# ttaoREtw/semi-tts

Hardware: AMD Instinct MI355X
Metric: mel-frames/sec (decode+attn) (higher is better)
Workload: dtype f32

## Files before the change

include/semitts.h:

```cpp
#ifndef SEMITTS_H
#define SEMITTS_H

#include <stddef.h>
#include <stdint.h>

#ifdef __cplusplus
extern "C" {
#endif

#define ST_ABI_VERSION 1

#define ST_ACT_NONE 0
#define ST_ACT_RELU 1
#define ST_ACT_TANH 2
#define ST_ACT_SIGMOID 3

const char* st_last_error(void);
int st_abi_version(void);
int st_device_info(int* n_cu, int* lds_bytes, char* name, int name_len);

int st_stream_create(void** stream_out);
int st_stream_destroy(void* stream);
int st_stream_sync(void* stream);
int st_graph_begin(void* stream);
// ... 5 lines not shown
int st_event_elapsed_ms(void* ev_start, void* ev_stop, float* ms_out);
int st_event_destroy(void* ev);

typedef struct st_seg {
    const float* x;
    const float* w;
    int ldx;
    int ldw;
    int k;
} st_seg;

int st_lstm_cell_fwd(const st_seg* segs, int nseg, const float* b_ih, const float* b_hh,
                     const float* pre, int ldpre, const float* c_prev, int ldc_prev,
                     const float* mask, float* h_out, int ldh, float* c_out, int ldc,
                     float* gates_out, int B, int H, void* stream);

int st_skinny_linear_fwd(const st_seg* segs, int nseg, const float* bias, int act,
                         const float* mask, int ldmask, float* y, int ldy,
                         int n_split, float* y2, int ldy2, int rep,
                         int B, int N, void* stream);

typedef struct st_t16_view {
    float* base;
    int kb_stride;
    int kb0;
} st_t16_view;

size_t st_packed_weight_floats(const int* k, int nseg, int N, int lstm_H);
size_t st_t16_floats(int B, int K);
int st_pack_weight(const float* const* w, const int* ldw, const int* k, int nseg, int N, int lstm_H,
                   float* packed, void* stream);
typedef struct st_pack_job { const float* w[3]; int ldw[3]; int k[3]; int nseg; int N; int lstm_H; float* packed; } st_pack_job;
int st_pack_weight_batch(const st_pack_job* jobs, int n, void* stream);
int st_pack_weight_t(const float* const* w, const int* ldw, const int* cols, int nseg, int K, float* packed, void* stream);
int st_tile_rows(const float* src, int ld, const st_t16_view* dst, int B, int K, void* stream);
int st_untile_rows(const st_t16_view* src, float* dst, int ld, int B, int K, void* stream);
int st_lstm_cell_packed_fwd(const float* packed_w, const st_t16_view* x, int K,
                            const float* b_ih, const float* b_hh,
                            const float* c_prev, int ldc_prev, const float* mask,
                            const st_t16_view* h_dst0, const st_t16_view* h_dst1,
                            float* c_out, int ldc, float* gates_out,
                            const float* ada_std, const float* ada_mean, const st_t16_view* hadapt_dst,
                            int B, int H, void* stream);
int st_lstm_cell_packed_part_fwd(const float* packed_w, int w_kbs, const st_t16_view* x, int K, const float* part,
                                 const float* b_ih, const float* b_hh,
                                 const float* c_prev, int ldc_prev, const float* mask,
                                 const st_t16_view* h_dst0, const st_t16_view* h_dst1,
                                 float* c_out, int ldc, float* gates_out, int B, int H, void* stream);
typedef struct st_lstm_cell_packed_job {
    const float* packed_w; st_t16_view x; int K;
    const float* b_ih; const float* b_hh;
    const float* c_prev; int ldc_prev; const float* mask;
    st_t16_view h_dst0; st_t16_view h_dst1;
    float* c_out; int ldc; float* gates_out;
    const float* ada_std; const float* ada_mean; st_t16_view hadapt_dst;
    int B, H;
    const float* part; int w_kbs;
} st_lstm_cell_packed_job;
int st_lstm_cell_packed_pair_fwd(const st_lstm_cell_packed_job* j0, const st_lstm_cell_packed_job* j1, void* stream);
int st_skinny_linear_packed_fwd(const float* packed_w, const st_t16_view* x, int K,
                                const float* bias, int act, const float* mask, int ldmask,
                                float* y, int ldy, const st_t16_view* y_dst,
                                int n_split, float* y2, int ldy2, int rep,
                                int n_split2, int act2, const float* mask2, int ldmask2, const st_t16_view* y3_dst,
                                int B, int N, void* stream);

int st_attn_step_fwd(const float* pq, const float* pm, const float* memory,
                     const float* w_prev, int ld_wprev, const float* w_cum_prev,
                     float* w_out, int ld_wout, float* w_cum_out,
                     const float* loc_conv_w, const float* loc_lin_w, const float* v,
                     float* ctx, int ld_ctx,
                     const float* h_q, int ld_hq, const float* ada_std, const float* ada_mean,
                     float* h_adapt, int Q,
                     int B, int L, int A, int E, int F, int K, void* stream);
int st_attn_step_t16_fwd(const float* pq, const float* pm, const float* memory,
                         const float* w_prev, int ld_wprev, const float* w_cum_prev,
                         float* w_out, int ld_wout, float* w_cum_out,
                         const float* loc_conv_w, const float* loc_lin_w, const float* v,
                         const st_t16_view* ctx_dst, int n_ctx_dst, float* ctx, int ld_ctx,
                         int B, int L, int A, int E, int F, int K, void* stream);
int st_attn_pre_fwd(const float* pm, const float* w_prev, int ld_wprev, const float* w_cum_prev,
                    const float* loc_conv_w, const float* loc_lin_w, float* s_buf, int parts,
                    int B, int L, int A, int F, int K, void* stream);
int st_attn_fin_t16_fwd(const float* pq, const float* s_buf, const float* memory, const float* w_cum_prev,
                        float* w_out, int ld_wout, float* w_cum_out, const float* v,
                        const st_t16_view* ctx_dst, int n_ctx_dst, float* ctx, int ld_ctx, int parts,
                        int B, int L, int A, int E, int F, int K, void* stream);
struct st_partial_product_job;
typedef struct st_attn_pre_job {
    const float* pm; const float* w_prev; int ld_wprev; const float* w_cum_prev;
    const float* loc_conv_w; const float* loc_lin_w; float* s_buf;
    int L, A, F, K;
    int parts;
    float* cf_out;
    const struct st_partial_product_job* part;
} st_attn_pre_job;
int st_skinny_linear_packed_attnpre_fwd(const float* packed_w, const st_t16_view* x, int K,
                                        const float* bias, int act, const float* mask, int ldmask,
                                        float* y, int ldy, const st_t16_view* y_dst,
                                        int n_split, float* y2, int ldy2, int rep,
                                        int n_split2, int act2, const float* mask2, int ldmask2, const st_t16_view* y3_dst,
                                        int B, int N, const st_attn_pre_job* pre, void* stream);

typedef struct st_lstm_pw_job {
    int n0, H;
    const float* dh1; int ld1;
    const float* dh2; int ld2; const float* scale2;
    const float* mask;
    const float* gates;
    const float* c; int ldc; const float* c_prev; int ldcp;
    float* dc;
    float* dgates; int ldg;
    st_t16_view dgates_t16;
    int dh1_slabs; long dh1_slab_stride;
} st_lstm_pw_job;
int st_skinny_linear_packed_lstm_bwd_fwd(const float* packed_w, const st_t16_view* x, int K, float* y, int ldy, int B, int N,
                                         const st_lstm_pw_job* job, void* stream);

size_t st_attn_fin_split_workspace_floats(int B, int E, int parts);
int st_attn_fin_split_fwd(const float* pq, const float* s_buf, const float* memory, const float* w_cum_prev,
                          float* w_out, int ld_wout, float* w_cum_out, const float* v,
                          const st_t16_view* ctx_dst, int n_ctx_dst, float* ctx, int ld_ctx, float* workspace, int parts,
                          int B, int L, int A, int E, void* stream);

typedef struct st_attn_fin_job {
    const float* s_buf; const float* memory; const float* w_cum_prev;
    float* w_out; int ld_wout; float* w_cum_out; const float* v;
    st_t16_view ctx_dst[3]; int n_ctx_dst;
    int parts;
    int L, A, E, F, K;
    unsigned* status;
} st_attn_fin_job;
int st_query_attn_fin_fwd(const float* packed_wq, const st_t16_view* h_q, int Q, unsigned long long* granules, unsigned epoch,
                          const st_attn_fin_job* job, int B, void* stream);
typedef struct st_partial_product_job {
    const float* packed_w; int w_kbs; int kb0; int KB;
    st_t16_view x;
    int N;
    float* part;
} st_partial_product_job;
int st_query_attn_fin_part_fwd(const float* packed_wq, const st_t16_view* h_q, int Q, unsigned long long* granules, unsigned epoch,
                               const st_attn_fin_job* job, int B, const st_partial_product_job* part, void* stream);
int st_partial_product_fwd(const st_partial_product_job* job, int B, void* stream);
int st_query_attn_rng_fits(int B, int A, int parts);
size_t st_attn_rng_xchg_words(int B, int E, int parts);
int st_query_attn_rng_fwd(const float* packed_wq, const st_t16_view* h_q, int Q, unsigned long long* granules,
                          unsigned long long* xchg, unsigned epoch, const st_attn_fin_job* job, int B, void* stream);
int st_handoff_wait_selftest(const unsigned long long* granules, unsigned epoch, int A, unsigned* status, float* out,
                             int max_spins, void* stream);

typedef struct st_gemm_epilogue {
    const float* bias;
    int act_pre;
    const float* bn_mean; const float* bn_var; const float* bn_w; const float* bn_b; float bn_eps;
    int act_post;
    const float* res; int ldres;
    const float* highway_h; int ldhw;
    const float* mask; int ldmask;
    int w_tap_major;
    float* splitk_ws;
    int splitk_slabs;
} st_gemm_epilogue;
int st_gemm_splitk_slabs(int Bn, int Tout, int Cin, int N, int KT);

int st_gemm_fwd(const float* A, int lda, const float* W, float* C, int ldc, int coff,
                int Bn, int Tin, int Tout, int Cin, int N, int KT, int pad, int stride, int pool_prev,
                const st_gemm_epilogue* ep, void* stream);

typedef struct st_gemm_job {
    const float* A; int lda; const float* W; float* C; int ldc; int coff;
    int Bn, Tin, Tout, Cin, N, KT, pad, stride, pool_prev;
    st_gemm_epilogue ep;
} st_gemm_job;
int st_gemm_fwd_batch(const st_gemm_job* jobs, int n, void* stream);
int st_gemm_fwd_variant(const float* A, int lda, const float* W, const float* C, int ldc, int coff,
                        int Bn, int Tin, int Tout, int Cin, int N, int KT, int pad, int stride, int pool_prev,
                        const st_gemm_epilogue* ep);
int st_gemm_fwd_batch_variant(const st_gemm_job* jobs, int n);
// ... 134 lines not shown
int st_vq_pack_table(const float* table, float* packed, int D, int V, void* stream);
int st_vq_l2_packed_fwd(const float* x, const float* table, const float* packed, const float* temp, float* p_code,
                        int64_t* idx, float* out, int n, int D, int V, void* stream);
size_t st_vq_l2_workspace_floats(int D, int V);
int st_softmax_bwd(const float* p, const float* dp, const float* relu_scale, float scale, float* dz, float* rowsum,
                   int n, int V, void* stream);
int st_rowscale_combine(const float* a, float alpha, const float* x, const float* r, float beta, const float* c,
                        float* out, int M, int D, void* stream);
int st_vq_mean_fwd(const float* p_code, const float* latent, float* out, int* lens, int* frame_seg, float* frame_w,
                   int B, int T, int D, int V, int max_frames_per_phn, void* stream);
int st_vq_mean_bwd(const float* dout, int n_seg_rows, const int* frame_seg, const float* frame_w, float* dlatent,
                   int B, int T, int D, void* stream);
int st_softmax_argmax(const float* logits, float* p, int64_t* idx, int n, int V, void* stream);

typedef struct st_decoder_weights {
    const float* prenet_w0;
    const float* prenet_w1;
    const float* q_w_ih;
    const float* q_w_hh;
    const float* q_b_ih; const float* q_b_hh;
    const float* attn_query_w;
    const float* attn_v;
    const float* attn_loc_conv_w;
    const float* attn_loc_lin_w;
    const float* d_w_ih;
    const float* d_w_hh;
    const float* d_b_ih; const float* d_b_hh;
    const float* projgate_w;
    const float* projgate_b;
    const float* pre_norm_w[2]; const float* pre_norm_b[2];
    float* pre_norm_rm[2]; float* pre_norm_rv[2]; long long* pre_norm_nbt[2];
    float pre_norm_eps, pre_norm_momentum;
} st_decoder_weights;

typedef struct st_decoder_dims {
    int B, L, E, n_mels, r, P, Q, D, A, F, K;
    int fuse_pre0;
    int prenet_norm;
} st_decoder_dims;

typedef struct st_decoder_io {
    const float* memory;
    const float* pm;
    const float* ada_std;
    const float* ada_mean;
    const int* step_src;
    const float* teacher_pre;
    const float* teacher_mean;
    int Bt, Tt;
    const float* prenet_mask;
    const float* q_mask;
    const float* d_mask;
    int steps;
    float* mel_out;
    float* align_out;
    float* stop_out;
    const float* packed;
    float* xq_tape; float* xd_tape; float* xo_tape;
    float* cq_tape; float* cd_tape; float* wcum_tape;
    float* pq_buf;
    float* pre1_t16;
    float* mel_t16;
    float* zero_row;
    float* gates_q_tape;
    float* gates_d_tape;
    float* attn_s_buf;
    int attn_pre_parts;
    int attn_fin_parts;
    int defer_proj;
    int pre1_step_floats;
    int attn_s_step_floats;
    float* attn_loc_tape;
    float* attn_split_ws;
    int attn_split_parts;
    unsigned long long* pq_granules;
    const float* dec_in0;
    float* pre_nat;
    unsigned long long* attn_xchg;
    unsigned* handoff_status;
    int pair_cells;
    float* pre_nat_tape;
    float* gate_part;
    int gate_part_k;
} st_decoder_io;

int st_decoder_gate_split_k(const st_decoder_dims* d);
size_t st_decoder_packed_floats(const st_decoder_dims* d);
size_t st_decoder_tape_floats(const st_decoder_dims* d, int which);
int st_decoder_pack(const st_decoder_weights* w, const st_decoder_dims* d, float* packed, void* stream);
int st_decoder_forward(const st_decoder_weights* w, const st_decoder_dims* d, const st_decoder_io* io,
                       void* stream);
int st_decoder_fwd_forms(const st_decoder_dims* d, const st_decoder_io* io, int cus, int rng_capacity);

int st_attn_step_bwd(const float* pq, const float* pm, const float* memory,
                     const float* w_prev, int ld_wprev, const float* w_cum_prev, const float* w, int ld_w,
                     const float* loc_conv_w, const float* loc_lin_w, const float* v,
                     const float* const* dctx, const int* ld_dctx, int n_dctx,
                     const float* const* dw_direct, const int* ld_dw, int n_dw,
                     float* dcum, const float* dcum_add, int ld_dcum_add,
                     float* dpq, float* dhist, float* ds_t, float* loc_t, float* dloc_t, float* hist_t,
                     float* dctx_t, float* dv_t,
                     int B, int L, int A, int E, int F, int K, void* stream);

int st_attn_dmem(const float* align, const float* dctx_tape, float* dmem, int B, int steps, int L, int E, void* stream);

typedef struct st_decoder_bwd_weights {
    const float* q_w_cat_t;
    const float* d_w_cat_t;
    const float* attn_query_w_t;
    const float* q_w_cat_t_p16;
    const float* d_w_cat_t_p16;
    const float* attn_query_w_t_p16;
    const float* attn_v; const float* attn_loc_conv_w; const float* attn_loc_lin_w;
} st_decoder_bwd_weights;

typedef struct st_decoder_bwd_io {
    const float* memory; const float* pm; const float* ada_std;
    const float* align;
    const float* wcum_tape;
    const float* cq_tape; const float* cd_tape;
    const float* gates_q_tape; const float* gates_d_tape;
    const float* q_mask; const float* d_mask;
    const float* pq_all;
    int steps; int Bp;
    const float* dxo;
    const float* dalign;
    float* dgq; float* dgd;
    float* dxq; float* dxd;
    float* dpq;
    float* ds_tape; float* loc_tape; float* dloc_tape;
    float* hist_tape; float* dctx_tape; float* dv_tape;
    float* dcq; float* dcd;
    float* dhist[2];
    float* dcum;
    float* dhq_attn;
    float* dgq_t16; float* dgd_t16;
    const int* step_src; int Bt;
    float* dY;
    float* dxo_rw;
    const float* wpg_t;
    const float* pre_w1_t; const float* pre_w0_t;
    const float* own_mask;
    const float* xq_nat;
    const float* pre1_nat;
    float* d2_tape; float* dp1_tape;
    float* tmp_p; float* tmp_in;
    int fuse_pw;
    float* dgd_t16_b;
    float* dpq_t16;
    int need_dxq0;
    const float* attn_s_tape;
    int overlap_attn;
    int prenet_norm;
    const float* pre_y_tape;
    const float* pre_norm_w[2]; const float* pre_norm_rm[2]; const float* pre_norm_rv[2];
    float pre_norm_eps;
    float* dpre_norm_w[2]; float* dpre_norm_b[2];
    int attn_parts; float* dloc_part;
    float* dxd_part; int dxd_splits;
    float* dxq_part; int dxq_splits;
} st_decoder_bwd_io;
int st_decoder_bwd_fuse_dims(const st_decoder_dims* d);
int st_decoder_bwd_forms(const st_decoder_dims* d, const st_decoder_bwd_io* io);
int st_attn_step_bwd_s(const float* pq, const float* pm, const float* memory,
                       const float* w_prev, int ld_wprev, const float* w_cum_prev, const float* w, int ld_w,
                       const float* loc_conv_w, const float* loc_lin_w, const float* v,
                       const float* const* dctx, const int* ld_dctx, int n_dctx,
                       const float* const* dw_direct, const int* ld_dw, int n_dw,
                       float* dcum, const float* dcum_add, int ld_dcum_add,
                       float* dpq, float* dhist, float* ds_t, float* loc_t, float* dloc_t, float* hist_t,
                       float* dctx_t, float* dv_t, const float* s_in,
                       int B, int L, int A, int E, int F, int K, void* stream);
int st_attn_step_bwd_t16(const float* pq, const float* pm, const float* memory,
                         const float* w_prev, int ld_wprev, const float* w_cum_prev, const float* w, int ld_w,
                         const float* loc_conv_w, const float* loc_lin_w, const float* v,
// ... 152 lines not shown
```

semi_tts_amd/_lib.py:

```python
import ctypes as C
import os

HERE = os.path.dirname(os.path.abspath(__file__))
LIB_PATH = os.environ.get('ST_LIB_PATH') or os.path.join(HERE, 'lib', 'libsemitts_hip.so')

c_float_p = C.c_void_p
c_void_p = C.c_void_p


class StSeg(C.Structure):
    _fields_ = [('x', C.c_void_p), ('w', C.c_void_p), ('ldx', C.c_int), ('ldw', C.c_int), ('k', C.c_int)]


class StT16View(C.Structure):
    _fields_ = [('base', C.c_void_p), ('kb_stride', C.c_int), ('kb0', C.c_int)]


class StGemmEpilogue(C.Structure):
    _fields_ = [('bias', C.c_void_p), ('act_pre', C.c_int),
                ('bn_mean', C.c_void_p), ('bn_var', C.c_void_p), ('bn_w', C.c_void_p), ('bn_b', C.c_void_p),
                ('bn_eps', C.c_float), ('act_post', C.c_int),
                ('res', C.c_void_p), ('ldres', C.c_int),
                ('highway_h', C.c_void_p), ('ldhw', C.c_int),
                ('mask', C.c_void_p), ('ldmask', C.c_int), ('w_tap_major', C.c_int),
                ('splitk_ws', C.c_void_p), ('splitk_slabs', C.c_int)]


class StGemmJob(C.Structure):
    _fields_ = [('A', C.c_void_p), ('lda', C.c_int), ('W', C.c_void_p), ('C', C.c_void_p), ('ldc', C.c_int), ('coff', C.c_int),
                ('Bn', C.c_int), ('Tin', C.c_int), ('Tout', C.c_int), ('Cin', C.c_int), ('N', C.c_int), ('KT', C.c_int),
                ('pad', C.c_int), ('stride', C.c_int), ('pool_prev', C.c_int), ('ep', StGemmEpilogue)]


class StRelayoutDesc(C.Structure):
    _fields_ = [('src', C.c_void_p), ('dst', C.c_void_p), ('N', C.c_int), ('Cin', C.c_int), ('KT', C.c_int), ('mode', C.c_int),
                ('blk0', C.c_int), ('ld_dst', C.c_int)]


class StBnBankSeg(C.Structure):
    _fields_ = [('x', C.c_void_p), ('ldx', C.c_int), ('T', C.c_int), ('w', C.c_void_p), ('b', C.c_void_p), ('run_mean', C.c_void_p),
                ('run_var', C.c_void_p), ('batches_tracked', C.c_void_p), ('momentum', C.c_float), ('eps', C.c_float),
                ('mean', C.c_void_p), ('var', C.c_void_p), ('dx', C.c_void_p), ('lddx', C.c_int), ('sums', C.c_void_p)]


class StDecoderWeights(C.Structure):
    _fields_ = [(n, C.c_void_p) for n in (
        'prenet_w0', 'prenet_w1', 'q_w_ih', 'q_w_hh', 'q_b_ih', 'q_b_hh',
        'attn_query_w', 'attn_v', 'attn_loc_conv_w', 'attn_loc_lin_w',
        'd_w_ih', 'd_w_hh', 'd_b_ih', 'd_b_hh', 'projgate_w', 'projgate_b')] + [
        ('pre_norm_w', C.c_void_p * 2), ('pre_norm_b', C.c_void_p * 2), ('pre_norm_rm', C.c_void_p * 2), ('pre_norm_rv', C.c_void_p * 2),
        ('pre_norm_nbt', C.c_void_p * 2), ('pre_norm_eps', C.c_float), ('pre_norm_momentum', C.c_float)]


class StDecoderDims(C.Structure):
    _fields_ = [(n, C.c_int) for n in ('B', 'L', 'E', 'n_mels', 'r', 'P', 'Q', 'D', 'A', 'F', 'K', 'fuse_pre0', 'prenet_norm')]


class StDecoderIO(C.Structure):
    _fields_ = [('memory', C.c_void_p), ('pm', C.c_void_p), ('ada_std', C.c_void_p), ('ada_mean', C.c_void_p),
                ('step_src', C.POINTER(C.c_int)), ('teacher_pre', C.c_void_p), ('teacher_mean', C.c_void_p),
                ('Bt', C.c_int), ('Tt', C.c_int),
                ('prenet_mask', C.c_void_p), ('q_mask', C.c_void_p), ('d_mask', C.c_void_p),
                ('steps', C.c_int),
                ('mel_out', C.c_void_p), ('align_out', C.c_void_p), ('stop_out', C.c_void_p),
                ('packed', C.c_void_p),
                ('xq_tape', C.c_void_p), ('xd_tape', C.c_void_p), ('xo_tape', C.c_void_p),
                ('cq_tape', C.c_void_p), ('cd_tape', C.c_void_p), ('wcum_tape', C.c_void_p),
                ('pq_buf', C.c_void_p), ('pre1_t16', C.c_void_p), ('mel_t16', C.c_void_p),
                ('zero_row', C.c_void_p),
                ('gates_q_tape', C.c_void_p), ('gates_d_tape', C.c_void_p), ('attn_s_buf', C.c_void_p), ('attn_pre_parts', C.c_int), ('attn_fin_parts', C.c_int), ('defer_proj', C.c_int),
                ('pre1_step_floats', C.c_int), ('attn_s_step_floats', C.c_int), ('attn_loc_tape', C.c_void_p),
                ('attn_split_ws', C.c_void_p), ('attn_split_parts', C.c_int), ('pq_granules', C.c_void_p),
                ('dec_in0', C.c_void_p), ('pre_nat', C.c_void_p), ('attn_xchg', C.c_void_p), ('handoff_status', C.c_void_p),
                ('pair_cells', C.c_int), ('pre_nat_tape', C.c_void_p), ('gate_part', C.c_void_p), ('gate_part_k', C.c_int)]


class StDecoderBwdWeights(C.Structure):
    _fields_ = [(n, C.c_void_p) for n in ('q_w_cat_t', 'd_w_cat_t', 'attn_query_w_t', 'q_w_cat_t_p16', 'd_w_cat_t_p16', 'attn_query_w_t_p16',
                                          'attn_v', 'attn_loc_conv_w', 'attn_loc_lin_w')]


class StDecoderBwdIO(C.Structure):
    _fields_ = ([(n, C.c_void_p) for n in ('memory', 'pm', 'ada_std', 'align', 'wcum_tape', 'cq_tape', 'cd_tape',
                                           'gates_q_tape', 'gates_d_tape', 'q_mask', 'd_mask', 'pq_all')] +
                [('steps', C.c_int), ('Bp', C.c_int)] +
                [(n, C.c_void_p) for n in ('dxo', 'dalign', 'dgq', 'dgd', 'dxq', 'dxd', 'dpq', 'ds_tape', 'loc_tape', 'dloc_tape',
                                           'hist_tape', 'dctx_tape', 'dv_tape', 'dcq', 'dcd')] +
                [('dhist', C.c_void_p * 2), ('dcum', C.c_void_p), ('dhq_attn', C.c_void_p), ('dgq_t16', C.c_void_p),
                 ('dgd_t16', C.c_void_p), ('step_src', C.POINTER(C.c_int)), ('Bt', C.c_int)] +
                [(n, C.c_void_p) for n in ('dY', 'dxo_rw', 'wpg_t', 'pre_w1_t', 'pre_w0_t', 'own_mask', 'xq_nat', 'pre1_nat',
                                           'd2_tape', 'dp1_tape', 'tmp_p', 'tmp_in')] +
                [('fuse_pw', C.c_int), ('dgd_t16_b', C.c_void_p), ('dpq_t16', C.c_void_p), ('need_dxq0', C.c_int), ('attn_s_tape', C.c_void_p),
                 ('overlap_attn', C.c_int), ('prenet_norm', C.c_int), ('pre_y_tape', C.c_void_p), ('pre_norm_w', C.c_void_p * 2),
                 ('pre_norm_rm', C.c_void_p * 2), ('pre_norm_rv', C.c_void_p * 2), ('pre_norm_eps', C.c_float),
                 ('dpre_norm_w', C.c_void_p * 2), ('dpre_norm_b', C.c_void_p * 2), ('attn_parts', C.c_int), ('dloc_part', C.c_void_p),
                 ('dxd_part', C.c_void_p), ('dxd_splits', C.c_int), ('dxq_part', C.c_void_p), ('dxq_splits', C.c_int)])



class StLstmPwJob(C.Structure):
    _fields_ = [('n0', C.c_int), ('H', C.c_int), ('dh1', C.c_void_p), ('ld1', C.c_int), ('dh2', C.c_void_p), ('ld2', C.c_int),
                ('scale2', C.c_void_p), ('mask', C.c_void_p), ('gates', C.c_void_p), ('c', C.c_void_p), ('ldc', C.c_int),
                ('c_prev', C.c_void_p), ('ldcp', C.c_int), ('dc', C.c_void_p), ('dgates', C.c_void_p), ('ldg', C.c_int),
                ('dgates_t16', StT16View), ('dh1_slabs', C.c_int), ('dh1_slab_stride', C.c_long)]


class StLstmCellPackedJob(C.Structure):
    _fields_ = [('packed_w', C.c_void_p), ('x', StT16View), ('K', C.c_int), ('b_ih', C.c_void_p), ('b_hh', C.c_void_p),
                ('c_prev', C.c_void_p), ('ldc_prev', C.c_int), ('mask', C.c_void_p), ('h_dst0', StT16View), ('h_dst1', StT16View),
                ('c_out', C.c_void_p), ('ldc', C.c_int), ('gates_out', C.c_void_p), ('ada_std', C.c_void_p), ('ada_mean', C.c_void_p),
                ('hadapt_dst', StT16View), ('B', C.c_int), ('H', C.c_int), ('part', C.c_void_p), ('w_kbs', C.c_int)]


class StAttnBwdJob(C.Structure):
    _fields_ = [('pq', C.c_void_p), ('pm', C.c_void_p), ('memory', C.c_void_p),
                ('w_prev', C.c_void_p), ('ld_wprev', C.c_int), ('w_cum_prev', C.c_void_p), ('w', C.c_void_p), ('ld_w', C.c_int),
                ('loc_conv_w', C.c_void_p), ('loc_lin_w', C.c_void_p), ('v', C.c_void_p),
                ('dctx', C.c_void_p * 3), ('ld_dctx', C.c_int * 3), ('n_dctx', C.c_int),
                ('dw_direct', C.c_void_p * 3), ('ld_dw', C.c_int * 3), ('n_dw', C.c_int),
                ('dcum', C.c_void_p), ('dcum_add', C.c_void_p), ('ld_dcum_add', C.c_int),
                ('dpq', C.c_void_p), ('dpq_t16', StT16View), ('dhist', C.c_void_p), ('ds_t', C.c_void_p), ('loc_t', C.c_void_p),
                ('dloc_t', C.c_void_p), ('hist_t', C.c_void_p), ('dctx_t', C.c_void_p), ('dv_t', C.c_void_p), ('s_in', C.c_void_p),
                ('B', C.c_int), ('L', C.c_int), ('A', C.c_int), ('E', C.c_int), ('F', C.c_int), ('K', C.c_int),
                ('parts', C.c_int), ('dloc_part', C.c_void_p),
                ('dctx_more', C.c_void_p * 3), ('ld_dctx_more', C.c_int * 3), ('n_dctx_more', C.c_int)]


class StAttnHistJob(C.Structure):
    _fields_ = [('dloc_part', C.c_void_p), ('parts', C.c_int), ('loc_conv_w', C.c_void_p),
                ('w_prev', C.c_void_p), ('ld_wprev', C.c_int), ('w_cum_prev', C.c_void_p),
                ('dloc_t', C.c_void_p), ('hist_t', C.c_void_p), ('dhist', C.c_void_p), ('dcum', C.c_void_p),
                ('B', C.c_int), ('L', C.c_int), ('F', C.c_int), ('K', C.c_int)]


class StWgradJob(C.Structure):
    _fields_ = [('dC', C.c_void_p), ('lddc', C.c_int), ('dcoff', C.c_int), ('A', C.c_void_p), ('lda', C.c_int), ('dW', C.c_void_p), ('db', C.c_void_p),
                ('Bn', C.c_int), ('Tin', C.c_int), ('Tout', C.c_int), ('Cin', C.c_int), ('N', C.c_int), ('KT', C.c_int), ('pad', C.c_int)]


class StPartialSumJob(C.Structure):
    _fields_ = [('part', C.c_void_p), ('S', C.c_int), ('N', C.c_int), ('y', C.c_void_p), ('ldy', C.c_int), ('pw', C.c_void_p)]


class StAttnPreJob(C.Structure):
    _fields_ = [('pm', C.c_void_p), ('w_prev', C.c_void_p), ('ld_wprev', C.c_int), ('w_cum_prev', C.c_void_p),
                ('loc_conv_w', C.c_void_p), ('loc_lin_w', C.c_void_p), ('s_buf', C.c_void_p),
                ('L', C.c_int), ('A', C.c_int), ('F', C.c_int), ('K', C.c_int), ('parts', C.c_int), ('cf_out', C.c_void_p),
                ('part', C.c_void_p)]


class StAttnFinJob(C.Structure):
    _fields_ = [('s_buf', C.c_void_p), ('memory', C.c_void_p), ('w_cum_prev', C.c_void_p),
                ('w_out', C.c_void_p), ('ld_wout', C.c_int), ('w_cum_out', C.c_void_p), ('v', C.c_void_p),
                ('ctx_dst', StT16View * 3), ('n_ctx_dst', C.c_int), ('parts', C.c_int),
                ('L', C.c_int), ('A', C.c_int), ('E', C.c_int), ('F', C.c_int), ('K', C.c_int), ('status', C.c_void_p)]


P, I, F, Z = C.c_void_p, C.c_int, C.c_float, C.c_size_t

SIGNATURES = {
    'st_last_error': [],
    'st_abi_version': [],
    'st_device_info': [C.POINTER(I), C.POINTER(I), C.c_char_p, I],
    'st_stream_create': [C.POINTER(P)],
    'st_stream_destroy': [P],
    'st_stream_sync': [P],
    'st_graph_begin': [P],
    'st_graph_end': [P, C.POINTER(P)],
    'st_graph_launch': [P, P],
    'st_graph_destroy': [P],
    'st_event_create': [C.POINTER(P)],
    'st_event_record': [P, P],
    'st_event_elapsed_ms': [P, P, C.POINTER(F)],
    'st_event_destroy': [P],
    'st_lstm_cell_fwd': [C.POINTER(StSeg), I, P, P, P, I, P, I, P, P, I, P, I, P, I, I, P],
    'st_skinny_linear_fwd': [C.POINTER(StSeg), I, P, I, P, I, P, I, I, P, I, I, I, I, P],
    'st_attn_step_fwd': [P, P, P, P, I, P, P, I, P, P, P, P, P, I, P, I, P, P, P, I, I, I, I, I, I, I, P],
    'st_gemm_fwd': [P, I, P, P, I, I, I, I, I, I, I, I, I, I, I, C.POINTER(StGemmEpilogue), P],
    'st_gemm_fwd_batch': [C.POINTER(StGemmJob), I, P],
    'st_gemm_fwd_variant': [P, I, P, P, I, I, I, I, I, I, I, I, I, I, I, C.POINTER(StGemmEpilogue)],
    'st_gemm_fwd_batch_variant': [C.POINTER(StGemmJob), I],
    'st_highway_stack_supported': [I, I],
    'st_highway_stack_fwd': [P, I, C.POINTER(P), C.POINTER(P), C.POINTER(P), C.POINTER(P), I, P, I, I, I, P],
    'st_gemm_splitk_slabs': [I, I, I, I, I],
    'st_bn_stats': [P, I, I, I, I, P, P, P, P, F, P, P, P],
    'st_colreduce_workspace_floats': [I, I],
    'st_bn_apply': [P, I, I, I, I, P, P, P, P, F, I, P],
    'st_lstm_seq_fwd': [P, P, P, P, I, I, P, P, P, I, I, I, I, P],
    'st_lstm_cell_bwd_pointwise': [P, I, P, I, P, I, P, P, P, P, I, P, I, P, P, I, C.POINTER(StT16View), I, I, P],
    'st_lstm_seq_bwd': [P, I, I, P, P, P, P, P, I, I, I, I, P],
    'st_gru_seq_fwd': [P, P, P, P, P, P, P, I, P, I, I, I, I, P],
    'st_gru_seq_bwd': [P, I, P, I, P, P, P, P, P, P, P, I, I, I, I, P],
    'st_gru_seq_variant': [I, I],
    'st_vq_build_table': [P, I, P, I, P, P, I, P, I, P],
    'st_gather_rows': [P, P, P, I, I, I, P],
    'st_vq_l2_fwd': [P, P, P, P, P, P, P, I, I, I, P],
    'st_vq_pack_table': [P, P, I, I, P],
    'st_vq_l2_packed_fwd': [P, P, P, P, P, P, P, I, I, I, P],
    'st_vq_l2_workspace_floats': [I, I],
    'st_ctc_workspace_floats': [I, I],
    'st_ctc_loss': [P, P, C.c_float, P, P, P, I, I, I, I, I, P],
    'st_ctc_greedy_edit_distance': [P, I, I, I, P, I, P, I, P, P, P, P, P],
    'st_ids_edit_distance': [P, I, I, P, I, P, I, P, P, P, P, P],
    'st_hyp_edit_distance': [P, P, I, I, P, I, P, I, P, P, P],
    'st_ctc_beam_workspace_bytes': [I, I, I],
    'st_ctc_beam_search': [P, I, I, I, P, I, I, I, I, F, P, P, P, P, P],
    'st_ctc_beam_search_lm': [P, I, I, I, P, I, I, I, I, F, P, I, I, P, P, P, P, P],
    'st_ctc_align_workspace_bytes': [I, I, I],
    'st_ctc_forced_align': [P, I, I, I, P, P, I, P, I, I, F, P, P, P, P, P, P],
    'st_scalar_combine': [P, I, P, I, P, P],
    'st_scalar_fanout': [P, P, I, P, P],
    'st_softmax_bwd': [P, P, P, C.c_float, P, P, I, I, P],
    'st_rowscale_combine': [P, C.c_float, P, P, C.c_float, P, P, I, I, P],
    'st_vq_mean_fwd': [P, P, P, P, P, P, I, I, I, I, I, P],
    'st_vq_mean_bwd': [P, I, P, P, P, I, I, I, P],
    'st_softmax_argmax': [P, P, P, I, I, P],
    'st_packed_weight_floats': [C.POINTER(I), I, I, I],
    'st_t16_floats': [I, I],
    'st_pack_weight': [C.POINTER(P), C.POINTER(I), C.POINTER(I), I, I, I, P, P],
    'st_pack_weight_t': [C.POINTER(P), C.POINTER(I), C.POINTER(I), I, I, P, P],
    'st_relayout_blocks': [I, I, I],
    'st_relayout_batch': [P, I, I, P, P],
    'st_pack_weight_batch': [P, I, P],
    'st_tile_rows': [P, I, C.POINTER(StT16View), I, I, P],
    'st_untile_rows': [C.POINTER(StT16View), P, I, I, I, P],
    'st_lstm_cell_packed_fwd': [P, C.POINTER(StT16View), I, P, P, P, I, P, C.POINTER(StT16View), C.POINTER(StT16View),
                                P, I, P, P, P, C.POINTER(StT16View), I, I, P],
    'st_lstm_cell_packed_part_fwd': [P, I, C.POINTER(StT16View), I, P, P, P, P, I, P, C.POINTER(StT16View), C.POINTER(StT16View),
                                     P, I, P, I, I, P],
    'st_lstm_cell_packed_pair_fwd': [C.POINTER(StLstmCellPackedJob), C.POINTER(StLstmCellPackedJob), P],
    'st_skinny_linear_packed_fwd': [P, C.POINTER(StT16View), I, P, I, P, I, P, I, C.POINTER(StT16View), I, P, I, I,
                                    I, I, P, I, C.POINTER(StT16View), I, I, P],
    'st_attn_step_t16_fwd': [P, P, P, P, I, P, P, I, P, P, P, P, C.POINTER(StT16View), I, P, I, I, I, I, I, I, I, P],
    'st_skinny_linear_packed_attnpre_fwd': [P, C.POINTER(StT16View), I, P, I, P, I, P, I, C.POINTER(StT16View), I, P, I, I,
                                            I, I, P, I, C.POINTER(StT16View), I, I, C.POINTER(StAttnPreJob), P],
    'st_attn_pre_fwd': [P, P, I, P, P, P, P, I, I, I, I, I, I, P],
    'st_attn_fin_t16_fwd': [P, P, P, P, P, I, P, P, C.POINTER(StT16View), I, P, I, I, I, I, I, I, I, I, P],
    'st_attn_fin_split_workspace_floats': [I, I, I],
    'st_attn_fin_split_fwd': [P, P, P, P, P, I, P, P, C.POINTER(StT16View), I, P, I, P, I, I, I, I, I, P],
    'st_query_attn_fin_fwd': [P, C.POINTER(StT16View), I, P, C.c_uint, C.POINTER(StAttnFinJob), I, P],
    'st_query_attn_fin_part_fwd': [P, C.POINTER(StT16View), I, P, C.c_uint, C.POINTER(StAttnFinJob), I, P, P],
    'st_partial_product_fwd': [P, I, P],
    'st_layer_norm_fwd': [P, I, P, P, F, P, I, P, P, I, I, P],
    'st_layer_norm_bwd': [P, I, P, I, P, P, P, P, I, P, I, I, P],
    'st_log_softmax_fwd': [P, P, I, I, P],
    'st_log_softmax_bwd': [P, P, P, I, I, P],
    'st_prenet_norm_fwd': [P, I, I, P, P, P, P, P, F, F, P, I, C.POINTER(StT16View), I, I, I, P],
    'st_prenet_norm_bwd': [P, I, P, I, I, P, P, P, F, P, P, I, I, P],
    'st_handoff_wait_selftest': [P, C.c_uint, I, P, P, I, P],
    'st_query_attn_rng_fits': [I, I, I],
    'st_attn_rng_xchg_words': [I, I, I],
    'st_query_attn_rng_fwd': [P, C.POINTER(StT16View), I, P, P, C.c_uint, C.POINTER(StAttnFinJob), I, P],
    'st_decoder_packed_floats': [C.POINTER(StDecoderDims)],
    'st_decoder_gate_split_k': [C.POINTER(StDecoderDims)],
    'st_decoder_tape_floats': [C.POINTER(StDecoderDims), I],
    'st_decoder_pack': [C.POINTER(StDecoderWeights), C.POINTER(StDecoderDims), P, P],
    'st_decoder_forward': [C.POINTER(StDecoderWeights), C.POINTER(StDecoderDims), C.POINTER(StDecoderIO), P],
    'st_decoder_fwd_forms': [C.POINTER(StDecoderDims), C.POINTER(StDecoderIO), I, I],
    'st_attn_step_bwd': [P, P, P, P, I, P, P, I, P, P, P, C.POINTER(P), C.POINTER(I), I, C.POINTER(P), C.POINTER(I), I,
                         P, P, I, P, P, P, P, P, P, P, P, I, I, I, I, I, I, P],
    'st_attn_step_bwd_s': [P, P, P, P, I, P, P, I, P, P, P, C.POINTER(P), C.POINTER(I), I, C.POINTER(P), C.POINTER(I), I,
                           P, P, I, P, P, P, P, P, P, P, P, P, I, I, I, I, I, I, P],
    'st_attn_step_bwd_t16': [P, P, P, P, I, P, P, I, P, P, P, C.POINTER(P), C.POINTER(I), I, C.POINTER(P), C.POINTER(I), I,
                             P, P, I, P, C.POINTER(StT16View), P, P, P, P, P, P, P, P, I, I, I, I, I, I, P],
    'st_skinny_linear_packed_lstm_bwd_fwd': [P, C.POINTER(StT16View), I, P, I, I, I, C.POINTER(StLstmPwJob), P],
    'st_skinny_linear_packed_lstm_bwd_attn_bwd': [P, C.POINTER(StT16View), I, P, I, I, I, C.POINTER(StLstmPwJob), C.POINTER(StAttnBwdJob), P],
    'st_attn_bwd_wide_fits': [I, I, I, I, I],
    'st_attn_bwd_variant': [I, I, I, I, I, I, I, I, I, I, P],
    'st_skinny_linear_packed_attn_hist': [P, C.POINTER(StT16View), I, P, I, I, I, C.POINTER(StAttnHistJob), P],
    'st_skinny_partial_attn_hist': [P, C.POINTER(StT16View), I, P, I, I, I, C.POINTER(StAttnHistJob), P],
    'st_decoder_bwd_forms': [C.POINTER(StDecoderDims), C.POINTER(StDecoderBwdIO)],
    'st_decoder_bwd_fuse_dims': [C.POINTER(StDecoderDims)],
    'st_loop_graph_stats': [P, P],
    'st_loop_graphs_enable': [I],
    'st_skinny_partial_attn_bwd': [P, C.POINTER(StT16View), I, P, I, I, I, C.POINTER(StAttnBwdJob), P],
    'st_skinny_linear_packed_lstm_bwd_attn_hist_sum': [P, C.POINTER(StT16View), I, P, I, I, I, C.POINTER(StLstmPwJob), C.POINTER(StAttnHistJob),
                                                       C.POINTER(StPartialSumJob), P],
    'st_skinny_linear_packed_lstm_bwd_attn_hist': [P, C.POINTER(StT16View), I, P, I, I, I, C.POINTER(StLstmPwJob), C.POINTER(StAttnHistJob), P],
    'st_lstm_seq2_fwd': [C.POINTER(P), C.POINTER(P), C.POINTER(P), P, I, C.POINTER(I), P, C.POINTER(P), C.POINTER(P), I, I, I, P],
    'st_lstm_seq2_persist_supported': [I, I, I, I, I, I],
    'st_lstm_seq2_persist_fwd': [C.POINTER(P), C.POINTER(P), C.POINTER(P), P, I, C.POINTER(I), C.POINTER(P), C.POINTER(P), I, I, I, P, P],
    'st_lstm_seq2_bwd_persist_supported': [I, I, I, I, I, I],
    'st_lstm_seq2_bwd_persist': [P, I, C.POINTER(I), C.POINTER(P), C.POINTER(P), C.POINTER(P), C.POINTER(P), I, I, I, P, P],
    'st_lstm_seq2_bwd': [P, I, C.POINTER(I), C.POINTER(P), C.POINTER(P), C.POINTER(P), C.POINTER(P), P, I, I, I, P],
    'st_skinny_linear_pair_fwd': [P, C.POINTER(P), I, I, I, P],
    'st_lstm_seq2_bwd_packed': [P, I, C.POINTER(I), C.POINTER(P), C.POINTER(P), C.POINTER(P), C.POINTER(P), P, P, I, I, I, P],
    'st_skinny_linear_packed_lstm_bwd_pair_fwd': [C.POINTER(P), C.POINTER(StT16View), I, C.POINTER(P), I, I, I, C.POINTER(StLstmPwJob), P],
    'st_lstm_cell_pair_fwd': [P, C.POINTER(P), C.POINTER(P), I, C.POINTER(P), I, C.POINTER(P), I, C.POINTER(P), I, C.POINTER(P), I, I, P],
    'st_attn_dmem': [P, P, P, I, I, I, I, P],
    'st_decoder_backward': [C.POINTER(StDecoderBwdWeights), C.POINTER(StDecoderDims), C.POINTER(StDecoderBwdIO), P],
    'st_decoder_pack_dout': [P, P, P, I, I, I, I, I, I, P],
    'st_decoder_unpack_out': [P, P, P, I, I, I, I, I, I, P],
    'st_decoder_dteacher_sum': [P, P, I, I, I, I, I, I, I, P],
    'st_adain_bwd': [P, C.c_long, I, P, C.c_long, I, P, P, P, P, I, I, I, P],
    'st_mt_blocks': [P, I],
    'st_mt_table_misses': [],
    'st_mt_grad_norm': [P, P, I, P, P, P],
    'st_mt_clip_scale': [P, P, I, P, F, P],
    'st_mt_grad_norm_scaled': [P, P, I, P, P, F, P],
    'st_mt_clip_scale_pre': [P, P, I, P, F, F, P],
    'st_mt_copy': [P, P, P, I, P],
    'st_mt_adam': [P, P, P, P, P, I, F, F, F, F, F, P],
    'st_mt_adam_guarded': [P, P, P, P, P, I, F, F, F, F, F, P, P],
    'st_freq_loss': [P, P, P, P, P, I, I, I, I, F, F, F, I, P],
    'st_freq_loss_workspace_floats': [],
    'st_scale_by': [P, P, P, Z, P],
    'st_bn_norm_fwd': [P, I, I, P, I, I, I, I, P, P, P, P, F, I, P],
    'st_gemm_wgrad_workspace_floats': [I, I, I, I, I],
    'st_gemm_wgrad': [P, I, I, P, I, P, P, I, I, I, I, I, I, I, I, I, P],
    'st_gemm_wgrad_db': [P, I, I, P, I, P, P, P, I, I, I, I, I, I, I, I, I, P],
    'st_gemm_wgrad_batch_workspace_floats': [C.POINTER(StWgradJob), I],
    'st_gemm_wgrad_batch': [C.POINTER(StWgradJob), I, P, P],
    'st_gemm_wgrad_variant': [P, I, I, P, I, I, I, I, I, I, I, I, I, I, I, I],
    'st_gemm_wgrad_batch_variant': [C.POINTER(StWgradJob), I, C.POINTER(I)],
    'st_gemm_wgrad_split': [P, I, I, P, I, P, I, P, P, P, P, I, I, I, I, P],
    'st_colsum': [P, I, I, P, I, I, I, I, P, I, P, P],
    'st_act_bwd': [P, I, P, I, I, P, I, P, I, I, I, P],
    'st_bn_bwd': [P, I, I, P, I, I, I, P, I, I, P, P, P, F, I, I, P, I, I, P, P, I, P, P],
    'st_bn_bwd_reduce': [P, I, I, P, I, I, I, P, I, I, P, P, F, I, I, P, P, P],
    'st_bn_norm_res_mask_fwd': [P, P, P, I, I, P, P, P, P, F, I, P, P, P],
    'st_bn_bwd_reduce_masked': [P, I, P, I, P, I, I, P, I, P, P, F, I, I, P, P, P],
    'st_bn_bwd_apply_masked': [P, I, P, I, P, I, I, P, I, P, P, P, F, I, I, P, I, P, P, I, P, I, P],
    'st_bn_bwd_apply': [P, I, I, P, I, I, I, P, I, I, P, P, P, F, I, I, P, I, P, I, I, P],
    'st_bn_stats_record': [P, I, I, I, I, P, P, P, P],
    'st_bn_sync_merge': [P, I, I, P, P, P, P, F, P, P],
    'st_bn_bwd_apply_sync': [P, I, I, P, I, I, I, P, I, I, P, P, P, F, I, I, P, P, P, I, I, P],
    'st_highway_fwd': [P, P, P, P, Z, P],
    'st_bn_bank_workspace_floats': [I, I, I],
    'st_bn_bank_fwd': [C.POINTER(StBnBankSeg), I, I, I, P, I, I, P, P],
    'st_bn_bank_bwd': [C.POINTER(StBnBankSeg), I, I, I, P, I, I, I, P, P],
    'st_bn_bank_stats_record': [C.POINTER(StBnBankSeg), I, I, I, P, P, P],
    'st_bn_bank_sync_merge': [C.POINTER(StBnBankSeg), I, I, I, P, I, P, P],
    'st_bn_bank_norm': [C.POINTER(StBnBankSeg), I, I, I, P, I, I, P],
    'st_bn_bank_bwd_reduce': [C.POINTER(StBnBankSeg), I, I, I, P, I, I, P, P],
    'st_bn_bank_bwd_apply': [C.POINTER(StBnBankSeg), I, I, I, P, I, I, I, P, P],
    'st_highway_ht_fwd': [P, P, P, I, I, P],
    'st_highway_ht_bwd': [P, P, P, P, P, I, I, P],
    'st_highway_bwd': [P, P, P, P, P, P, P, Z, P],
    'st_pool_prev_fwd': [P, P, I, I, I, P],
    'st_pool_prev_bwd': [P, P, P, I, I, I, P],
    'st_copy3d': [P, C.c_long, C.c_long, P, C.c_long, C.c_long, I, I, I, I, P],
    'st_scatter_add_rows': [P, P, P, I, I, I, P],
    'st_fill': [P, F, Z, P],
    'st_copy2d': [P, I, P, I, I, I, P],
    'st_mean_rows': [P, P, I, I, I, P],
    'st_istft_workspace_floats': [I, I, I, I, I],
    'st_gl_workspace_floats': [I, I, I, I, I],
    'st_stft_fwd': [P, P, I, I, I, I, I, P],
    'st_istft': [P, P, I, I, I, I, I, P, P],
    'st_griffin_lim': [P, C.c_long, C.c_long, C.c_long, I, F, P, P, I, I, I, I, I, I, I, P, P],
    'st_features_workspace_floats': [I],
    'st_audio_features': [P, C.c_long, P, C.c_ulonglong, P, P, P, P, P, I, I, I, I, I, F, P, P, P, P, I, P, P, I, P, I, P, P],
    'st_feature_noise': [P, C.c_long, I, C.c_ulonglong, P],
}
_RESTYPES = {'st_last_error': C.c_char_p, 'st_packed_weight_floats': C.c_size_t, 'st_t16_floats': C.c_size_t,
             'st_decoder_packed_floats': C.c_size_t, 'st_vq_l2_workspace_floats': C.c_size_t, 'st_ctc_workspace_floats': C.c_size_t, 'st_decoder_tape_floats': C.c_size_t,
             'st_gemm_wgrad_workspace_floats': C.c_size_t, 'st_gemm_wgrad_batch_workspace_floats': C.c_size_t, 'st_freq_loss_workspace_floats': C.c_size_t, 'st_attn_fin_split_workspace_floats': C.c_size_t, 'st_attn_rng_xchg_words': C.c_size_t, 'st_colreduce_workspace_floats': C.c_size_t, 'st_mt_blocks': C.c_size_t, 'st_mt_table_misses': C.c_long,
             'st_bn_bank_workspace_floats': C.c_size_t, 'st_istft_workspace_floats': C.c_size_t, 'st_gl_workspace_floats': C.c_size_t,
             'st_features_workspace_floats': C.c_size_t, 'st_ctc_beam_workspace_bytes': C.c_size_t, 'st_ctc_align_workspace_bytes': C.c_size_t}

_lib = None


def load():
    global _lib
    if _lib is not None:
        return _lib
    import torch
    if not os.path.exists(LIB_PATH):
        raise RuntimeError(
            'libsemitts_hip.so not found at %s -- build it with `python -m semi_tts_amd.build` '
            '(hipcc --offload-arch=gfx950).  There is no CPU fallback.' % LIB_PATH)
    lib = C.CDLL(LIB_PATH)
    for name, args in SIGNATURES.items():
        fn = getattr(lib, name)
        fn.argtypes = args
        fn.restype = _RESTYPES.get(name, C.c_int)
    if lib.st_abi_version() != 1:
        raise RuntimeError('libsemitts_hip.so ABI version mismatch')
    _lib = lib
    return lib


def check(rc, what):
    if rc != 0:
        msg = load().st_last_error()
        raise RuntimeError('%s failed (%d): %s' % (what, rc, msg.decode() if msg else '?'))


def check_header_symbols():
    import re
    hdr = open(os.path.join(os.path.dirname(HERE), 'include', 'semitts.h')).read()
    declared = sorted(set(re.findall(r'\b(st_[a-z0-9_]+)\s*\(', hdr)))
    lib = C.CDLL(LIB_PATH)
    missing = [s for s in declared if not hasattr(lib, s)]
    if missing:
        raise RuntimeError('declared in include/semitts.h but not exported by %s: %s' % (LIB_PATH, missing))
    if sorted(SIGNATURES) != declared:
        raise RuntimeError('ctypes table and include/semitts.h disagree: %s' % sorted(set(SIGNATURES) ^ set(declared)))
    return declared
```

semi_tts_amd/csrc/attention.hip:

```cpp
#include "attention_body.h"

namespace {

template <int PART>
int at_launch(const AtArgs& a, hipStream_t stream) {
    ST_CHECK_ARG(a.B > 0 && a.L > 0 && a.A > 0 && a.E > 0 && a.F > 0 && a.K > 0, "attention step: bad dims");
    ST_CHECK_ARG(a.K % 2 == 1, "attention step: location kernel size %d must be odd", a.K);
    ST_CHECK_ARG(a.E % 4 == 0 && a.E / 4 <= AT_THREADS, "attention step: E=%d must be a multiple of 4 and <= %d", a.E, 4 * AT_THREADS);
    ST_CHECK_ARG(PART == 1 || st_aligned16(a.memory), "attention step: memory must be 16-byte aligned");
    ST_CHECK_ARG((a.A % 4 != 0) || (st_aligned16(a.pm) && st_aligned16(a.pq) && st_aligned16(a.v)),
                 "attention step: pm/pq/v must be 16-byte aligned");
    ST_CHECK_ARG(PART == 1 || a.ctx || a.ctx_dst[0].base, "attention step: no context output");
    ST_CHECK_ARG(PART == 0 || (a.s_buf && ((a.A % 4 != 0) || st_aligned16(a.s_buf))), "attention step: S buffer missing / unaligned");
    ST_CHECK_ARG(!a.h_q || (a.ada_std && a.ada_mean && a.h_adapt), "attention step: AdaIN pointers");
    const bool vec = (a.A % 4 == 0) && (a.F % 4 == 0) && st_aligned16(a.pm) && (PART == 1 || (st_aligned16(a.pq) && st_aligned16(a.v))) &&
                     st_aligned16(a.loc_lin_w);
    const int pre_parts = PART == 1 && a.pre_parts > 1 ? a.pre_parts : 1;
    const AtLds o = at_layout(a.L, a.A, a.E, a.F, a.K, PART, at_pos_per(a.L, pre_parts), PART == 1 && vec && a.F == 32 && a.A % 16 == 0);
    const size_t lds_bytes = (size_t)o.total * sizeof(float);
    ST_CHECK_ARG(lds_bytes <= 160 * 1024, "attention step: L=%d needs %zu B of LDS (> 160 KiB)%s", a.L, lds_bytes,
                 PART == 0 ? "; the split form (st_attn_pre_fwd with more parts + st_attn_fin_t16_fwd) takes longer texts" : "");
    static bool configured = false;
    if (!configured) {
        ST_HIP(hipFuncSetAttribute(reinterpret_cast<const void*>(at_kernel<true, PART>),
// ... 131 lines not shown
    for (int p = 0; p < CPF; ++p) cpf[p] = wsb[(size_t)min(p, P - 1) * (4 + E) + 4 + min(tid, E - 1)];
    if (tid < 64) {
        const float m = tid < P ? wsb[(size_t)tid * (4 + E)] : -INFINITY;
        const float s = tid < P ? wsb[(size_t)tid * (4 + E) + 1] : 0.0f;
        const float M = st_wave_max_dpp(m);
        const float t = tid < P ? s * __expf(m - M) : 0.0f;
        const float D = st_wave_sum_dpp(t);
        sc[tid] = tid < P ? __expf(m - M) / D : 0.0f;
    }
    __syncthreads();
    for (int e = tid; e < E; e += AT_THREADS) {
        float s = 0.0f;
        if (e == tid) {
#pragma unroll
            for (int p = 0; p < CPF; ++p) s = p < P ? fmaf(sc[p], cpf[p], s) : s;
            for (int p = CPF; p < P; ++p) s = fmaf(sc[p], wsb[(size_t)p * (4 + E) + 4 + e], s);
        } else {
            for (int p = 0; p < P; ++p) s = fmaf(sc[p], wsb[(size_t)p * (4 + E) + 4 + e], s);
        }
        if (a.ctx) a.ctx[(size_t)b * a.ld_ctx + e] = s;
#pragma unroll
        for (int d = 0; d < 3; ++d)
            if (a.ctx_dst[d].base) a.ctx_dst[d].base[at_t16_off(b, a.ctx_dst[d].kb0 * 16 + e, a.ctx_dst[d].kb_stride)] = s;
    }
    for (int l = tid; l < a.L; l += AT_THREADS) {
        const float w = a.w[(size_t)b * a.ld_w + l] * sc[l / a.Lp];
        a.w[(size_t)b * a.ld_w + l] = w;
        a.w_cum_out[(size_t)b * a.L + l] = w + a.w_cum_prev[(size_t)b * a.L + l];
    }
}

}

extern "C" int st_attn_step_fwd(const float* pq, const float* pm, const float* memory,
                                const float* w_prev, int ld_wprev, const float* w_cum_prev,
                                float* w_out, int ld_wout, float* w_cum_out,
                                const float* loc_conv_w, const float* loc_lin_w, const float* v,
                                float* ctx, int ld_ctx,
                                const float* h_q, int ld_hq, const float* ada_std, const float* ada_mean,
                                float* h_adapt, int Q,
                                int B, int L, int A, int E, int F, int K, void* stream) {
    (void)hipGetLastError();
    AtArgs a;
    memset(&a, 0, sizeof(a));
    a.pq = pq; a.pm = pm; a.memory = memory; a.w_prev = w_prev; a.ld_wprev = ld_wprev; a.w_cum_prev = w_cum_prev;
    a.w_out = w_out; a.ld_wout = ld_wout; a.w_cum_out = w_cum_out;
    a.loc_conv_w = loc_conv_w; a.loc_lin_w = loc_lin_w; a.v = v; a.ctx = ctx; a.ld_ctx = ld_ctx;
    a.h_q = h_q; a.ld_hq = ld_hq; a.ada_std = ada_std; a.ada_mean = ada_mean; a.h_adapt = h_adapt; a.Q = Q;
    a.B = B; a.L = L; a.A = A; a.E = E; a.F = F; a.K = K;
    return at_launch<0>(a, (hipStream_t)stream);
}

extern "C" int st_attn_step_t16_fwd(const float* pq, const float* pm, const float* memory,
                                    const float* w_prev, int ld_wprev, const float* w_cum_prev,
                                    float* w_out, int ld_wout, float* w_cum_out,
                                    const float* loc_conv_w, const float* loc_lin_w, const float* v,
                                    const st_t16_view* ctx_dst, int n_ctx_dst, float* ctx, int ld_ctx,
                                    int B, int L, int A, int E, int F, int K, void* stream) {
    (void)hipGetLastError();
    ST_CHECK_ARG(n_ctx_dst >= 0 && n_ctx_dst <= 3 && (n_ctx_dst == 0 || ctx_dst), "st_attn_step_t16_fwd: n_ctx_dst=%d", n_ctx_dst);
    AtArgs a;
    memset(&a, 0, sizeof(a));
    a.pq = pq; a.pm = pm; a.memory = memory; a.w_prev = w_prev; a.ld_wprev = ld_wprev; a.w_cum_prev = w_cum_prev;
    a.w_out = w_out; a.ld_wout = ld_wout; a.w_cum_out = w_cum_out;
    a.loc_conv_w = loc_conv_w; a.loc_lin_w = loc_lin_w; a.v = v; a.ctx = ctx; a.ld_ctx = ld_ctx;
    for (int d = 0; d < n_ctx_dst; ++d) a.ctx_dst[d] = ctx_dst[d];
    a.B = B; a.L = L; a.A = A; a.E = E; a.F = F; a.K = K;
    return at_launch<0>(a, (hipStream_t)stream);
}

extern "C" int st_attn_pre_fwd(const float* pm, const float* w_prev, int ld_wprev, const float* w_cum_prev,
                               const float* loc_conv_w, const float* loc_lin_w, float* s_buf, int parts,
                               int B, int L, int A, int F, int K, void* stream) {
    (void)hipGetLastError();
    AtArgs a;
    memset(&a, 0, sizeof(a));
    a.pm = pm; a.w_prev = w_prev; a.ld_wprev = ld_wprev; a.w_cum_prev = w_cum_prev;
    a.loc_conv_w = loc_conv_w; a.loc_lin_w = loc_lin_w; a.s_buf = s_buf;
    a.pre_parts = (parts >= 2 && parts <= 64 && (parts & (parts - 1)) == 0) ? parts : 1;
    a.B = B; a.L = L; a.A = A; a.E = 4; a.F = F; a.K = K;
    return at_launch<1>(a, (hipStream_t)stream);
}

extern "C" int st_attn_fin_t16_fwd(const float* pq, const float* s_buf, const float* memory, const float* w_cum_prev,
                                   float* w_out, int ld_wout, float* w_cum_out, const float* v,
                                   const st_t16_view* ctx_dst, int n_ctx_dst, float* ctx, int ld_ctx, int parts,
                                   int B, int L, int A, int E, int F, int K, void* stream) {
    (void)hipGetLastError();
    ST_CHECK_ARG(n_ctx_dst >= 0 && n_ctx_dst <= 3 && (n_ctx_dst == 0 || ctx_dst), "st_attn_fin_t16_fwd: n_ctx_dst=%d", n_ctx_dst);
    ST_CHECK_ARG(parts == 1 || ((parts == 2 || parts == 4 || parts == 8) && E % (4 * parts) == 0),
                 "st_attn_fin_t16_fwd: parts=%d must be 1, 2, 4 or 8 with E=%d a multiple of 4*parts", parts, E);
    AtArgs a;
    memset(&a, 0, sizeof(a));
    a.pq = pq; a.pm = s_buf; a.s_buf = const_cast<float*>(s_buf); a.memory = memory; a.w_cum_prev = w_cum_prev;
    a.w_out = w_out; a.ld_wout = ld_wout; a.w_cum_out = w_cum_out; a.v = v; a.ctx = ctx; a.ld_ctx = ld_ctx;
    a.loc_lin_w = s_buf;
    a.fin_parts = parts;
    for (int d = 0; d < n_ctx_dst; ++d) a.ctx_dst[d] = ctx_dst[d];
    a.B = B; a.L = L; a.A = A; a.E = E; a.F = F; a.K = K;
    return at_launch<2>(a, (hipStream_t)stream);
}

extern "C" size_t st_attn_fin_split_workspace_floats(int B, int E, int parts) { return (size_t)B * parts * (4 + E); }

extern "C" int st_attn_fin_split_fwd(const float* pq, const float* s_buf, const float* memory, const float* w_cum_prev,
                                     float* w_out, int ld_wout, float* w_cum_out, const float* v,
                                     const st_t16_view* ctx_dst, int n_ctx_dst, float* ctx, int ld_ctx, float* workspace, int parts,
                                     int B, int L, int A, int E, void* stream) {
    (void)hipGetLastError();
    ST_CHECK_ARG(pq && s_buf && memory && w_cum_prev && w_out && w_cum_out && v && workspace && B > 0 && L > 0, "st_attn_fin_split_fwd: bad arguments");
    ST_CHECK_ARG(n_ctx_dst >= 0 && n_ctx_dst <= 3 && (n_ctx_dst == 0 || ctx_dst) && (ctx || n_ctx_dst > 0), "st_attn_fin_split_fwd: context outputs");
    ST_CHECK_ARG(A % 4 == 0 && A >= 4 && A <= 256 && E % 4 == 0 && E / 4 <= AT_THREADS && AT_THREADS % (E / 4) == 0,
                 "st_attn_fin_split_fwd: A=%d must be a multiple of 4 up to 256, E=%d / 4 a divisor of %d", A, E, AT_THREADS);
    ST_CHECK_ARG(parts >= 2 && parts <= 64, "st_attn_fin_split_fwd: parts=%d (2..64)", parts);
    const int Lp = (L + parts - 1) / parts;
    ST_CHECK_ARG(Lp <= 512, "st_attn_fin_split_fwd: %d positions per part (> 512): use more parts", Lp);
    parts = (L + Lp - 1) / Lp;
    ST_CHECK_ARG(st_aligned16(pq) && st_aligned16(s_buf) && st_aligned16(memory) && st_aligned16(v) && st_aligned16(workspace),
                 "st_attn_fin_split_fwd: operands must be 16-byte aligned");
    AsArgs s;
    memset(&s, 0, sizeof(s));
    s.pq = pq; s.s_buf = s_buf; s.memory = memory; s.v = v; s.w_tmp = w_out; s.ld_w = ld_wout; s.ws = workspace;
    s.B = B; s.L = L; s.A = A; s.E = E; s.P = parts; s.Lp = Lp;
    hipLaunchKernelGGL(at_split_kernel, dim3(B * parts), dim3(AT_THREADS), 0, (hipStream_t)stream, s);
    ST_LAUNCH_CHECK();
    AcArgs c;
    memset(&c, 0, sizeof(c));
    c.ws = workspace; c.w = w_out; c.ld_w = ld_wout; c.w_cum_prev = w_cum_prev; c.w_cum_out = w_cum_out; c.ctx = ctx; c.ld_ctx = ld_ctx;
    for (int d = 0; d < n_ctx_dst; ++d) c.ctx_dst[d] = ctx_dst[d];
    c.B = B; c.L = L; c.E = E; c.P = parts; c.Lp = Lp;
    hipLaunchKernelGGL(at_combine_kernel, dim3(B), dim3(AT_THREADS), 0, (hipStream_t)stream, c);
    ST_LAUNCH_CHECK();
    return 0;
}


namespace {
__global__ __launch_bounds__(64) void handoff_wait_kernel(const unsigned long long* granules, unsigned epoch, int A, unsigned* status,
                                                          float* out, int max_spins) {
    const int lane = threadIdx.x;
    const f32x4 q4 = at_wait_granules(granules, epoch, lane, A, status, max_spins);
    if (lane * 4 < A) *reinterpret_cast<f32x4*>(out + lane * 4) = q4;
}
}

extern "C" int st_handoff_wait_selftest(const unsigned long long* granules, unsigned epoch, int A, unsigned* status, float* out,
                                        int max_spins, void* stream) {
    (void)hipGetLastError();
    ST_CHECK_ARG(granules && out && A > 0 && A % 4 == 0 && A <= 256 && max_spins > 0 && st_aligned16(out),
                 "st_handoff_wait_selftest: bad arguments");
    hipLaunchKernelGGL(handoff_wait_kernel, dim3(1), dim3(64), 0, (hipStream_t)stream, granules, epoch, A, status, out, max_spins);
    ST_LAUNCH_CHECK();
    return 0;
}
```

semi_tts_amd/csrc/attention_body.h:

```cpp
#pragma once
#include "st_common.h"

#ifndef AT_PROF
#define AT_PROF(n)
#endif

namespace {

constexpr int AT_THREADS = 512;
constexpr int AT_WAVES = AT_THREADS / 64;
constexpr int AT_PF = 12;
constexpr int AT_LB = 8;
constexpr int AT_LP = 6;
constexpr int AT_CB = 4;
constexpr int AT_WLPF = 4;

struct AtArgs {
    const float* pq; const float* pm; const float* memory;
    const float* w_prev; int ld_wprev; const float* w_cum_prev;
    float* w_out; int ld_wout; float* w_cum_out;
    const float* loc_conv_w; const float* loc_lin_w; const float* v;
    float* ctx; int ld_ctx; st_t16_view ctx_dst[3];
    const float* h_q; int ld_hq; const float* ada_std; const float* ada_mean; float* h_adapt; int Q;
    float* s_buf;
    float* cf_out;
    int pre_parts;
    int fin_parts;
    int B, L, A, E, F, K;
    const unsigned long long* pq_gran; unsigned epoch;
    unsigned* status;
};

constexpr int AT_GRAN_SPINS = 1 << 18;
__device__ __forceinline__ f32x4 at_wait_granules(const unsigned long long* base, unsigned epoch, int lane, int A, unsigned* status,
                                                  int max_spins) {
    typedef __attribute__((address_space(1))) unsigned long long gu64;
    gu64* gp = (gu64*)(base + min(lane * 4, A - 4));
    unsigned long long g0 = 0, g1 = 0, g2 = 0, g3 = 0;
    bool ok = false;
    for (int spins = 0; spins < max_spins; ++spins) {
        g0 = __hip_atomic_load(gp + 0, __ATOMIC_RELAXED, __HIP_MEMORY_SCOPE_AGENT);
        g1 = __hip_atomic_load(gp + 1, __ATOMIC_RELAXED, __HIP_MEMORY_SCOPE_AGENT);
        g2 = __hip_atomic_load(gp + 2, __ATOMIC_RELAXED, __HIP_MEMORY_SCOPE_AGENT);
        g3 = __hip_atomic_load(gp + 3, __ATOMIC_RELAXED, __HIP_MEMORY_SCOPE_AGENT);
        const bool mine = (unsigned)(g0 >> 32) == epoch && (unsigned)(g1 >> 32) == epoch &&
                          (unsigned)(g2 >> 32) == epoch && (unsigned)(g3 >> 32) == epoch;
        ok = __all(mine);
        if (ok) break;
        __builtin_amdgcn_s_sleep(2);
    }
    if (!ok && lane == 0 && status) __hip_atomic_fetch_or(status, 1u, __ATOMIC_RELAXED, __HIP_MEMORY_SCOPE_AGENT);
    const float nanv = __builtin_nanf("");
    return ok ? f32x4{__uint_as_float((unsigned)g0), __uint_as_float((unsigned)g1), __uint_as_float((unsigned)g2),
                      __uint_as_float((unsigned)g3)}
              : f32x4{nanv, nanv, nanv, nanv};
}

struct AtLds {
    int wt, wt_ld, wc, kp, hs, hl, cf, cf_ld, e, part, total;
};

__host__ __device__ inline int at_pos_per(int L, int nparts) {
    return nparts > 1 ? (((L + nparts - 1) / nparts + 11) / 12) * 12 : L;
}

__host__ __device__ inline AtLds at_layout(int L, int A, int E, int F, int K, int part = 0, int Lr = 0, bool pre_mfma = false) {
    AtLds o;
    int p = 0;
    const int Lh = part == 1 ? Lr : L;
    o.wt_ld = ((A + 3) & ~3) + 4;
    o.wt = p; if (part == 0 || (part == 1 && !pre_mfma)) p += F * o.wt_ld;
    o.kp = K <= 32 ? 32 : ((K + 3) & ~3);
    o.wc = p; if (part != 2) p += F * 2 * o.kp;
    o.hl = ((Lh + AT_CB + o.kp + 3) + 3) & ~3;
    o.hs = p; if (part != 2) p += 2 * o.hl;
    o.cf_ld = ((((Lh + AT_LP - 1) / AT_LP) * AT_LP + AT_CB + 3) & ~3) + (part == 1 ? 16 : 0);
    o.cf = p; if (part != 2) p += F * o.cf_ld;
    o.e = p; p += ((L + 3) & ~3);
    o.part = p; p += 4 * AT_THREADS;
    o.total = p;
    return o;
}

__device__ __forceinline__ float at_tanh(float x) {
    const float t = __expf(-2.0f * fabsf(x));
    return copysignf(__fdividef(1.0f - t, 1.0f + t), x);
}

__device__ __forceinline__ size_t at_t16_off(int b, int k, int KB) {
    return (((size_t)(b >> 4) * KB + (k >> 4)) * 64 + ((k >> 2) & 3) * 16 + (b & 15)) * 4 + (k & 3);
}

__device__ __forceinline__ void at_put_granule(unsigned long long* p, float v, unsigned epoch) {
    typedef __attribute__((address_space(1))) unsigned long long gu64;
    __hip_atomic_store((gu64*)p, ((unsigned long long)epoch << 32) | (unsigned long long)__float_as_uint(v), __ATOMIC_RELAXED,
                       __HIP_MEMORY_SCOPE_AGENT);
}

struct ArArgs {
    const float* s_buf; const float* memory; const float* v; const float* w_cum_prev;
    float* w_out; int ld_wout; float* w_cum_out;
    st_t16_view ctx_dst[3];
    const unsigned long long* pq_gran;
    unsigned long long* xchg;
    unsigned epoch; unsigned* status;
    int B, L, A, E, P, Lp;
};

template <int NT>
__device__ __forceinline__ void at_range_body(const ArArgs& a, const int wg) {
    __shared__ float es[512];
    __shared__ __attribute__((aligned(16))) float part[4 * NT];
    __shared__ __attribute__((aligned(16))) float pqs[256];
    __shared__ __attribute__((aligned(16))) float cb[8 * 256];
// ... 484 lines not shown
                const float keep = hi32 ? esum[j + 4] : esum[j];
                r4[j] = keep + __shfl_xor(send, 32, 64);
            }
#pragma unroll
            for (int j = 0; j < 2; ++j) {
                const float send = hi16 ? r4[j] : r4[j + 2];
                const float keep = hi16 ? r4[j + 2] : r4[j];
                r2[j] = keep + __shfl_xor(send, 16, 64);
            }
            float r = (hi8 ? r2[1] : r2[0]) + st_dpp<ST_DPP_ROW_ROR8>(hi8 ? r2[0] : r2[1]);
            r = st_oct_sum_dpp(r);
            const int l = l0 + (lane >> 3);
            if ((lane & 7) == 0 && (lane >> 3) < AT_LP && l < L) es[l] = r;
        }
    };
#pragma unroll
    for (int i = 0; i < NPB; ++i) {
        const int l0 = (wave + i * NWV) * AT_LP;
        if (l0 < pos_hi) energy_block(l0, pf_pm4[i]);
    }
    for (int l0 = pos_lo + (wave + NPB * NWV) * AT_LP; l0 < pos_hi; l0 += NWV * AT_LP) energy_block(l0, nullptr);
    if (PART == 1) return;
    AT_PROF(6);
    st_lds_barrier();
    AT_PROF(7);

    if (wave == 0) {
        float m = -INFINITY;
        for (int l = lane; l < L; l += 64) m = fmaxf(m, es[l]);
        m = st_wave_max_dpp(m);
        float s = 0.0f;
        for (int l = lane; l < L; l += 64) {
            const float ex = expf(es[l] - m);
            es[l] = ex;
            s += ex;
        }
        s = st_wave_sum_dpp(s);
        for (int l = lane; l < L; l += 64) {
            const float w = es[l] / s;
            es[l] = w;
            if (PART == 2 && ipart != 0) continue;
            a.w_out[(size_t)b * a.ld_wout + l] = w;
            const float cum_prev = PART == 2 ? (VEC && l < 64 ? pf_cum : a.w_cum_prev[(size_t)b * L + l]) : hs[o.hl + pad + l];
            a.w_cum_out[(size_t)b * L + l] = w + cum_prev;
        }
    }
    AT_PROF(8);
    st_lds_barrier();
    AT_PROF(9);

    if (ctx_active) {
        f32x4 acc = {0.f, 0.f, 0.f, 0.f};
#pragma unroll
        for (int j = 0; j < PFR; ++j) {
            const int l = g + j * ng;
            const float wv = es[min(l, L - 1)];
            const float w = l < L ? wv : 0.0f;
            acc[0] = fmaf(w, mpf[j][0], acc[0]); acc[1] = fmaf(w, mpf[j][1], acc[1]);
            acc[2] = fmaf(w, mpf[j][2], acc[2]); acc[3] = fmaf(w, mpf[j][3], acc[3]);
        }
        for (int l = g + PFR * ng; l < L; l += ng) {
            const f32x4 m4 = st_ld4(memb + (size_t)l * E + e_lo + e4 * 4);
            const float w = es[l];
            acc[0] = fmaf(w, m4[0], acc[0]); acc[1] = fmaf(w, m4[1], acc[1]);
            acc[2] = fmaf(w, m4[2], acc[2]); acc[3] = fmaf(w, m4[3], acc[3]);
        }
        *reinterpret_cast<f32x4*>(part + (size_t)(g * ne4 + e4) * 4) = acc;
    }
    AT_PROF(10);
    st_lds_barrier();
    AT_PROF(11);
    for (int e = tid; e < Es; e += NT) {
        float s = 0.0f;
        for (int gg = 0; gg < ng; ++gg) s += part[gg * Es + e];
        if (a.ctx) a.ctx[(size_t)b * a.ld_ctx + e_lo + e] = s;
#pragma unroll
        for (int d = 0; d < 3; ++d)
            if (a.ctx_dst[d].base) a.ctx_dst[d].base[at_t16_off(b, a.ctx_dst[d].kb0 * 16 + e_lo + e, a.ctx_dst[d].kb_stride)] = s;
    }
    AT_PROF(12);
}


template <bool VEC, int PART, int NT = AT_THREADS>
__global__ __launch_bounds__(NT) void at_kernel(const float* pq, const float* pm, const float* v, const float* w_cum_prev, const float* memory,
                                                float* s_buf, const int L, const int A, const int E, const int fin_parts, const AtArgs rest) {
    extern __shared__ __attribute__((aligned(16))) float at_lds[];
    AtArgs a = rest;
    a.pq = pq; a.pm = pm; a.v = v; a.w_cum_prev = w_cum_prev; a.memory = memory; a.s_buf = s_buf; a.L = L; a.A = A; a.E = E; a.fin_parts = fin_parts;
    at_body<VEC, PART, NT>(a, blockIdx.x, at_lds);
}

}
```

semi_tts_amd/csrc/decoder.hip:

```cpp
#include "st_common.h"
#include "loop_graph.h"
#include <cstdlib>

namespace {

struct ZeroArgs { float* p[12]; size_t floats[12]; int n; };
__global__ __launch_bounds__(256) void zero_regions_kernel(const ZeroArgs a) {
    float* __restrict__ p = a.p[blockIdx.y];
    const size_t n = a.floats[blockIdx.y];
    const size_t n4 = (((uintptr_t)p & 15u) == 0) ? n / 4 : 0;
    const f32x4 z = {0.f, 0.f, 0.f, 0.f};
    for (size_t i = (size_t)blockIdx.x * blockDim.x + threadIdx.x; i < n4; i += (size_t)gridDim.x * blockDim.x) reinterpret_cast<f32x4*>(p)[i] = z;
    for (size_t i = n4 * 4 + (size_t)blockIdx.x * blockDim.x + threadIdx.x; i < n; i += (size_t)gridDim.x * blockDim.x) p[i] = 0.0f;
}

}

extern "C" size_t st_packed_weight_floats(const int* k, int nseg, int N, int lstm_H);
extern "C" size_t st_t16_floats(int B, int K);

namespace {

struct PackedLayout {
    size_t q, pq, d, pg, p0, p1, total;
};

PackedLayout packed_layout(const st_decoder_dims* d) {
    PackedLayout o;
    const int in_dim = d->r * d->n_mels;
    size_t p = 0;
    { int k[3] = {d->P, d->E, d->Q}; o.q = p; p += st_packed_weight_floats(k, 3, 4 * d->Q, d->Q); }
    { int k[1] = {d->Q}; o.pq = p; p += st_packed_weight_floats(k, 1, d->A, 0); }
    { int k[3] = {d->E, d->Q, d->D}; o.d = p; p += st_packed_weight_floats(k, 3, 4 * d->D, d->D); }
    { int k[2] = {d->D, d->E}; o.pg = p; p += st_packed_weight_floats(k, 2, in_dim + 1 + (d->fuse_pre0 ? d->P : 0), 0); }
    { int k[1] = {in_dim}; o.p0 = p; p += st_packed_weight_floats(k, 1, d->P, 0); }
    { int k[1] = {d->P}; o.p1 = p; p += st_packed_weight_floats(k, 1, d->P, 0); }
    o.total = p;
    return o;
}

inline int kb16(int k) { return (k + 15) >> 4; }

struct StepViews {
    int q_kbs, q_ctx, q_h;
    int d_kbs, d_ha, d_h;
    int o_kbs, o_ctx;
    size_t q_floats, d_floats, o_floats;
};

StepViews step_views(const st_decoder_dims* d) {
    StepViews v;
    const int bt = (d->B + 15) >> 4;
    v.q_ctx = kb16(d->P); v.q_h = v.q_ctx + kb16(d->E); v.q_kbs = v.q_h + kb16(d->Q);
    v.d_ha = kb16(d->E); v.d_h = v.d_ha + kb16(d->Q); v.d_kbs = v.d_h + kb16(d->D);
    v.o_ctx = kb16(d->D); v.o_kbs = v.o_ctx + kb16(d->E);
    v.q_floats = (size_t)bt * v.q_kbs * 256; v.d_floats = (size_t)bt * v.d_kbs * 256; v.o_floats = (size_t)bt * v.o_kbs * 256;
    return v;
}

__global__ __launch_bounds__(256) void tile_teacher_kernel(const float* teacher_pre, int Tt, float* xq_tape, size_t slot_floats,
                                                           int q_kbs, int steps, int Bt, int P) {
    const size_t total = (size_t)(steps - 1) * Bt * P;
    for (size_t i = (size_t)blockIdx.x * blockDim.x + threadIdx.x; i < total; i += (size_t)gridDim.x * blockDim.x) {
        const int k = (int)(i % P);
        const size_t sb = i / P;
        const int b = (int)(sb % Bt), s = (int)(sb / Bt) + 1;
        const int frame = s - 1 < Tt ? s - 1 : Tt - 1;
        const float v = teacher_pre[((size_t)b * Tt + frame) * P + k];
        xq_tape[(size_t)s * slot_floats + (((size_t)(b >> 4) * q_kbs + (k >> 4)) * 64 + ((k >> 2) & 3) * 16 + (b & 15)) * 4 + (k & 3)] = v;
    }
}

int prenet_own(const st_decoder_weights* w, const st_decoder_dims* d, const st_decoder_io* io, const PackedLayout& pl, const StepViews& sv,
               int t, bool layer1_done, void* stream) {
    const int in_dim = d->r * d->n_mels;
    const size_t BP = (size_t)d->B * d->P;
    const float* m1 = io->prenet_mask ? io->prenet_mask + ((size_t)t * 2 + 0) * BP : nullptr;
    const float* m2 = io->prenet_mask ? io->prenet_mask + ((size_t)t * 2 + 1) * BP : nullptr;
    st_t16_view mel = {io->mel_t16, kb16(in_dim), 0};
    st_t16_view pre1 = {io->pre1_t16 + (size_t)t * io->pre1_step_floats, kb16(d->P), 0};
    int rc = 0;
    if (d->prenet_norm) {
        st_t16_view next_n = {io->xq_tape + (size_t)(t + 1) * sv.q_floats, sv.q_kbs, 0};
        const st_t16_view* dsts[2] = {&pre1, &next_n};
        const st_t16_view* srcs[2] = {&mel, &pre1};
        const float* pw[2] = {io->packed + pl.p0, io->packed + pl.p1};
        const int Ks[2] = {16 * kb16(in_dim), 16 * kb16(d->P)};
        const float* ms[2] = {m1, m2};
        const int b0 = io->step_src[t] == -1 ? 0 : io->Bt;
        for (int l = 0; l < 2; ++l) {
            float* y = io->pre_nat_tape ? io->pre_nat_tape + ((size_t)t * 2 + l) * BP : io->pre_nat;
            rc = st_skinny_linear_packed_fwd(pw[l], srcs[l], Ks[l], nullptr, ST_ACT_NONE, nullptr, 0, y, d->P, nullptr, 0,
                                             nullptr, 0, 0, 0, 0, nullptr, 0, nullptr, d->B, d->P, stream);
            if (rc) return rc;
            rc = st_prenet_norm_fwd(y, d->P, d->prenet_norm, w->pre_norm_w[l], w->pre_norm_b[l], w->pre_norm_rm[l], w->pre_norm_rv[l],
                                    w->pre_norm_nbt[l], w->pre_norm_eps, w->pre_norm_momentum, ms[l], d->P, dsts[l], b0, d->B, d->P, stream);
            if (rc) return rc;
        }
        return 0;
    }
    if (!layer1_done)
        rc = st_skinny_linear_packed_fwd(io->packed + pl.p0, &mel, 16 * kb16(in_dim), nullptr, ST_ACT_RELU, m1, d->P,
                                         nullptr, 0, &pre1, 0, nullptr, 0, 0, 0, 0, nullptr, 0, nullptr, d->B, d->P, stream);
    if (rc) return rc;
    st_t16_view next = {io->xq_tape + (size_t)(t + 1) * sv.q_floats, sv.q_kbs, 0};
    return st_skinny_linear_packed_fwd(io->packed + pl.p1, &pre1, 16 * kb16(d->P), nullptr, ST_ACT_RELU, m2, d->P,
                                       nullptr, 0, &next, 0, nullptr, 0, 0, 0, 0, nullptr, 0, nullptr, d->B, d->P, stream);
}

}

extern "C" int st_decoder_gate_split_k(const st_decoder_dims* d) {
    if (!d) return 0;
    const StepViews sv = step_views(d);
    int hosted = (sv.d_kbs / 2) / 16 * 16;
    if (hosted < 16 || hosted > sv.d_kbs - sv.d_ha) hosted = sv.d_kbs - sv.d_ha;
    return 16 * (sv.d_kbs - hosted);
}

extern "C" size_t st_decoder_packed_floats(const st_decoder_dims* d) { return d ? packed_layout(d).total : 0; }

extern "C" int st_decoder_pack(const st_decoder_weights* w, const st_decoder_dims* d, float* packed, void* stream) {
    (void)hipGetLastError();
    ST_CHECK_ARG(w && d && packed, "st_decoder_pack: null pointer");
    const PackedLayout pl = packed_layout(d);
    const int in_dim = d->r * d->n_mels;
    st_pack_job j[6];
    memset(j, 0, sizeof(j));
    auto seg = [&](st_pack_job& q, int s, const float* wp, int ld, int k) { q.w[s] = wp; q.ldw[s] = ld; q.k[s] = k; q.nseg = s + 1; };
    seg(j[0], 0, w->q_w_ih, d->P + d->E, d->P); seg(j[0], 1, w->q_w_ih + d->P, d->P + d->E, d->E); seg(j[0], 2, w->q_w_hh, d->Q, d->Q);
    j[0].N = 4 * d->Q; j[0].lstm_H = d->Q; j[0].packed = packed + pl.q;
    seg(j[1], 0, w->attn_query_w, d->Q, d->Q); j[1].N = d->A; j[1].packed = packed + pl.pq;
    seg(j[2], 0, w->d_w_ih, d->E + d->Q, d->E); seg(j[2], 1, w->d_w_ih + d->E, d->E + d->Q, d->Q); seg(j[2], 2, w->d_w_hh, d->D, d->D);
    j[2].N = 4 * d->D; j[2].lstm_H = d->D; j[2].packed = packed + pl.d;
    seg(j[3], 0, w->projgate_w, d->D + d->E, d->D); seg(j[3], 1, w->projgate_w + d->D, d->D + d->E, d->E);
    j[3].N = in_dim + 1 + (d->fuse_pre0 ? d->P : 0); j[3].packed = packed + pl.pg;
    seg(j[4], 0, w->prenet_w0, in_dim, in_dim); j[4].N = d->P; j[4].packed = packed + pl.p0;
    seg(j[5], 0, w->prenet_w1, d->P, d->P); j[5].N = d->P; j[5].packed = packed + pl.p1;
    return st_pack_weight_batch(j, 6, stream);
}

extern "C" size_t st_decoder_tape_floats(const st_decoder_dims* d, int which) {
    if (!d) return 0;
    const StepViews sv = step_views(d);
    return which == 0 ? sv.q_floats : (which == 1 ? sv.d_floats : sv.o_floats);
}

namespace {

enum FwdAttn {
    ATTN_WHOLE,
    ATTN_PRE_FIN,
    ATTN_FIN_SPLIT,
    ATTN_PQ_FIN,
    ATTN_PQ_RNG
};
enum FwdProd {
    PROD_NONE,
    PROD_OWN,
    PROD_PQ_FIN,
    PROD_PQ_PRE
};
struct FwdForms {
    bool pure_tf;
    bool defer;
    bool pre_in_pq;
    bool pair_cells;
    FwdAttn attn;
    FwdProd prod;
    int fin_parts;
    int pq_pre_parts;
    int d_k0;
};

FwdForms fwd_forms(const st_decoder_dims* d, const st_decoder_io* io, int cus, int rng_capacity) {
    FwdForms f;
    const int B = d->B, L = d->L, E = d->E, Q = d->Q, D = d->D, A = d->A, BT = (B + 15) / 16;
    f.pure_tf = io->teacher_pre && io->Bt == B && io->Tt > 0;
    for (int t = 0; t + 1 < io->steps && f.pure_tf; ++t) f.pure_tf = io->step_src[t] == (t < io->Tt ? t : io->Tt - 1);
    f.defer = io->defer_proj != 0;
    f.pair_cells = f.defer && f.pure_tf && io->pair_cells;
    const bool split_attn = io->attn_s_buf != nullptr;
    f.pre_in_pq = split_attn && f.defer;
    const int fp_req = io->attn_fin_parts;
    f.fin_parts = (fp_req == 2 || fp_req == 4 || fp_req == 8) && E % (4 * fp_req) == 0 ? fp_req : 1;
    const int sp = io->attn_split_parts;
    const bool fin_split = split_attn && io->attn_split_ws && sp >= 2 && sp <= 64 && A % 4 == 0 && A <= 256 && E % 4 == 0 &&
                           E / 4 <= 512 && 512 % (E / 4) == 0 && (L + sp - 1) / sp <= 512;
    const bool fin_rng = fin_split && !f.pre_in_pq && io->pq_granules && io->attn_xchg && sp <= 8 && A % 16 == 0 && E % (4 * sp) == 0 &&
                         E / sp <= 256 && (sp - 1) * ((L + sp - 1) / sp) < L && (A / 16) * BT + B * sp <= rng_capacity;
    const bool fuse_pq_fin = !fin_split && split_attn && !f.pre_in_pq && io->pq_granules && A % 16 == 0 && A <= 256 && E % 4 == 0 &&
                             (A / 16) * BT + B * f.fin_parts <= cus;
    f.attn = !split_attn ? ATTN_WHOLE : fin_rng ? ATTN_PQ_RNG : fin_split ? ATTN_FIN_SPLIT : fuse_pq_fin ? ATTN_PQ_FIN : ATTN_PRE_FIN;
    const bool split_d = io->gate_part && (!f.defer || f.pre_in_pq) && B > 16 && B <= 32 && D % 16 == 0 && (D / 4) % 2 == 0 &&
                         E % 16 == 0 && Q % 16 == 0 && st_aligned16(io->gate_part);
    const int pre_parts_split = io->attn_pre_parts > 2 ? 2 : io->attn_pre_parts;
    const bool split_pre = split_d && f.pre_in_pq && A <= 16 * 128 &&
                           ((A + 15) / 16) * BT + B * (pre_parts_split > 1 ? pre_parts_split : 1) + (4 * D) / 32 <= cus;
    f.pq_pre_parts = split_pre ? pre_parts_split : io->attn_pre_parts;
    if (!split_d) f.prod = PROD_NONE;
    else if (split_pre) f.prod = PROD_PQ_PRE;
    else if (fuse_pq_fin && (A / 16) * BT + B * f.fin_parts + (4 * D) / 32 <= cus) f.prod = PROD_PQ_FIN;
    else f.prod = PROD_OWN;
    f.d_k0 = (io->gate_part_k ? io->gate_part_k : st_decoder_gate_split_k(d)) / 16;
    return f;
}

}

int pk_attnrng_capacity();

extern "C" int st_decoder_fwd_forms(const st_decoder_dims* d, const st_decoder_io* io, int cus, int rng_capacity) {
    if (!d || !io || (io->steps > 1 && !io->step_src)) return -1;
    const FwdForms f = fwd_forms(d, io, cus > 0 ? cus : st_device_cus(), rng_capacity > 0 ? rng_capacity : pk_attnrng_capacity());
    return (int)f.attn | ((int)f.prod << 4) | (f.pure_tf ? 1 << 8 : 0) | (f.defer ? 1 << 9 : 0) | (f.pre_in_pq ? 1 << 10 : 0) |
           (f.pair_cells ? 1 << 11 : 0) | (f.fin_parts << 12) | ((f.prod != PROD_NONE ? f.d_k0 & 0xfff : 0) << 16);
}

static int decoder_forward_issue(const st_decoder_weights* w, const st_decoder_dims* d, const st_decoder_io* io, void* stream);

static stlg::Cache g_fwd_graphs;
extern "C" void st_loop_graph_stats(long* fwd3, long* bwd3);
extern "C" void stx_fwd_loop_graph_stats(long* out3) {
    std::lock_guard<std::mutex> lock(g_fwd_graphs.mu);
    out3[0] = g_fwd_graphs.replays; out3[1] = g_fwd_graphs.captures; out3[2] = g_fwd_graphs.eager;
}

extern "C" int st_decoder_forward(const st_decoder_weights* w, const st_decoder_dims* d, const st_decoder_io* io,
                                  void* stream) {
    (void)hipGetLastError();
    ST_CHECK_ARG(w && d && io, "st_decoder_forward: null struct pointer");
    if (io->defer_proj && io->steps > 0 && io->step_src && stlg::enabled(d->B)) {
        st_decoder_io key_io = *io;
        key_io.step_src = nullptr;
        uint64_t key = stlg::fnv(stlg::FNV0, w, sizeof(*w));
        key = stlg::fnv(key, d, sizeof(*d));
        key = stlg::fnv(key, &key_io, sizeof(key_io));
        key = stlg::fnv(key, io->step_src, sizeof(int) * (size_t)io->steps);
        stlg::Entry* e = nullptr;
        hipStream_t issue_on = (hipStream_t)stream;
        const int mode = stlg::begin(g_fwd_graphs, key, (hipStream_t)stream, &e, &issue_on);
        if (mode == 1) return 0;
        int rc = decoder_forward_issue(w, d, io, (void*)issue_on);
        if (mode == 2) {
            rc = stlg::end(g_fwd_graphs, e, (hipStream_t)stream, rc);
            if (rc == -5) st_set_error("st_decoder_forward: capturing the loop into a hipGraph failed");
        }
        return rc;
    }
    return decoder_forward_issue(w, d, io, stream);
}

static int decoder_forward_issue(const st_decoder_weights* w, const st_decoder_dims* d, const st_decoder_io* io, void* stream) {
    ST_CHECK_ARG(w && d && io, "st_decoder_forward: null struct pointer");
    const int B = d->B, L = d->L, E = d->E, P = d->P, Q = d->Q, D = d->D, A = d->A;
    const int steps = io->steps;
    const int in_dim = d->r * d->n_mels;
    ST_CHECK_ARG(B > 0 && L > 0 && steps > 0 && in_dim > 0, "st_decoder_forward: B=%d L=%d steps=%d", B, L, steps);
    ST_CHECK_ARG(io->memory && io->pm && io->ada_std && io->ada_mean && io->step_src && io->packed,
                 "st_decoder_forward: null input");
    ST_CHECK_ARG(io->mel_out && io->align_out && io->stop_out, "st_decoder_forward: null output");
    ST_CHECK_ARG(io->xq_tape && io->xd_tape && io->xo_tape && io->cq_tape && io->cd_tape && io->wcum_tape &&
                 io->pq_buf && io->pre1_t16 && io->mel_t16 && io->zero_row, "st_decoder_forward: null tape/scratch");
    ST_CHECK_ARG(d->prenet_norm >= 0 && d->prenet_norm <= 3 && (!d->prenet_norm || (!d->fuse_pre0 && io->pre_nat && w->pre_norm_w[0] &&
                 w->pre_norm_w[1] && w->pre_norm_b[0] && w->pre_norm_b[1])), "st_decoder_forward: normalised prenet needs pre_nat, the norm weights and fuse_pre0 = 0");
    for (int t = 0; t + 1 < steps; ++t) {
        const int src = io->step_src[t];
        ST_CHECK_ARG(!d->fuse_pre0 || src == -1, "st_decoder_forward: fuse_pre0 needs every next input to be the own output");
        ST_CHECK_ARG(src >= -2 && (src < 0 || (io->teacher_pre && src < io->Tt)), "st_decoder_forward: step_src[%d]=%d invalid", t, src);
        ST_CHECK_ARG(src != -2 || io->teacher_mean, "st_decoder_forward: step_src[%d]=-2 without teacher_mean", t);
        ST_CHECK_ARG(src == -1 || (io->Bt > 0 && io->Bt <= B), "st_decoder_forward: Bt=%d invalid", io->Bt);
    }
    const StepViews sv = step_views(d);
    ST_CHECK_ARG(io->gate_part_k == 0 || !io->gate_part || (io->gate_part_k % 16 == 0 && io->gate_part_k >= 16 * sv.d_ha && io->gate_part_k < 16 * sv.d_kbs),
                 "st_decoder_forward: gate_part_k = %d must be a multiple of 16 in [%d, %d)", io->gate_part_k, 16 * sv.d_ha, 16 * sv.d_kbs);
    FwdForms f = fwd_forms(d, io, st_device_cus(), pk_attnrng_capacity());
    ST_CHECK_ARG(!f.defer || (f.pure_tf && !d->fuse_pre0), "st_decoder_forward: defer_proj needs pure teacher forcing");
#ifdef ST_ABLATE
    const int skip = getenv("ST_SKIP") ? atoi(getenv("ST_SKIP")) : 0;
    if ((skip & 8) || (f.prod == PROD_PQ_FIN && (skip & 6)) || (f.prod == PROD_PQ_PRE && (skip & 2))) f.prod = PROD_NONE;
#define ST_SKIPPED(bit) (skip & (1 << (bit)))
#else
#define ST_SKIPPED(bit) 0
#endif
    hipStream_t st = (hipStream_t)stream;
    const PackedLayout pl = packed_layout(d);
    const size_t BQ = (size_t)B * Q, BD = (size_t)B * D, BL = (size_t)B * L;
    ZeroArgs za;
    memset(&za, 0, sizeof(za));
    auto zero = [&](void* p, size_t bytes) { za.p[za.n] = (float*)p; za.floats[za.n] = bytes / sizeof(float); ++za.n; };
    zero(io->cq_tape, BQ * sizeof(float));
    zero(io->cd_tape, BD * sizeof(float));
    zero(io->wcum_tape, BL * sizeof(float));
    zero(io->zero_row, BL * sizeof(float));
    zero(io->xq_tape, sv.q_floats * sizeof(float));
    zero(io->xd_tape, sv.d_floats * sizeof(float));
    if (io->attn_loc_tape) zero(io->attn_loc_tape, BL * d->F * sizeof(float));
    const int sp_parts = io->attn_split_parts;
    if (f.attn == ATTN_PQ_FIN || f.attn == ATTN_PQ_RNG) zero(io->pq_granules, (size_t)B * A * sizeof(unsigned long long));
    if (f.attn == ATTN_PQ_RNG) zero(io->attn_xchg, st_attn_rng_xchg_words(B, E, sp_parts) * sizeof(unsigned long long));
    {
        size_t most = 0;
        for (int i = 0; i < za.n; ++i) most = za.floats[i] > most ? za.floats[i] : most;
        size_t blocks = (most / 4 + 255) / 256 + 1;
        if (blocks > 256) blocks = 256;
        hipLaunchKernelGGL(zero_regions_kernel, dim3((unsigned)blocks, za.n), dim3(256), 0, st, za);
        ST_LAUNCH_CHECK();
    }
    if (io->dec_in0) {
        st_t16_view xq0 = {io->xq_tape, sv.q_kbs, 0};
        int rc0 = st_tile_rows(io->dec_in0, P, &xq0, B, P, stream);
        if (rc0) return rc0;
    }
    if (f.pure_tf && steps > 1) {
        const size_t total = (size_t)(steps - 1) * B * P;
        size_t blocks = (total + 255) / 256;
        if (blocks > 4096) blocks = 4096;
        hipLaunchKernelGGL(tile_teacher_kernel, dim3((unsigned)blocks), dim3(256), 0, st, io->teacher_pre, io->Tt, io->xq_tape,
                           sv.q_floats, sv.q_kbs, steps, B, P);
        ST_LAUNCH_CHECK();
    }

    const size_t ldmel = (size_t)steps * in_dim;
    const int ldal = steps * L;
    const int Kq = 16 * sv.q_kbs, Kd = 16 * sv.d_kbs, Ko = 16 * sv.o_kbs;
    st_partial_product_job pj_d;
    memset(&pj_d, 0, sizeof(pj_d));
    pj_d.packed_w = io->packed + pl.d; pj_d.w_kbs = sv.d_kbs; pj_d.kb0 = f.d_k0; pj_d.KB = sv.d_kbs - f.d_k0; pj_d.N = 4 * D; pj_d.part = io->gate_part;
    int rc = 0;
    for (int t = 0; t < steps; ++t) {
        float* xq = io->xq_tape + (size_t)t * sv.q_floats;
        float* xq_next = io->xq_tape + (size_t)(t + 1) * sv.q_floats;
        float* xd = io->xd_tape + (size_t)t * sv.d_floats;
        float* xd_next = io->xd_tape + (size_t)(t + 1) * sv.d_floats;
        float* xo = io->xo_tape + (size_t)t * sv.o_floats;
        pj_d.x = st_t16_view{xd, sv.d_kbs, f.d_k0};

        st_t16_view xq_v = {xq, sv.q_kbs, 0};
        st_t16_view hq_dst = {xq_next, sv.q_kbs, sv.q_h};
        st_t16_view ha_dst = {xd, sv.d_kbs, sv.d_ha};
        if (!(f.pair_cells && t > 0) && !ST_SKIPPED(0)) {
            rc = st_lstm_cell_packed_fwd(io->packed + pl.q, &xq_v, Kq, w->q_b_ih, w->q_b_hh,
                                         io->cq_tape + (size_t)t * BQ, Q, io->q_mask ? io->q_mask + (size_t)t * BQ : nullptr,
                                         &hq_dst, nullptr, io->cq_tape + (size_t)(t + 1) * BQ, Q,
                                         io->gates_q_tape ? io->gates_q_tape + (size_t)t * 4 * BQ : nullptr,
                                         io->ada_std, io->ada_mean, &ha_dst, B, Q, stream);
            if (rc) return rc;
        }

        if (f.attn != ATTN_PQ_FIN && f.attn != ATTN_PQ_RNG && !ST_SKIPPED(1)) {
            if (f.pre_in_pq && t > 0) {
                st_attn_pre_job job = {io->pm, io->align_out + (size_t)(t - 1) * L, ldal, io->wcum_tape + (size_t)t * BL,
                                       w->attn_loc_conv_w, w->attn_loc_lin_w, io->attn_s_buf + (size_t)t * io->attn_s_step_floats, L, A, d->F,
                                       d->K, f.pq_pre_parts, io->attn_loc_tape ? io->attn_loc_tape + (size_t)t * BL * d->F : nullptr};
                if (f.prod == PROD_PQ_PRE) job.part = &pj_d;
                rc = st_skinny_linear_packed_attnpre_fwd(io->packed + pl.pq, &hq_dst, 16 * kb16(Q), nullptr, ST_ACT_NONE, nullptr, 0,
                                                         io->pq_buf, A, nullptr, 0, nullptr, 0, 0, 0, 0, nullptr, 0, nullptr, B, A,
                                                         &job, stream);
            } else
                rc = st_skinny_linear_packed_fwd(io->packed + pl.pq, &hq_dst, 16 * kb16(Q), nullptr, ST_ACT_NONE, nullptr, 0,
                                                 io->pq_buf, A, nullptr, 0, nullptr, 0, 0, 0, 0, nullptr, 0, nullptr, B, A, stream);
            if (rc) return rc;
        }

        st_t16_view ctx_dst[3] = {{xq_next, sv.q_kbs, sv.q_ctx}, {xd, sv.d_kbs, 0}, {xo, sv.o_kbs, sv.o_ctx}};
        const float* s_t = t == 0 || f.attn == ATTN_WHOLE ? io->pm : io->attn_s_buf + (size_t)t * io->attn_s_step_floats;
        auto fin_job = [&](int parts) {
            st_attn_fin_job fj;
            memset(&fj, 0, sizeof(fj));
            fj.s_buf = s_t; fj.memory = io->memory; fj.w_cum_prev = io->wcum_tape + (size_t)t * BL;
            fj.w_out = io->align_out + (size_t)t * L; fj.ld_wout = ldal; fj.w_cum_out = io->wcum_tape + (size_t)(t + 1) * BL; fj.v = w->attn_v;
            for (int c = 0; c < 3; ++c) fj.ctx_dst[c] = ctx_dst[c];
            fj.status = io->handoff_status;
            fj.n_ctx_dst = 3; fj.parts = parts; fj.L = L; fj.A = A; fj.E = E; fj.F = d->F; fj.K = d->K;
            return fj;
        };
        switch (f.attn) {
        case ATTN_WHOLE:
            if (!ST_SKIPPED(2))
                rc = st_attn_step_t16_fwd(io->pq_buf, io->pm, io->memory, t == 0 ? io->zero_row : io->align_out + (size_t)(t - 1) * L,
                                          t == 0 ? L : ldal, io->wcum_tape + (size_t)t * BL, io->align_out + (size_t)t * L, ldal,
                                          io->wcum_tape + (size_t)(t + 1) * BL,
                                          w->attn_loc_conv_w, w->attn_loc_lin_w, w->attn_v, ctx_dst, 3, nullptr, 0,
                                          B, L, A, E, d->F, d->K, stream);
            break;
        case ATTN_PRE_FIN:
            if (!ST_SKIPPED(2))
                rc = st_attn_fin_t16_fwd(io->pq_buf, s_t, io->memory, io->wcum_tape + (size_t)t * BL,
                                         io->align_out + (size_t)t * L, ldal, io->wcum_tape + (size_t)(t + 1) * BL, w->attn_v,
                                         ctx_dst, 3, nullptr, 0, f.fin_parts, B, L, A, E, d->F, d->K, stream);
            break;
        case ATTN_FIN_SPLIT:
            if (!ST_SKIPPED(2))
                rc = st_attn_fin_split_fwd(io->pq_buf, s_t, io->memory, io->wcum_tape + (size_t)t * BL, io->align_out + (size_t)t * L, ldal,
                                           io->wcum_tape + (size_t)(t + 1) * BL, w->attn_v, ctx_dst, 3, nullptr, 0, io->attn_split_ws, sp_parts,
                                           B, L, A, E, stream);
            break;
        case ATTN_PQ_FIN:
            if (!(ST_SKIPPED(1) || ST_SKIPPED(2))) {
                const st_attn_fin_job fj = fin_job(f.fin_parts);
                rc = f.prod == PROD_PQ_FIN
                         ? st_query_attn_fin_part_fwd(io->packed + pl.pq, &hq_dst, 16 * kb16(Q), io->pq_granules, (unsigned)(t + 1), &fj, B, &pj_d, stream)
                         : st_query_attn_fin_fwd(io->packed + pl.pq, &hq_dst, 16 * kb16(Q), io->pq_granules, (unsigned)(t + 1), &fj, B, stream);
            }
            break;
        case ATTN_PQ_RNG:
            if (!(ST_SKIPPED(1) || ST_SKIPPED(2))) {
                const st_attn_fin_job fj = fin_job(sp_parts);
                rc = st_query_attn_rng_fwd(io->packed + pl.pq, &hq_dst, 16 * kb16(Q), io->pq_granules, io->attn_xchg, (unsigned)(t + 1), &fj, B, stream);
            }
            break;
        }
        if (rc) return rc;

        if (f.prod == PROD_OWN || (f.prod == PROD_PQ_PRE && t == 0)) {
            rc = st_partial_product_fwd(&pj_d, B, stream);
            if (rc) return rc;
        }
        st_t16_view xd_v = {xd, sv.d_kbs, 0};
        st_t16_view hd_dst0 = {xd_next, sv.d_kbs, sv.d_h};
        st_t16_view hd_dst1 = {xo, sv.o_kbs, 0};
        const bool part = f.prod != PROD_NONE;
        if (!ST_SKIPPED(3)) {
            if (f.pair_cells && t + 1 < steps) {
                st_lstm_cell_packed_job jd, jq;
                memset(&jd, 0, sizeof(jd)); memset(&jq, 0, sizeof(jq));
                jd.packed_w = io->packed + pl.d; jd.x = xd_v; jd.K = Kd; jd.b_ih = w->d_b_ih; jd.b_hh = w->d_b_hh;
                if (part) { jd.K = 16 * f.d_k0; jd.part = io->gate_part; jd.w_kbs = sv.d_kbs; }
                jd.c_prev = io->cd_tape + (size_t)t * BD; jd.ldc_prev = D; jd.mask = io->d_mask ? io->d_mask + (size_t)t * BD : nullptr;
                jd.h_dst0 = hd_dst0; jd.h_dst1 = hd_dst1; jd.c_out = io->cd_tape + (size_t)(t + 1) * BD; jd.ldc = D;
                jd.gates_out = io->gates_d_tape ? io->gates_d_tape + (size_t)t * 4 * BD : nullptr;
                jd.B = B; jd.H = D;
                float* xq_next2 = io->xq_tape + (size_t)(t + 2) * sv.q_floats;
                jq.packed_w = io->packed + pl.q; jq.x = st_t16_view{xq_next, sv.q_kbs, 0}; jq.K = Kq; jq.b_ih = w->q_b_ih; jq.b_hh = w->q_b_hh;
                jq.c_prev = io->cq_tape + (size_t)(t + 1) * BQ; jq.ldc_prev = Q; jq.mask = io->q_mask ? io->q_mask + (size_t)(t + 1) * BQ : nullptr;
                jq.h_dst0 = st_t16_view{xq_next2, sv.q_kbs, sv.q_h}; jq.c_out = io->cq_tape + (size_t)(t + 2) * BQ; jq.ldc = Q;
                jq.gates_out = io->gates_q_tape ? io->gates_q_tape + (size_t)(t + 1) * 4 * BQ : nullptr;
                jq.ada_std = io->ada_std; jq.ada_mean = io->ada_mean; jq.hadapt_dst = st_t16_view{xd_next, sv.d_kbs, sv.d_ha};
                jq.B = B; jq.H = Q;
                rc = st_lstm_cell_packed_pair_fwd(&jd, &jq, stream);
            } else if (part)
                rc = st_lstm_cell_packed_part_fwd(io->packed + pl.d, sv.d_kbs, &xd_v, 16 * f.d_k0, io->gate_part, w->d_b_ih, w->d_b_hh,
                                                  io->cd_tape + (size_t)t * BD, D, io->d_mask ? io->d_mask + (size_t)t * BD : nullptr,
                                                  &hd_dst0, &hd_dst1, io->cd_tape + (size_t)(t + 1) * BD, D,
                                                  io->gates_d_tape ? io->gates_d_tape + (size_t)t * 4 * BD : nullptr, B, D, stream);
            else
                rc = st_lstm_cell_packed_fwd(io->packed + pl.d, &xd_v, Kd, w->d_b_ih, w->d_b_hh,
                                             io->cd_tape + (size_t)t * BD, D, io->d_mask ? io->d_mask + (size_t)t * BD : nullptr,
                                             &hd_dst0, &hd_dst1, io->cd_tape + (size_t)(t + 1) * BD, D,
                                             io->gates_d_tape ? io->gates_d_tape + (size_t)t * 4 * BD : nullptr,
                                             nullptr, nullptr, nullptr, B, D, stream);
            if (rc) return rc;
        }

        st_t16_view xo_v = {xo, sv.o_kbs, 0};
        st_t16_view mel_dst = {io->mel_t16, kb16(in_dim), 0};
        st_t16_view pre1_dst = {io->pre1_t16 + (size_t)t * io->pre1_step_floats, kb16(P), 0};
        const bool fuse = d->fuse_pre0 != 0;
        if (f.defer) continue;
        const bool split_attn = f.attn != ATTN_WHOLE;
        st_attn_pre_job job = {io->pm, io->align_out + (size_t)t * L, ldal, io->wcum_tape + (size_t)(t + 1) * BL,
                               w->attn_loc_conv_w, w->attn_loc_lin_w,
                               split_attn ? io->attn_s_buf + (size_t)(t + 1) * io->attn_s_step_floats : nullptr, L, A, d->F, d->K,
                               io->attn_pre_parts, io->attn_loc_tape ? io->attn_loc_tape + (size_t)(t + 1) * BL * d->F : nullptr};
        if (!ST_SKIPPED(4)) {
            rc = st_skinny_linear_packed_attnpre_fwd(io->packed + pl.pg, &xo_v, ST_SKIPPED(7) ? Ko / 4 : Ko, w->projgate_b, ST_ACT_NONE, nullptr, 0,
                                                     io->mel_out + (size_t)t * in_dim, (int)ldmel, fuse ? nullptr : &mel_dst, in_dim,
                                                     io->stop_out + (size_t)t * d->r, steps * d->r, d->r,
                                                     fuse ? in_dim + 1 : 0, ST_ACT_RELU,
                                                     io->prenet_mask ? io->prenet_mask + (size_t)t * 2 * B * P : nullptr, P,
                                                     fuse ? &pre1_dst : nullptr, B, in_dim + 1 + (fuse ? P : 0),
                                                     split_attn && t + 1 < steps && !ST_SKIPPED(6) ? &job : nullptr, stream);
            if (rc) return rc;
        }

        if (t + 1 < steps) {
            const int src = io->step_src[t];
            st_t16_view next = {xq_next, sv.q_kbs, 0};
            if ((src == -1 || io->Bt < B) && !ST_SKIPPED(5)) {
                rc = prenet_own(w, d, io, pl, sv, t, fuse, stream);
                if (rc) return rc;
            }
            if (!f.pure_tf && src >= 0) rc = st_tile_rows(io->teacher_pre + (size_t)src * P, io->Tt * P, &next, io->Bt, P, stream);
            else if (!f.pure_tf && src == -2) rc = st_tile_rows(io->teacher_mean, P, &next, io->Bt, P, stream);
            if (rc) return rc;
        } else if (d->prenet_norm == 3 && (io->step_src[t] == -1 || io->Bt < B)) {
            rc = prenet_own(w, d, io, pl, sv, t, false, stream);
            if (rc) return rc;
        }
    }
    return 0;
}
```

semi_tts_amd/csrc/skinny_packed.hip:

```cpp
#include "st_common.h"
#include "attention_body.h"
#include "attention_bwd_body.h"
#include <cstdlib>

#ifndef PK_PROF
#define PK_PROF(n)
#endif
#ifndef RT2_PROF
#define RT2_PROF(n)
#endif

namespace {

constexpr int PK_MAXSEG = 3;

__host__ __device__ inline int pk_kb(int k) { return (k + 15) >> 4; }

struct PackArgs {
    const float* w[PK_MAXSEG]; int ldw[PK_MAXSEG]; int k[PK_MAXSEG]; int kb0[PK_MAXSEG];
    int nseg; int N; int H; int KB; int tiles; float* out;
};

__device__ __forceinline__ void pack_weight_body(const PackArgs& a);
__global__ __launch_bounds__(256) void pack_weight_kernel(const PackArgs a) { pack_weight_body(a); }
// ... 812 lines not shown
    if (exp_ == 2 && i >= n_ab) return;
    if (i < n_ab) {
        if (KW * 64 > AB_THREADS && (int)threadIdx.x >= AB_THREADS) return;
        const int part = i / ab.B;
        ab_body<true, LBLK, NS>(ab, i - part * ab.B, pk_dyn_lds, part);
        return;
    }
    pk_part_body<KW, TRIP>(p, i - n_ab, red);
}

template <int KW, int TRIP>
__global__ __launch_bounds__(KW * 64) void pk_part_hist_kernel(const PkPartArgs p, const int n_h, const AbHistArgs hist) {
    extern __shared__ __attribute__((aligned(16))) float pk_dyn_lds[];
    __shared__ f32x4 red[KW * 4 * 64];
    const int i = blockIdx.x;
    if (i < n_h) { ab_hist_body(hist, i, pk_dyn_lds); return; }
    pk_part_body<KW, TRIP>(p, i - n_h, red);
}

template <int KW, int TRIP>
__global__ __launch_bounds__(KW * 64) void pk_part_kernel(const PkPartArgs p) {
    __shared__ f32x4 red[KW * 4 * 64];
    pk_part_body<KW, TRIP>(p, blockIdx.x, red);
}

template <int KW, int TRIP, int LBLK, int NS>
__global__ __launch_bounds__(2 * KW * 64) void pk_pw_ab_dual_kernel(const f32x4* w, const f32x4* x, const int w_kbs, const int x_kbs, const int KB,
                                                                    const int B, const int N, const int n_ab,
                                                                    const PkArgs rest, const PkPw pw, const AbArgs ab, const int exp_) {
    extern __shared__ __attribute__((aligned(16))) float pk_dyn_lds[];
    __shared__ f32x4 red[2 * KW * 64];
    static_assert(KW * 64 == AB_THREADS, "both parts use 512-thread bodies");
    const int i = blockIdx.x;
    const int half = __builtin_amdgcn_readfirstlane((int)threadIdx.x / (KW * 64));
    if (exp_ == 1 && i < n_ab) return;
    if (exp_ == 2 && i >= n_ab) return;
    if (i < n_ab) {
        if (half) return;
        const int part = i / ab.B;
        ab_body<true, LBLK, NS>(ab, i - part * ab.B, pk_dyn_lds, part);
        return;
    }
    PkArgs a = rest;
    a.w = w; a.x = x; a.w_kbs = w_kbs; a.x_kbs = x_kbs; a.KB = KB; a.B = B; a.N = N; a.H = 0;
    pk_body<2, 1, KW, TRIP>(a, i - n_ab, half, red + half * KW * 64, &pw, half * KW * 64);
}

template <int MODE, int NB, int KW, int TRIP>
__global__ __launch_bounds__(KW * 64) void pk_pw_hist_kernel(const f32x4* w, const f32x4* x, const int w_kbs, const int x_kbs, const int KB,
                                                             const int B, const int N, const int tiles_a, const int n_h, const int n_sum,
                                                             const PkArgs rest, const PkPw pw, const AbHistArgs hist, const PkSumArgs sum, const int exp_) {
    extern __shared__ __attribute__((aligned(16))) float pk_dyn_lds[];
    __shared__ f32x4 red[KW * NB * 64];
    const int i = blockIdx.x;
    if (exp_ == 3 && i < n_h) return;
    if (exp_ == 4 && i >= n_h && i < n_h + n_sum) return;
    if (exp_ == 5 && i >= n_h + n_sum) return;
    if (i < n_h) { ab_hist_body(hist, i, pk_dyn_lds); return; }
    if (i < n_h + n_sum) { pk_sum_body(sum, i - n_h, KW * 64); return; }
    PkArgs a = rest;
    a.w = w; a.x = x; a.w_kbs = w_kbs; a.x_kbs = x_kbs; a.KB = KB; a.B = B; a.N = N; a.H = 0;
    const int j = i - n_h - n_sum;
    const int by = j / tiles_a;
    pk_body<MODE, NB, KW, TRIP>(a, j - by * tiles_a, by, red, MODE == 2 ? &pw : nullptr);
}

template <int NB, int KW, int TRIP, bool VEC>
__global__ __launch_bounds__(KW * 64) void pk_attnpre_kernel(const f32x4* w, const f32x4* x, const int w_kbs, const int x_kbs, const int KB,
                                                             const int B, const int N, const int tiles_a, const int n_lin,
                                                             const float* at_pm, const float* at_wprev, const int at_L,
                                                             const PkArgs a_rest, const AtArgs t_rest) {
    extern __shared__ __attribute__((aligned(16))) float pk_dyn_lds[];
    __shared__ f32x4 red[KW * NB * 64];
    PkArgs a = a_rest;
    a.w = w; a.x = x; a.w_kbs = w_kbs; a.x_kbs = x_kbs; a.KB = KB; a.B = B; a.N = N;
    AtArgs t = t_rest;
    t.pm = at_pm; t.w_prev = at_wprev; t.L = at_L;
    static_assert(KW * 64 == AT_THREADS, "both parts use 512-thread workgroups");
    const int i = blockIdx.x;
    if (i < n_lin) {
        const int by = n_lin <= 2 * tiles_a ? (i >= tiles_a ? 1 : 0) : i / tiles_a;
        pk_body<1, NB, KW, TRIP>(a, i - by * tiles_a, by, red);
    }
    else at_body<VEC, 1>(t, i - n_lin, pk_dyn_lds);
}

template <int NB, int KW, int TRIP, bool VEC>
__global__ __launch_bounds__(KW * 64) void pk_attnpre_part_kernel(const f32x4* w, const f32x4* x, const int w_kbs, const int x_kbs, const int KB,
                                                                  const int B, const int N, const int tiles_a, const int n_lin,
                                                                  const float* at_pm, const float* at_wprev, const int at_L,
                                                                  const PkArgs a_rest, const AtArgs t_rest, const int n_at, const PkPartArgs p) {
    extern __shared__ __attribute__((aligned(16))) float pk_dyn_lds[];
    __shared__ f32x4 red[KW * NB * 64];
    static_assert(KW * 64 == AT_THREADS, "both parts use 512-thread workgroups");
    const int i = blockIdx.x;
    if (i < n_lin) {
        PkArgs a = a_rest;
        a.w = w; a.x = x; a.w_kbs = w_kbs; a.x_kbs = x_kbs; a.KB = KB; a.B = B; a.N = N;
        const int by = n_lin <= 2 * tiles_a ? (i >= tiles_a ? 1 : 0) : i / tiles_a;
        pk_body<1, NB, KW, TRIP>(a, i - by * tiles_a, by, red);
    } else if (i < n_lin + n_at) {
        AtArgs t = t_rest;
        t.pm = at_pm; t.w_prev = at_wprev; t.L = at_L;
        at_body<VEC, 1>(t, i - n_lin, pk_dyn_lds);
    } else pk_part_body<KW, 2>(p, i - n_lin - n_at, reinterpret_cast<f32x4*>(pk_dyn_lds));
}


template <int NB, int KW, int TRIP>
__global__ __launch_bounds__(KW * 64) void pk_attnfin_kernel(const f32x4* w, const f32x4* x, const int w_kbs, const int x_kbs, const int KB,
                                                             const int B, const int N, const int tiles_a, const int n_lin,
                                                             const PkArgs a_rest, const AtArgs t) {
    extern __shared__ __attribute__((aligned(16))) float pk_dyn_lds[];
    __shared__ f32x4 red[KW * NB * 64];
    static_assert(KW * 64 == AT_THREADS, "both parts use 512-thread workgroups");
    const int i = blockIdx.x;
    if (i < n_lin) {
        PkArgs a = a_rest;
        a.w = w; a.x = x; a.w_kbs = w_kbs; a.x_kbs = x_kbs; a.KB = KB; a.B = B; a.N = N;
        const int by = n_lin <= 2 * tiles_a ? (i >= tiles_a ? 1 : 0) : i / tiles_a;
        pk_body<1, NB, KW, TRIP>(a, i - by * tiles_a, by, red);
    }
    else at_body<true, 2, AT_THREADS, true>(t, i - n_lin, pk_dyn_lds);
}

template <int NB, int KW, int TRIP>
__global__ __launch_bounds__(KW * 64) void pk_attnfin_part_kernel(const f32x4* w, const f32x4* x, const int w_kbs, const int x_kbs, const int KB,
                                                                  const int B, const int N, const int tiles_a, const int n_lin,
                                                                  const PkArgs a_rest, const AtArgs t, const int n_att, const PkPartArgs p) {
    extern __shared__ __attribute__((aligned(16))) float pk_dyn_lds[];
    __shared__ f32x4 red[KW * NB * 64];
    static_assert(KW * 64 == AT_THREADS, "both parts use 512-thread workgroups");
    const int i = blockIdx.x;
    if (i < n_lin) {
        PkArgs a = a_rest;
        a.w = w; a.x = x; a.w_kbs = w_kbs; a.x_kbs = x_kbs; a.KB = KB; a.B = B; a.N = N;
        const int by = n_lin <= 2 * tiles_a ? (i >= tiles_a ? 1 : 0) : i / tiles_a;
        pk_body<1, NB, KW, TRIP>(a, i - by * tiles_a, by, red);
    }
    else if (i < n_att) at_body<true, 2, AT_THREADS, true>(t, i - n_lin, pk_dyn_lds);
    else pk_part_body<KW, 2>(p, i - n_att, reinterpret_cast<f32x4*>(pk_dyn_lds));
}

template <int NB, int KW, int TRIP>
__global__ __launch_bounds__(KW * 64, 4) void pk_attnrng_kernel(const f32x4* w, const f32x4* x, const int w_kbs, const int x_kbs, const int KB,
                                                                const int B, const int N, const int tiles_a, const int n_lin,
                                                                const PkArgs a_rest, const ArArgs t) {
    __shared__ f32x4 red[KW * NB * 64];
    static_assert(KW * 64 == AT_THREADS, "both parts use 512-thread workgroups");
    const int i = blockIdx.x;
    if (i < n_lin) {
        PkArgs a = a_rest;
        a.w = w; a.x = x; a.w_kbs = w_kbs; a.x_kbs = x_kbs; a.KB = KB; a.B = B; a.N = N;
        const int by = n_lin <= 2 * tiles_a ? (i >= tiles_a ? 1 : 0) : i / tiles_a;
        pk_body<1, NB, KW, TRIP>(a, i - by * tiles_a, by, red);
    }
    else at_range_body<AT_THREADS>(t, i - n_lin);
}

#ifndef PK_TRIP_SMALL
#define PK_TRIP_SMALL 2
#endif
int pk_fill(PkArgs& a, const float* packed_w, const st_t16_view* x, int K, const char* who);

template <int NB>
int pk_launch_attnpre(const PkArgs& a, int tiles, const AtArgs& t, hipStream_t st, const PkPartArgs* pp = nullptr) {
    constexpr int KW = 8, TRIP = NB == 1 ? PK_TRIP_SMALL : 2;
    const int BT = (a.B + 15) >> 4, gy = (BT + NB - 1) / NB;
    if constexpr (NB == 1) if (pp) {
        const bool vec = (t.A % 4 == 0) && (t.F % 4 == 0) && st_aligned16(t.pm) && st_aligned16(t.loc_lin_w) && st_aligned16(t.s_buf);
        const AtLds o = at_layout(t.L, t.A, t.E, t.F, t.K, 1, at_pos_per(t.L, t.pre_parts > 1 ? t.pre_parts : 1), vec && t.F == 32 && t.A % 16 == 0);
        size_t lds = (size_t)o.total * sizeof(float);
        if (lds < sizeof(f32x4) * KW * 4 * 64) lds = sizeof(f32x4) * KW * 4 * 64;
        ST_CHECK_ARG(lds + sizeof(f32x4) * KW * NB * 64 <= 160 * 1024, "linear + attention-pre launch: L=%d needs too much LDS (use more parts)", t.L);
        auto kern = vec ? pk_attnpre_part_kernel<NB, KW, TRIP, true> : pk_attnpre_part_kernel<NB, KW, TRIP, false>;
        static size_t configured[2] = {0, 0};
        if (lds > 32 * 1024 && lds > configured[vec ? 1 : 0]) {
            ST_HIP(hipFuncSetAttribute(reinterpret_cast<const void*>(kern), hipFuncAttributeMaxDynamicSharedMemorySize, (int)lds));
            configured[vec ? 1 : 0] = lds;
        }
        const int n_at = t.B * (t.pre_parts > 1 ? t.pre_parts : 1);
        hipLaunchKernelGGL(kern, dim3(tiles * gy + n_at + (pp->N >> 5)), dim3(KW * 64), lds, st, a.w, a.x, a.w_kbs, a.x_kbs,
                           a.KB, a.B, a.N, tiles, tiles * gy, t.pm, t.w_prev, t.L, a, t, n_at, *pp);
        ST_LAUNCH_CHECK();
        return 0;
    }
    const bool vec = (t.A % 4 == 0) && (t.F % 4 == 0) && st_aligned16(t.pm) && st_aligned16(t.loc_lin_w) && st_aligned16(t.s_buf);
    const AtLds o = at_layout(t.L, t.A, t.E, t.F, t.K, 1, at_pos_per(t.L, t.pre_parts > 1 ? t.pre_parts : 1), vec && t.F == 32 && t.A % 16 == 0);
    const size_t lds = (size_t)o.total * sizeof(float);
    ST_CHECK_ARG(lds + sizeof(f32x4) * KW * NB * 64 <= 160 * 1024, "linear + attention-pre launch: L=%d needs too much LDS (use more parts)", t.L);
    auto kern = vec ? pk_attnpre_kernel<NB, KW, TRIP, true> : pk_attnpre_kernel<NB, KW, TRIP, false>;
    static size_t configured[2] = {0, 0};
    if (lds > 48 * 1024 && lds > configured[vec ? 1 : 0]) {
        ST_HIP(hipFuncSetAttribute(reinterpret_cast<const void*>(kern), hipFuncAttributeMaxDynamicSharedMemorySize, (int)lds));
        configured[vec ? 1 : 0] = lds;
    }
    hipLaunchKernelGGL(kern, dim3(tiles * gy + t.B * (t.pre_parts > 1 ? t.pre_parts : 1)), dim3(KW * 64), lds, st, a.w, a.x, a.w_kbs, a.x_kbs,
                       a.KB, a.B, a.N, tiles, tiles * gy, t.pm, t.w_prev, t.L, a, t);
    ST_LAUNCH_CHECK();
    return 0;
}

template <int MODE, int NB>
int pk_launch(const PkArgs& a, int tiles, hipStream_t st) {
    constexpr int KW = 8, TRIP = (MODE == 1 && NB == 1) ? PK_TRIP_SMALL : 2;
    const int BT = (a.B + 15) >> 4;
    dim3 grid(tiles, (BT + NB - 1) / NB);
    hipLaunchKernelGGL((pk_kernel<MODE, NB, KW, TRIP>), grid, dim3(KW * 64), 0, st, a.w, a.x, a.w_kbs, a.x_kbs, a.KB, a.B, a.N, a.H, a);
    ST_LAUNCH_CHECK();
    return 0;
}

#ifndef PK_LSTM_KW
#define PK_LSTM_KW 8
#endif
#ifndef PK_LSTM_TRIP
#define PK_LSTM_TRIP 2
#endif
inline bool pk_rt2_shape(int B, int tiles) {
    const int BT = (B + 15) >> 4;
    return (tiles & 1) == 0 && (BT == 2 || BT == 4) && B > 16 * (BT - 1);
}

template <int MODE>
int pk_dispatch(const PkArgs& a, int tiles, hipStream_t st) {
    const int BT = (a.B + 15) >> 4;
    if (MODE == 0 && pk_rt2_shape(a.B, tiles)) {
        constexpr int LKW = PK_LSTM_KW, LTR = PK_LSTM_TRIP;
#if defined(PK_AUX_Q0) || defined(PK_AUX_D0)
        if (BT == 2 && a.KB > 128)
            hipLaunchKernelGGL((pk_lstm_rt2_kernel<LKW, LTR, 1, PK_AUX_D0, PK_AUX_D1>), dim3(tiles / 2, 2), dim3(LKW * 64), 0, st, a.w, a.x, a.w_kbs, a.x_kbs, a.KB, a.B, a.H, a);
        else if (BT == 2)
            hipLaunchKernelGGL((pk_lstm_rt2_kernel<LKW, LTR, 1, PK_AUX_Q0, PK_AUX_Q1>), dim3(tiles / 2, 2), dim3(LKW * 64), 0, st, a.w, a.x, a.w_kbs, a.x_kbs, a.KB, a.B, a.H, a);
        else
#endif
        if (BT == 2)
            hipLaunchKernelGGL((pk_lstm_rt2_kernel<LKW, LTR, 1>), dim3(tiles / 2, 2), dim3(LKW * 64), 0, st, a.w, a.x, a.w_kbs, a.x_kbs, a.KB, a.B, a.H, a);
#ifdef PK_C5_NB4
        else if (getenv("ST_C5_NB4"))
            hipLaunchKernelGGL((pk_lstm_rt2_kernel<LKW, LTR, 4>), dim3(tiles / 2, 1), dim3(LKW * 64), 0, st, a.w, a.x, a.w_kbs, a.x_kbs, a.KB, a.B, a.H, a);
#endif
        else
            hipLaunchKernelGGL((pk_lstm_rt2_kernel<LKW, LTR, 2>), dim3(tiles / 2, 2), dim3(LKW * 64), 0, st, a.w, a.x, a.w_kbs, a.x_kbs, a.KB, a.B, a.H, a);
        ST_LAUNCH_CHECK();
        return 0;
    }
    if (MODE == 1 && BT > 1) {
        int nb = 1;
        while (nb < 4 && tiles * ((BT + nb - 1) / nb) > 512) ++nb;
        if (nb == 1) return pk_launch<MODE, 1>(a, tiles, st);
        if (nb == 2) return pk_launch<MODE, 2>(a, tiles, st);
        if (nb == 3) return pk_launch<MODE, 3>(a, tiles, st);
        return pk_launch<MODE, 4>(a, tiles, st);
    }
    if (BT == 1) return pk_launch<MODE, 1>(a, tiles, st);
    if (BT == 2) return pk_launch<MODE, 2>(a, tiles, st);
    if (BT == 3) return pk_launch<MODE, 3>(a, tiles, st);
    return pk_launch<MODE, 4>(a, tiles, st);
}

PkOut pk_out(const st_t16_view* v) {
    PkOut o = {nullptr, 0, 0};
    if (v && v->base) { o.base = v->base; o.kb_stride = v->kb_stride; o.kb0 = v->kb0; }
    return o;
}

int pk_fill(PkArgs& a, const float* packed_w, const st_t16_view* x, int K, const char* who) {
    ST_CHECK_ARG(packed_w && x && x->base && K > 0, "%s: bad packed operands", who);
    ST_CHECK_ARG(st_aligned16(packed_w) && st_aligned16(x->base), "%s: operands must be 16-byte aligned", who);
    ST_CHECK_ARG(x->kb0 >= 0 && x->kb0 + pk_kb(K) <= x->kb_stride, "%s: k-block range [%d,%d) outside the T16 buffer (%d)",
                 who, x->kb0, x->kb0 + pk_kb(K), x->kb_stride);
    a.w = reinterpret_cast<const f32x4*>(packed_w);
// ... 153 lines not shown
                                       float* c_out, int ldc, float* gates_out,
                                       const float* ada_std, const float* ada_mean, const st_t16_view* hadapt_dst,
                                       int B, int H, void* stream) {
    return lstm_cell_packed_impl(packed_w, x, K, b_ih, b_hh, c_prev, ldc_prev, mask, h_dst0, h_dst1, c_out, ldc, gates_out, ada_std, ada_mean,
                                 hadapt_dst, B, H, 0, nullptr, stream);
}

extern "C" int st_lstm_cell_packed_part_fwd(const float* packed_w, int w_kbs, const st_t16_view* x, int K, const float* part,
                                            const float* b_ih, const float* b_hh,
                                            const float* c_prev, int ldc_prev, const float* mask,
                                            const st_t16_view* h_dst0, const st_t16_view* h_dst1,
                                            float* c_out, int ldc, float* gates_out, int B, int H, void* stream) {
    ST_CHECK_ARG(part, "st_lstm_cell_packed_part_fwd: null slab");
    return lstm_cell_packed_impl(packed_w, x, K, b_ih, b_hh, c_prev, ldc_prev, mask, h_dst0, h_dst1, c_out, ldc, gates_out, nullptr, nullptr,
                                 nullptr, B, H, w_kbs, part, stream);
}

static int pk_lstm_fill(PkArgs& a, const st_lstm_cell_packed_job* j, const char* who) {
    ST_CHECK_ARG(j && j->B > 0 && j->H > 0 && j->H % 4 == 0 && j->c_out && j->h_dst0.base, "%s: bad arguments", who);
    memset(&a, 0, sizeof(a));
    int rc = pk_fill(a, j->packed_w, &j->x, j->K, who);
    if (rc) return rc;
    a.B = j->B; a.N = 4 * j->H; a.H = j->H;
    a.b_ih = j->b_ih; a.b_hh = j->b_hh;
    a.c_prev = j->c_prev; a.ldc_prev = j->ldc_prev; a.mask = j->mask;
    a.c_out = j->c_out; a.ldc = j->ldc; a.gates_out = j->gates_out;
    a.h_dst[0] = pk_out(&j->h_dst0); a.h_dst[1] = pk_out(&j->h_dst1);
    a.ada_std = j->ada_std; a.ada_mean = j->ada_mean; a.ha_dst = pk_out(&j->hadapt_dst);
    if (j->part) {
        ST_CHECK_ARG(pk_rt2_shape(j->B, j->H / 4) && ((j->B + 15) >> 4) == 2 && j->w_kbs >= a.KB && st_aligned16(j->part),
                     "%s: a slab needs B = 17..32, an even number of row tiles, w_kbs >= K / 16 and 16-byte alignment", who);
        a.part = j->part; a.w_kbs = j->w_kbs;
    }
    return 0;
}

extern "C" int st_lstm_cell_packed_pair_fwd(const st_lstm_cell_packed_job* j0, const st_lstm_cell_packed_job* j1, void* stream) {
    (void)hipGetLastError();
    PkArgs a0, a1;
    int rc = pk_lstm_fill(a0, j0, "st_lstm_cell_packed_pair_fwd");
    if (rc) return rc;
    rc = pk_lstm_fill(a1, j1, "st_lstm_cell_packed_pair_fwd");
    if (rc) return rc;
    const int t0 = a0.H / 4, t1 = a1.H / 4;
    const bool pair = pk_rt2_shape(a0.B, t0) && pk_rt2_shape(a1.B, t1) && ((a0.B + 15) >> 4) == 2 && ((a1.B + 15) >> 4) == 2 &&
                      a0.H % 8 == 0 && a1.H % 8 == 0;
    if (!pair) {
        rc = pk_dispatch<0>(a0, t0, (hipStream_t)stream);
        if (rc) return rc;
        return pk_dispatch<0>(a1, t1, (hipStream_t)stream);
    }
    hipLaunchKernelGGL((pk_lstm_rt2_pair_kernel<PK_LSTM_KW, PK_LSTM_TRIP>), dim3(t0 + t1), dim3(PK_LSTM_KW * 64), 0, (hipStream_t)stream, t0, a0, a1);
    ST_LAUNCH_CHECK();
    return 0;
}

static int pk_linear_impl(const float* packed_w, const st_t16_view* x, int K,
                          const float* bias, int act, const float* mask, int ldmask,
                          float* y, int ldy, const st_t16_view* y_dst,
                          int n_split, float* y2, int ldy2, int rep,
                          int n_split2, int act2, const float* mask2, int ldmask2,
                          const st_t16_view* y3_dst,
                          int B, int N, const st_attn_pre_job* pre, void* stream) {
    ST_CHECK_ARG(n_split2 <= 0 || (y3_dst && y3_dst->base && n_split2 >= n_split), "st_skinny_linear_packed_fwd: third range");
    ST_CHECK_ARG(B > 0 && N > 0 && (y || (y_dst && y_dst->base)), "st_skinny_linear_packed_fwd: bad arguments");
    ST_CHECK_ARG(n_split <= 0 || (y2 && rep >= 1), "st_skinny_linear_packed_fwd: n_split without y2/rep");
    PkArgs a;
    memset(&a, 0, sizeof(a));
    int rc = pk_fill(a, packed_w, x, K, "st_skinny_linear_packed_fwd");
    if (rc) return rc;
    a.B = B; a.N = N; a.H = 0;
    a.bias = bias; a.act = act; a.lmask = mask; a.ldmask = ldmask;
    a.y = y; a.ldy = ldy; a.y_dst = pk_out(y_dst);
    a.n_split = n_split; a.y2 = y2; a.ldy2 = ldy2; a.rep = rep;
    a.n_split2 = n_split2; a.act2 = act2; a.mask2 = mask2; a.ldmask2 = ldmask2; a.y3_dst = pk_out(y3_dst);
    const int tiles = (N + 15) / 16;
    if (pre && pre->s_buf) {
        ST_CHECK_ARG(pre->pm && pre->w_prev && pre->w_cum_prev && pre->loc_conv_w && pre->loc_lin_w && pre->L > 0 && pre->A > 0 &&
                     pre->F > 0 && pre->K > 0 && (pre->K & 1), "st_skinny_linear_packed_attnpre_fwd: bad attention job");
        AtArgs t;
        memset(&t, 0, sizeof(t));
        t.pm = pre->pm; t.w_prev = pre->w_prev; t.ld_wprev = pre->ld_wprev; t.w_cum_prev = pre->w_cum_prev;
        t.loc_conv_w = pre->loc_conv_w; t.loc_lin_w = pre->loc_lin_w; t.s_buf = pre->s_buf; t.cf_out = pre->cf_out;
        t.B = B; t.L = pre->L; t.A = pre->A; t.E = 4; t.F = pre->F; t.K = pre->K;
        t.pre_parts = (pre->parts >= 2 && pre->parts <= 64 && (pre->parts & (pre->parts - 1)) == 0) ? pre->parts : 1;
        const int BT = (B + 15) >> 4;
        if (pre->part) {
            const st_partial_product_job* pj = pre->part;
            ST_CHECK_ARG(pj->packed_w && pj->x.base && pj->part && pj->KB > 0 && pj->kb0 >= 0 && pj->kb0 + pj->KB <= pj->w_kbs &&
                         pj->x.kb0 + pj->KB <= pj->x.kb_stride && B > 16 && B <= 32 && pj->N > 0 && pj->N % 32 == 0 && st_aligned16(pj->packed_w) &&
                         st_aligned16(pj->x.base) && st_aligned16(pj->part) && tiles <= 128,
                         "st_skinny_linear_packed_attnpre_fwd: bad partial product (B = 17..32, N %% 32 == 0, a linear of at most 128 row tiles)");
            PkPartArgs pp;
            memset(&pp, 0, sizeof(pp));
            pp.w = reinterpret_cast<const f32x4*>(pj->packed_w) + (size_t)pj->kb0 * 64; pp.w_kbs = pj->w_kbs;
            pp.x = reinterpret_cast<const f32x4*>(pj->x.base) + (size_t)pj->x.kb0 * 64; pp.x_kbs = pj->x.kb_stride;
            pp.KB = pj->KB; pp.S = 1; pp.B = B; pp.N = pj->N; pp.part = pj->part;
            return pk_launch_attnpre<1>(a, tiles, t, (hipStream_t)stream, &pp);
        }
        if (BT == 1 || tiles <= 128) return pk_launch_attnpre<1>(a, tiles, t, (hipStream_t)stream);
        if (BT == 2) return pk_launch_attnpre<2>(a, tiles, t, (hipStream_t)stream);
        if (BT == 3) return pk_launch_attnpre<3>(a, tiles, t, (hipStream_t)stream);
        return pk_launch_attnpre<4>(a, tiles, t, (hipStream_t)stream);
    }
    return pk_dispatch<1>(a, tiles, (hipStream_t)stream);
}

static int query_attn_fin_impl(const float* packed_wq, const st_t16_view* h_q, int Q, unsigned long long* granules, unsigned epoch,
                               const st_attn_fin_job* job, int B, const st_partial_product_job* pj, void* stream) {
    (void)hipGetLastError();
    ST_CHECK_ARG(packed_wq && h_q && h_q->base && granules && epoch != 0 && job && B > 0, "st_query_attn_fin_fwd: bad arguments");
    const int L = job->L, A = job->A, E = job->E, parts = job->parts;
    ST_CHECK_ARG(L > 0 && E > 0 && A > 0 && A % 16 == 0 && A <= 256, "st_query_attn_fin_fwd: attention dim %d must be a multiple of 16, at most 256", A);
    ST_CHECK_ARG(parts == 1 || ((parts == 2 || parts == 4 || parts == 8) && E % (4 * parts) == 0), "st_query_attn_fin_fwd: parts=%d, E=%d", parts, E);
    ST_CHECK_ARG(job->s_buf && job->memory && job->w_cum_prev && job->w_out && job->w_cum_out && job->v, "st_query_attn_fin_fwd: null attention operand");
    ST_CHECK_ARG(job->n_ctx_dst >= 0 && job->n_ctx_dst <= 3, "st_query_attn_fin_fwd: n_ctx_dst=%d", job->n_ctx_dst);
    ST_CHECK_ARG(st_aligned16(job->s_buf) && st_aligned16(job->memory) && st_aligned16(job->v) && (reinterpret_cast<uintptr_t>(granules) & 7) == 0 &&
                 E % 4 == 0 && E / 4 <= AT_THREADS, "st_query_attn_fin_fwd: operands must be 16-byte aligned, E a multiple of 4");
    PkArgs a;
    memset(&a, 0, sizeof(a));
    int rc = pk_fill(a, packed_wq, h_q, Q, "st_query_attn_fin_fwd");
    if (rc) return rc;
    a.B = B; a.N = A; a.H = 0; a.act = ST_ACT_NONE;
    a.gran = granules; a.epoch = epoch;
    AtArgs t;
    memset(&t, 0, sizeof(t));
    t.pm = job->s_buf; t.s_buf = const_cast<float*>(job->s_buf); t.memory = job->memory; t.w_cum_prev = job->w_cum_prev;
    t.w_out = job->w_out; t.ld_wout = job->ld_wout; t.w_cum_out = job->w_cum_out; t.v = job->v; t.loc_lin_w = job->s_buf;
    t.fin_parts = parts;
    for (int d = 0; d < job->n_ctx_dst; ++d) t.ctx_dst[d] = job->ctx_dst[d];
    t.B = B; t.L = L; t.A = A; t.E = E; t.F = job->F; t.K = job->K;
    t.pq_gran = granules; t.epoch = epoch; t.status = job->status;
    const int tiles = A / 16, BT = (B + 15) >> 4;
    const int n_lin = tiles * BT, n_fin = B * parts;
    ST_CHECK_ARG(n_lin + n_fin <= st_device_cus(), "st_query_attn_fin_fwd: %d + %d workgroups do not fit the device at once (use the two launches)",
                 n_lin, n_fin);
    const AtLds o = at_layout(L, A, E, job->F, job->K, 2, L, false);
    size_t lds = (size_t)o.total * sizeof(float);
    constexpr int KW = 8;
    ST_CHECK_ARG(lds + sizeof(f32x4) * KW * 64 <= 160 * 1024, "st_query_attn_fin_fwd: L=%d needs too much LDS", L);
    if (pj) {
        ST_CHECK_ARG(pj->packed_w && pj->x.base && pj->part && pj->KB > 0 && pj->kb0 >= 0 && pj->kb0 + pj->KB <= pj->w_kbs &&
                     pj->x.kb0 + pj->KB <= pj->x.kb_stride && B > 16 && B <= 32 && pj->N > 0 && pj->N % 32 == 0 && st_aligned16(pj->packed_w) &&
                     st_aligned16(pj->x.base) && st_aligned16(pj->part), "st_query_attn_fin_part_fwd: bad partial product (B = 17..32, N %% 32 == 0)");
        const int n_part = pj->N >> 5;
        ST_CHECK_ARG(n_lin + n_fin + n_part <= st_device_cus(), "st_query_attn_fin_part_fwd: %d + %d + %d workgroups do not fit the device at once",
                     n_lin, n_fin, n_part);
        PkPartArgs pp;
        memset(&pp, 0, sizeof(pp));
        pp.w = reinterpret_cast<const f32x4*>(pj->packed_w) + (size_t)pj->kb0 * 64; pp.w_kbs = pj->w_kbs;
        pp.x = reinterpret_cast<const f32x4*>(pj->x.base) + (size_t)pj->x.kb0 * 64; pp.x_kbs = pj->x.kb_stride;
        pp.KB = pj->KB; pp.S = 1; pp.B = B; pp.N = pj->N; pp.part = pj->part;
        if (lds < sizeof(f32x4) * KW * 4 * 64) lds = sizeof(f32x4) * KW * 4 * 64;
        auto kernp = pk_attnfin_part_kernel<1, KW, PK_TRIP_SMALL>;
        static size_t configured_p = 0;
        if (lds > 48 * 1024 && lds > configured_p) {
            ST_HIP(hipFuncSetAttribute(reinterpret_cast<const void*>(kernp), hipFuncAttributeMaxDynamicSharedMemorySize, (int)lds));
            configured_p = lds;
        }
        hipLaunchKernelGGL(kernp, dim3(n_lin + n_fin + n_part), dim3(KW * 64), lds, (hipStream_t)stream, a.w, a.x, a.w_kbs, a.x_kbs, a.KB, a.B, a.N,
                           tiles, n_lin, a, t, n_lin + n_fin, pp);
        ST_LAUNCH_CHECK();
        return 0;
    }
    auto kern = pk_attnfin_kernel<1, KW, PK_TRIP_SMALL>;
    static size_t configured = 0;
// ... 429 lines not shown
```

semi_tts_amd/module.py:

```python
import ctypes as C

import numpy as np
import os
import torch
import torch.nn as nn

from . import ops
from . import _lib
from . import autograd as AG
from ._lib import StDecoderWeights, StDecoderDims, StDecoderIO, check


_ONES = {}


def _scaled_mask(shape, p, device):
    n = int(torch.Size(shape).numel())
    key = (str(device), n)
    ones = _ONES.get(key)
    if ones is None:
        if len(_ONES) > 64:
            _ONES.clear()
        ones = _ONES[key] = torch.ones(n, device=device, dtype=torch.float32)
    return torch.nn.functional.dropout(ones, p, training=True).view(shape)
# ... 205 lines not shown
        ctx = torch.empty(B, E, device=memory.device, dtype=torch.float32)
        wc, wl = self.location_weights()
        ops.attn_step(pq, processed_memory, memory, w_prev, w_cum, w, w_cum_new, wc.detach().contiguous(), wl.detach().contiguous(),
                      self.v.linear.weight, ctx)
        return ctx, w


def plan_decode(teacher_is_int, teacher_frames, teacher_bs, B, r, tf_rate, drop_dec_in, unpair_max_frame,
                coin=None):
    coin = coin or np.random.rand
    inference = tf_rate == 0.0
    partial = (not teacher_is_int) and B != teacher_bs
    if inference:
        steps = teacher_frames // r if teacher_is_int else teacher_frames
        t_groups = None
    else:
        assert not teacher_is_int, 'teacher forcing needs a teacher tensor'
        t_groups = teacher_frames // r
        if partial:
            assert unpair_max_frame is not None
            steps = max(t_groups, unpair_max_frame // r)
        else:
            steps = t_groups
    src = []
    for t in range(steps):
        if inference or (coin() > tf_rate):
            src.append(-1)
        elif coin() < drop_dec_in:
            src.append(-2)
        else:
            src.append(min(t, t_groups - 1))
    return steps, src


class Decoder(nn.Module):

    def __init__(self, n_mels, n_frames_per_step, enc_embed_dim, spkr_embed_dim, prenet_dim, prenet_dropout,
                 query_rnn_dim, dec_rnn_dim, query_dropout, dec_dropout, attn_dim, n_location_filters,
                 location_kernel_size, loc_aware, use_summed_weights, drop_dec_in, prenet_norm_type=None,
                 pretrain=False, spkr_embed_mode='adaIN'):
        super().__init__()
        self.n_mels = n_mels
        self.n_frames_per_step = n_frames_per_step
        self.enc_embed_dim = enc_embed_dim
        self.spkr_embed_dim = spkr_embed_dim
        self.query_rnn_dim = query_rnn_dim
        self.dec_rnn_dim = dec_rnn_dim
        self.prenet_dropout = prenet_dropout
        self.prenet_dim = prenet_dim
        self.query_dropout = nn.Dropout(query_dropout)
        self.dec_dropout = nn.Dropout(dec_dropout)
        self.attn_dim = attn_dim
        self.n_location_filters = n_location_filters
        self.location_kernel_size = location_kernel_size
        self.pretrain = pretrain
        self.loc_aware = loc_aware
        self.use_summed_weights = use_summed_weights
        self.drop_dec_in = drop_dec_in
        self.prenet_norm_type = prenet_norm_type
        self.spkr_embed_mode = spkr_embed_mode.lower()
        if self.spkr_embed_mode == 'adain':
            self.pseudo_latent_mean = nn.Linear(spkr_embed_dim, query_rnn_dim)
            self.pseudo_latent_std = nn.Sequential(nn.Linear(spkr_embed_dim, query_rnn_dim), nn.ReLU())
        elif self.spkr_embed_mode == 'concat':
            self.spkr_mem_proj = nn.Linear(spkr_embed_dim + enc_embed_dim, enc_embed_dim)
        elif self.spkr_embed_mode == 'add':
            self.spkr_proj = nn.Linear(spkr_embed_dim, enc_embed_dim)
            self.spkr_mem_proj = nn.Linear(enc_embed_dim, enc_embed_dim)
        else:
            raise NotImplementedError
        self.prenet = Prenet(n_mels * n_frames_per_step, [prenet_dim, prenet_dim], apply_dropout=prenet_dropout,
                             norm_type=prenet_norm_type)
        self.query_rnn = nn.LSTMCell(prenet_dim + enc_embed_dim, query_rnn_dim)
        self.attn = Attention(query_rnn_dim, enc_embed_dim, attn_dim, n_location_filters, location_kernel_size,
                              loc_aware, use_summed_weights)
        self.dec_rnn = nn.LSTMCell(query_rnn_dim + enc_embed_dim, dec_rnn_dim)
        self.proj = Linear(dec_rnn_dim + enc_embed_dim, n_mels * n_frames_per_step)
        self.gate_layer = Linear(dec_rnn_dim + enc_embed_dim, 1, bias=True, w_init_gain='sigmoid')
        self.last_tapes = None
        self.fuse_prenet = True
        self.cache_packed = False
        self.attn_split = True
        self.attn_pre_parts = 4
        self.attn_fin_parts = 2
        self.attn_pq_in_fin = True
        self.split_gates = os.environ.get('ST_SPLIT_GATES', '1') != '0'
        self.split_cell_k = int(os.environ.get('ST_SPLIT_CELL_K', '0'))
        self.split_gates_train = os.environ.get('ST_SPLIT_GATES_TRAIN', '1') != '0'
        self.check_handoff = True
        self.handoff_status = None
        self.attn_split_min_len = 128
        self.attn_split_positions = 43
        self.bwd_fuse_pointwise = True
        self.bwd_overlap_attn = True
        self.bwd_dxq_splits = int(os.environ.get('ST_DXQ_SPLITS', '4'))
        self.bwd_dxd_splits = int(os.environ.get('ST_DXD_SPLITS', '2'))
        self.bwd_attn_parts = int(os.environ.get('ST_ATTN_PARTS', '2'))
        self._last_fwd_forms = None
        self._last_bwd_forms = None
        self.fwd_pair_cells = True
        self.attn_rng_one_launch = True

    def gate_split_k(self):
        if self.split_cell_k:
            return int(self.split_cell_k)
        import ctypes as C
        from . import _lib
        d = StDecoderDims(B=32, L=1, E=self.enc_embed_dim, n_mels=self.n_mels, r=self.n_frames_per_step, P=self.prenet_dim,
                          Q=self.query_rnn_dim, D=self.dec_rnn_dim, A=1)
        return int(_lib.load().st_decoder_gate_split_k(C.byref(d)))

    def _weights_struct(self, keep, fuse_pre0=False):
        w = StDecoderWeights()
        pw, gw = self.proj.linear.weight, self.gate_layer.linear.weight
        in_dim, KO = pw.shape
        n_rows = in_dim + 1 + (self.prenet_dim if fuse_pre0 else 0)
        if not fuse_pre0 and not ops.capturing():
            pg_w = ops.cat_params([pw.detach(), gw.detach()])
            pg_b = ops.cat_params([self.proj.linear.bias.detach(), self.gate_layer.linear.bias.detach()])
        else:
            pg_w = torch.empty(n_rows, KO, device=pw.device, dtype=torch.float32)
            pg_b = torch.empty(n_rows, device=pw.device, dtype=torch.float32)
            ops.copy2d(pg_w, pw, in_dim, KO)
            ops.copy2d(pg_w[in_dim:], gw, 1, KO)
            ops.copy2d(pg_b.view(1, -1), self.proj.linear.bias.view(1, -1), 1, in_dim)
            ops.copy2d(pg_b.view(1, -1)[:, in_dim:], self.gate_layer.linear.bias.view(1, -1), 1, 1)
        if fuse_pre0:
            w0 = self.prenet.layers[0].linear.weight
            pwT = pw.detach().t().contiguous()
            ops.gemm(w0, pwT, out=pg_w[in_dim + 1:])
            ops.gemm(w0, self.proj.linear.bias.view(1, -1), out=pg_b[in_dim + 1:].view(-1, 1))
            keep.append(pwT)
        loc_wc, loc_wl = (t.detach().contiguous() for t in self.attn.location_weights())
        keep += [loc_wc, loc_wl]
        keep += [pg_w, pg_b]
        tensors = dict(
            prenet_w0=self.prenet.layers[0].linear.weight, prenet_w1=self.prenet.layers[1].linear.weight,
            q_w_ih=self.query_rnn.weight_ih, q_w_hh=self.query_rnn.weight_hh,
            q_b_ih=self.query_rnn.bias_ih, q_b_hh=self.query_rnn.bias_hh,
            attn_query_w=self.attn.query_layer.linear.weight, attn_v=self.attn.v.linear.weight,
            attn_loc_conv_w=loc_wc, attn_loc_lin_w=loc_wl,
            d_w_ih=self.dec_rnn.weight_ih, d_w_hh=self.dec_rnn.weight_hh,
            d_b_ih=self.dec_rnn.bias_ih, d_b_hh=self.dec_rnn.bias_hh, projgate_w=pg_w, projgate_b=pg_b)
        for k, t in tensors.items():
            setattr(w, k, ops._p(t))
        if self.prenet_norm_type is not None:
            for l, layer in enumerate(self.prenet.layers):
                nm = layer.norm
                w.pre_norm_w[l], w.pre_norm_b[l] = ops._p(nm.weight), ops._p(nm.bias)
                if self.prenet_norm_type == 'BatchNorm1d':
                    w.pre_norm_rm[l], w.pre_norm_rv[l] = ops._p(nm.running_mean), ops._p(nm.running_var)
                    w.pre_norm_nbt[l] = ops._p(nm.num_batches_tracked, torch.int64)
                    w.pre_norm_momentum = float(nm.momentum)
                w.pre_norm_eps = float(nm.eps)
        return w

    def forward(self, memory, memory_lengths, teacher, spkr_embed, tf_rate=0.0, unpair_max_frame=None, _masks=None):
        assert len(self.prenet.layers) == 2
        dev = memory.device
        memory = memory.contiguous()
        spkr_embed = spkr_embed.contiguous()
        B, L, E = memory.shape
        r, n_mels, P = self.n_frames_per_step, self.n_mels, self.prenet_dim
        Q, D, A = self.query_rnn_dim, self.dec_rnn_dim, self.attn_dim
        _masks = _masks or {}
        is_int = isinstance(teacher, int)
# ... 90 lines not shown
        for k, n in sizes.items():
            tapes[k] = tiled[off:off + n]
            off += n
        tapes.update(cq=torch.empty(steps + 1, B, Q, **f32), cd=torch.empty(steps + 1, B, D, **f32),
                     wcum=torch.empty(steps + 1, B, L, **f32), pq=torch.empty(B, A, **f32),
                     zero=torch.empty(B, L, **f32), tiled=tiled)
        if keep_tapes:
            tapes['gates_q'] = torch.empty(steps, B, 4, Q, **f32)
            tapes['gates_d'] = torch.empty(steps, B, 4, D, **f32)

        cache = self.__dict__.setdefault('_packed_cache', {}) if (self.cache_packed and not self.training) else None
        ckey = (bool(fuse_pre0), str(dev), tuple(p._version for p in self.parameters())) if cache is not None else None
        if cache is not None and ckey not in cache:
            cache.clear()
        if cache is not None and ckey in cache:
            w, keep_w, packed = cache[ckey]
            keep.append(keep_w)
        else:
            w = self._weights_struct(keep, fuse_pre0)
            packed = torch.empty(int(lib.st_decoder_packed_floats(C.byref(dims))), **f32)
            check(lib.st_decoder_pack(C.byref(w), C.byref(dims), ops._p(packed), ops.stream_handle()), 'st_decoder_pack')
            if cache is not None:
                cache[ckey] = (w, list(keep), packed)
        io = StDecoderIO()
        src_arr = (C.c_int * max(steps, 1))(*step_src)
        io.memory, io.pm, io.ada_std, io.ada_mean = ops._p(memory), ops._p(pm), ops._p(ada_std), ops._p(ada_mean)
        io.step_src = C.cast(src_arr, C.POINTER(C.c_int))
        io.teacher_pre, io.teacher_mean = ops._p(teacher_pre), ops._p(teacher_mean)
        io.Bt, io.Tt = Bt, Tt
        io.prenet_mask, io.q_mask, io.d_mask = ops._p(own_mask), ops._p(q_mask), ops._p(d_mask)
        io.steps = steps
        io.mel_out, io.align_out, io.stop_out = ops._p(mel), ops._p(align), ops._p(stop)
        io.packed = ops._p(packed)
        io.xq_tape, io.xd_tape, io.xo_tape = (ops._p(tapes[k]) for k in ('xq', 'xd', 'xo'))
        io.cq_tape, io.cd_tape, io.wcum_tape = (ops._p(tapes[k]) for k in ('cq', 'cd', 'wcum'))
        io.pq_buf, io.pre1_t16, io.mel_t16 = (ops._p(tapes[k]) for k in ('pq', 'pre1', 'melt'))
        io.zero_row = ops._p(tapes['zero'])
        if pn_mode:
            tapes['pre_nat'] = torch.empty(B, P, **f32)
            io.pre_nat = ops._p(tapes['pre_nat'])
            tapes['pn_mode'] = pn_mode
            if keep_tapes:
                tapes['pre_y'] = torch.empty(steps, 2, B, P, **f32)
                io.pre_nat_tape = ops._p(tapes['pre_y'])
        if plan.get('dec_in0') is not None:
            io.dec_in0 = ops._p(plan['dec_in0'])
        io.gates_q_tape, io.gates_d_tape = ops._p(tapes.get('gates_q')), ops._p(tapes.get('gates_d'))
        io.pre1_step_floats = t16(P) if keep_tapes else 0
        pure_tf = teacher_pre is not None and Bt == B and all(step_src[t] == min(t, Tt - 1) for t in range(steps - 1))
        defer = bool(keep_tapes and pure_tf)
        io.defer_proj = 1 if defer else 0
        io.pair_cells = 1 if (defer and self.fwd_pair_cells) else 0
        if self.attn_split and (not self.training or defer):
            if keep_tapes:
                tapes['attn_s'] = ops.uninit(steps, B, L, A, **f32)
                tapes['attn_loc'] = ops.uninit(steps, B, L, self.n_location_filters, **f32)
                io.attn_s_step_floats = B * L * A
                io.attn_loc_tape = ops._p(tapes['attn_loc'])
            else:
                tapes['attn_s'] = torch.empty(B, L, A, **f32)
            io.attn_s_buf = ops._p(tapes['attn_s'])
            parts = int(self.attn_pre_parts)
            while parts < 64 and (L + parts - 1) // parts > 512:
                parts *= 2
            io.attn_pre_parts = parts
            io.attn_fin_parts = int(self.attn_fin_parts)
            if L >= self.attn_split_min_len and not keep_tapes:
                sp = max(2, min(64, (L + self.attn_split_positions - 1) // self.attn_split_positions))
                tapes['attn_split_ws'] = torch.empty(int(lib.st_attn_fin_split_workspace_floats(B, E, sp)), **f32)
                io.attn_split_ws, io.attn_split_parts = ops._p(tapes['attn_split_ws']), sp
                if self.attn_pq_in_fin and sp <= 8 and self.attn_rng_one_launch:
                    tapes['attn_xchg'] = torch.empty(2 * int(lib.st_attn_rng_xchg_words(B, E, sp)), **f32)
                    io.attn_xchg = ops._p(tapes['attn_xchg'])
            if self.split_gates and 16 < B <= 32 and ((not keep_tapes and L < self.attn_split_min_len) or (defer and self.split_gates_train)):
                tapes['gate_part'] = torch.empty(B, 4 * D, **f32)
                io.gate_part = ops._p(tapes['gate_part'])
                io.gate_part_k = int(self.split_cell_k)
            if self.attn_pq_in_fin and not keep_tapes:
                tapes['pq_gran'] = torch.empty(B, 2 * A, **f32)
                io.pq_granules = ops._p(tapes['pq_gran'])
                if self.handoff_status is None or self.handoff_status.device != dev:
                    self.handoff_status = torch.zeros(1, device=dev, dtype=torch.int32)
                io.handoff_status = ops._p(self.handoff_status, torch.int32)
        self._last_fwd_forms = int(lib.st_decoder_fwd_forms(C.byref(dims), C.byref(io), 0, 0))
        check(lib.st_decoder_forward(C.byref(w), C.byref(dims), C.byref(io), ops.stream_handle()),
              'st_decoder_forward')
        if io.handoff_status and self.check_handoff and not ops.capturing():
            if ops.handoff_starved(self.handoff_status):
                ops.degrade('decode loop (query projection -> attention hand-off)', 'one launch each (attn_pq_in_fin = False)')
                self.attn_pq_in_fin = False
                io.pq_granules, io.handoff_status, io.attn_xchg = None, None, None
                self._last_fwd_forms = int(lib.st_decoder_fwd_forms(C.byref(dims), C.byref(io), 0, 0))
                check(lib.st_decoder_forward(C.byref(w), C.byref(dims), C.byref(io), ops.stream_handle()), 'st_decoder_forward')
        if not keep_tapes and self.check_handoff and not ops.capturing():
            ops.check_persist_status(dev)
        if defer:
            kb = ops.kb16
            Bp = ((B + 15) // 16) * 16
            xo_nat = ops.untile_tape(tapes['xo'], steps, Bp, kb(D) + kb(E), [(0, D), (kb(D), E)])
            y = ops.gemm(xo_nat.view(-1, D + E), keep[-2], bias=keep[-1]).view(steps, Bp, in_dim + 1)
            check(lib.st_decoder_unpack_out(ops._p(y), ops._p(mel), ops._p(stop), B, Bp, steps, r, n_mels, in_dim + 1, ops.stream_handle()),
                  'st_decoder_unpack_out')
            tapes['xo_nat'] = xo_nat
        tapes['packed'] = packed
        tapes.update(pm=pm, ada_std=ada_std, ada_mean=ada_mean, teacher_pre=teacher_pre, masks=(own_mask, q_mask, d_mask),
                     keep=keep, step_src=step_src, slot=slot)
        return mel, align, stop, tapes


class BatchNormConv1d(nn.Module):

    def __init__(self, in_size, out_size, kernel_size, stride, padding, activation=None):
        super().__init__()
        assert stride == 1
        self.conv1d = nn.Conv1d(in_size, out_size, kernel_size=kernel_size, stride=stride, padding=padding, bias=False)
        self.bn = nn.BatchNorm1d(out_size, momentum=0.99, eps=1e-3)
        self.activation = activation
        self.padding = padding

    def forward(self, x_cl, training=None, Tout=None, out=None, coff=0, pool_prev=False, stats_Tout=None, collect=None):
        order = 'relu_bn' if self.activation is not None else 'bn'
        return _conv_bn_act(x_cl, self.conv1d.weight, None, self.bn, self.padding, self.bn.eps, self.bn.momentum,
                            order, self.training if training is None else training, Tout, out, coff, pool_prev,
                            stats_Tout, collect)


class Highway(nn.Module):

    def __init__(self, in_size, out_size):
        super().__init__()
        self.H = nn.Linear(in_size, out_size)
        self.H.bias.data.zero_()
        self.T = nn.Linear(in_size, out_size)
        self.T.bias.data.fill_(-1)

    def forward(self, x):
        if self.training:
            return AG.highway_layer(x, self.H.weight, self.H.bias, self.T.weight, self.T.bias)
        h = ops.gemm(x, self.H.weight, bias=self.H.bias, act_pre='relu')
        return ops.gemm(x, self.T.weight, bias=self.T.bias, act_pre='sigmoid', highway_h=h, res=x)


class CBHG(nn.Module):

    def __init__(self, in_dim, K=16, hidden_sizes=(128, 128)):
        super().__init__()
        hidden_sizes = list(hidden_sizes)
        self.in_dim = in_dim
        relu = nn.ReLU()
        self.conv1d_banks = nn.ModuleList([BatchNormConv1d(in_dim, in_dim, kernel_size=k, stride=1, padding=k // 2,
                                                           activation=relu) for k in range(1, K + 1)])
        in_sizes = [K * in_dim] + hidden_sizes[:-1]
        acts = [relu] * (len(hidden_sizes) - 1) + [None]
        self.conv1d_projs = nn.ModuleList([BatchNormConv1d(i, o, kernel_size=3, stride=1, padding=1, activation=a)
                                           for i, o, a in zip(in_sizes, hidden_sizes, acts)])
        self.pre_highway_proj = nn.Linear(hidden_sizes[-1], in_dim, bias=False)
        self.highways = nn.ModuleList([Highway(in_dim, in_dim) for _ in range(4)])
        self.gru = nn.GRU(in_dim, in_dim, num_layers=1, batch_first=True, bidirectional=True)

    def forward(self, inputs, input_lengths=None):
        assert input_lengths is None, 'the reference never passes lengths to the postnet CBHG'
        x = inputs.contiguous()
        B, T, Cn = x.shape
        assert Cn == self.in_dim
        K = len(self.conv1d_banks)
        if self.training:
            return self._forward_train(x)
# ... 80 lines not shown
```

semi_tts_amd/ops.py:

```python
import os
import ctypes as C
from contextlib import contextmanager

import numpy as np
import torch

from . import _lib
from ._lib import StSeg, StGemmEpilogue, check

ACT = {None: 0, 'none': 0, 'relu': 1, 'tanh': 2, 'sigmoid': 3}

POISON_UNINIT = False


def uninit(*shape, device, dtype=torch.float32):
    t = torch.empty(*shape, device=device, dtype=dtype)
    if POISON_UNINIT:
        t.fill_(float('nan'))
    return t

_stream_override = None


def zeros(*shape, device, dtype=torch.float32):
# ... 88 lines not shown
    for ev in _SIDE_PENDING:
        torch.cuda.current_stream().wait_event(ev)


def _p(t, dtype=torch.float32):
    if t is None:
        return None
    if not t.is_cuda:
        raise RuntimeError('semi_tts_amd: the HIP path needs device tensors (got a CPU tensor); there is no CPU fallback')
    if t.dtype != dtype:
        raise RuntimeError('semi_tts_amd: expected %s, got %s' % (dtype, t.dtype))
    return t.data_ptr()


def _seg(x, w, k=None, ldx=None, ldw=None):
    s = StSeg()
    s.x, s.w = _p(x), _p(w)
    s.k = int(k if k is not None else w.shape[-1])
    s.ldx = int(ldx if ldx is not None else x.stride(-2) if x.dim() > 1 else s.k)
    s.ldw = int(ldw if ldw is not None else w.stride(-2) if w.dim() > 1 else s.k)
    return s


def _segs(pairs):
    arr = (StSeg * len(pairs))()
    for i, s in enumerate(pairs):
        arr[i] = s
    return arr


def lstm_cell(segs, b_ih, b_hh, c_prev, h_out, c_out, mask=None, pre=None, ldpre=0, gates_out=None,
              ldh=None, ldc=None, ldc_prev=None):
    lib = _lib.load()
    B, H = h_out.shape[0], h_out.shape[-1]
    arr = _segs(segs)
    check(lib.st_lstm_cell_fwd(arr, len(segs), _p(b_ih), _p(b_hh), _p(pre), int(ldpre),
                               _p(c_prev), int(ldc_prev if ldc_prev is not None else (c_prev.stride(0) if c_prev is not None else H)),
                               _p(mask), _p(h_out), int(ldh if ldh is not None else h_out.stride(0)),
                               _p(c_out), int(ldc if ldc is not None else c_out.stride(0)),
                               _p(gates_out), B, H, stream_handle()), 'st_lstm_cell_fwd')


seg = _seg


def skinny_linear(segs, y, bias=None, act=None, mask=None, n_split=0, y2=None, rep=0, N=None):
    lib = _lib.load()
    B = y.shape[0]
    N = int(N if N is not None else y.shape[-1])
    arr = _segs(segs)
    check(lib.st_skinny_linear_fwd(arr, len(segs), _p(bias), ACT[act], _p(mask), int(mask.stride(0)) if mask is not None else 0,
                                   _p(y), int(y.stride(0)), int(n_split), _p(y2), int(y2.stride(0)) if y2 is not None else 0,
                                   int(rep), B, N, stream_handle()), 'st_skinny_linear_fwd')
    return y


def linear_small(x, w, bias=None, act=None, mask=None, out=None):
    if out is None:
        out = torch.empty(x.shape[0], w.shape[0], device=x.device, dtype=torch.float32)
    return skinny_linear([_seg(x, w)], out, bias, act, mask)


def attn_step(pq, pm, memory, w_prev, w_cum_prev, w_out, w_cum_out, loc_conv_w, loc_lin_w, v, ctx,
              h_q=None, ada_std=None, ada_mean=None, h_adapt=None):
    lib = _lib.load()
    B, L, E = memory.shape
    A = pm.shape[-1]
    F_, _, K = loc_conv_w.shape
    Q = h_q.shape[-1] if h_q is not None else 0
    check(lib.st_attn_step_fwd(_p(pq), _p(pm), _p(memory), _p(w_prev), int(w_prev.stride(0)), _p(w_cum_prev),
                               _p(w_out), int(w_out.stride(0)), _p(w_cum_out), _p(loc_conv_w), _p(loc_lin_w), _p(v),
                               _p(ctx), int(ctx.stride(0)), _p(h_q), int(h_q.stride(0)) if h_q is not None else 0,
                               _p(ada_std), _p(ada_mean), _p(h_adapt), Q, B, L, A, E, F_, K, stream_handle()),
          'st_attn_step_fwd')


def attn_pre(pm, w_prev, w_cum_prev, loc_conv_w, loc_lin_w, s_buf=None, parts=1):
    B, L, A = pm.shape
    F_, _, K = loc_conv_w.shape
    if s_buf is None:
        s_buf = torch.empty(B, L, A, device=pm.device, dtype=torch.float32)
    check(_lib.load().st_attn_pre_fwd(_p(pm), _p(w_prev), int(w_prev.stride(0)), _p(w_cum_prev), _p(loc_conv_w), _p(loc_lin_w),
                                      _p(s_buf), int(parts), B, L, A, F_, K, stream_handle()), 'st_attn_pre_fwd')
    return s_buf


def attn_fin(pq, s_buf, memory, w_cum_prev, v, w_out, w_cum_out, ctx, F_, K, parts=1):
    B, L, E = memory.shape
    A = s_buf.shape[-1]
    check(_lib.load().st_attn_fin_t16_fwd(_p(pq), _p(s_buf), _p(memory), _p(w_cum_prev), _p(w_out), int(w_out.stride(0)),
                                          _p(w_cum_out), _p(v), None, 0, _p(ctx), int(ctx.stride(0)), int(parts), B, L, A, E, int(F_), int(K),
                                          stream_handle()), 'st_attn_fin_t16_fwd')


def attn_fin_split(pq, s_buf, memory, w_cum_prev, v, w_out, w_cum_out, ctx, parts):
    lib = _lib.load()
    B, L, E = memory.shape
    A = s_buf.shape[-1]
    ws = torch.empty(int(lib.st_attn_fin_split_workspace_floats(B, E, int(parts))), device=memory.device, dtype=torch.float32)
    check(lib.st_attn_fin_split_fwd(_p(pq), _p(s_buf), _p(memory), _p(w_cum_prev), _p(w_out), int(w_out.stride(0)), _p(w_cum_out), _p(v),
                                    None, 0, _p(ctx), int(ctx.stride(0)), _p(ws), int(parts), B, L, A, E, stream_handle()),
          'st_attn_fin_split_fwd')


def query_attn_fin(packed_wq, h_q_t16, Q, s_buf, memory, w_cum_prev, v, w_out, w_cum_out, ctx_t16, F_, K, parts=2, epoch=1, granules=None):
    B, L, E = memory.shape
    A = s_buf.shape[-1]
    if granules is None:
        granules = torch.zeros(B, 2 * A, device=memory.device, dtype=torch.float32)
    job = _lib.StAttnFinJob()
    job.s_buf, job.memory, job.w_cum_prev = _p(s_buf), _p(memory), _p(w_cum_prev)
    job.w_out, job.ld_wout, job.w_cum_out, job.v = _p(w_out), int(w_out.stride(0)), _p(w_cum_out), _p(v)
    job.ctx_dst[0] = t16_view(ctx_t16, K=E)
    job.n_ctx_dst, job.parts, job.L, job.A, job.E, job.F, job.K = 1, int(parts), L, A, E, int(F_), int(K)
    hv = t16_view(h_q_t16, K=Q)
    check(_lib.load().st_query_attn_fin_fwd(_p(packed_wq), C.byref(hv), 16 * kb16(Q), _p(granules), int(epoch), C.byref(job), B,
                                            stream_handle()), 'st_query_attn_fin_fwd')
    return granules


def query_attn_rng(packed_wq, h_q_t16, Q, s_buf, memory, w_cum_prev, v, w_out, w_cum_out, ctx_t16, parts, epoch=1, granules=None,
                   xchg=None, status=None):
    lib = _lib.load()
    B, L, E = memory.shape
    A = s_buf.shape[-1]
    if granules is None:
        granules = torch.zeros(B, 2 * A, device=memory.device, dtype=torch.float32)
    if xchg is None:
        xchg = torch.zeros(2 * int(lib.st_attn_rng_xchg_words(B, E, int(parts))), device=memory.device, dtype=torch.float32)
    job = _lib.StAttnFinJob()
    job.s_buf, job.memory, job.w_cum_prev = _p(s_buf), _p(memory), _p(w_cum_prev)
    job.w_out, job.ld_wout, job.w_cum_out, job.v = _p(w_out), int(w_out.stride(0)), _p(w_cum_out), _p(v)
    job.ctx_dst[0] = t16_view(ctx_t16, K=E)
    job.n_ctx_dst, job.parts, job.L, job.A, job.E, job.F, job.K = 1, int(parts), L, A, E, 0, 0
    job.status = _p(status, torch.int32)
    hv = t16_view(h_q_t16, K=Q)
    check(lib.st_query_attn_rng_fwd(_p(packed_wq), C.byref(hv), 16 * kb16(Q), _p(granules), _p(xchg), int(epoch), C.byref(job), B,
                                    stream_handle()), 'st_query_attn_rng_fwd')
    return granules, xchg


class _ParamLayouts:
    MAX_ENTRIES = 1024

    def __init__(self):
        self.entries = {}
        self.cats = {}
        self.table = None
        self.blk_desc = None
        self.count = 0
        self.total_blocks = 0
        self.dirty = True
        self.refreshes = 0
        self.epoch = 0

    def get(self, w, mode):
        key = (w.data_ptr(), tuple(w.shape), mode)
        e = self.entries.get(key)
        if e is not None:
            e[4] = self.epoch
            if capturing():
                e[5] = True
            if e[2] != e[0]._version:
                self.epoch += 1
                e[4] = self.epoch
                self.refresh()
# ... 1399 lines not shown
```

Baseline: 2.896 million.

## Fold location conv and linear into one packed filter applied via MFMA

Precomputes the product of the location-conv weights and the location-linear weights into a single A x (2K) filter, packed at weight-pack time in an MFMA-friendly layout. The attention-pre stage then computes s = pm + filter * [w_prev, w_cum] windows directly with 16x16x4 f32 MFMAs, with no LDS and no intermediate F-channel conv output. This cuts the two-stage conv+linear work and the LDS footprint, which could also improve occupancy of the fused linear+attn-pre kernel. In exchange the per-tap work grows from F to A columns, and summation order changes because the product is precomputed in double.

```diff
diff --git a/include/semitts.h b/include/semitts.h
--- a/include/semitts.h
+++ b/include/semitts.h
@@ -111,6 +111,10 @@
 int st_attn_pre_fwd(const float* pm, const float* w_prev, int ld_wprev, const float* w_cum_prev,
                     const float* loc_conv_w, const float* loc_lin_w, float* s_buf, int parts,
                     int B, int L, int A, int F, int K, void* stream);
+size_t st_attn_loc_filter_floats(int A, int K);
+int st_attn_loc_filter_pack(const float* loc_conv_w, const float* loc_lin_w, float* loc_filter, int A, int F, int K, void* stream);
+int st_attn_pre_fused_fwd(const float* pm, const float* w_prev, int ld_wprev, const float* w_cum_prev, const float* loc_filter,
+                          float* s_buf, int parts, int B, int L, int A, int K, void* stream);
 int st_attn_fin_t16_fwd(const float* pq, const float* s_buf, const float* memory, const float* w_cum_prev,
                         float* w_out, int ld_wout, float* w_cum_out, const float* v,
                         const st_t16_view* ctx_dst, int n_ctx_dst, float* ctx, int ld_ctx, int parts,
@@ -123,6 +127,7 @@
     int parts;
     float* cf_out;
     const struct st_partial_product_job* part;
+    const float* loc_filter;
 } st_attn_pre_job;
 int st_skinny_linear_packed_attnpre_fwd(const float* packed_w, const st_t16_view* x, int K,
                                         const float* bias, int act, const float* mask, int ldmask,
@@ -423,6 +428,7 @@
     float* pre_nat_tape;
     float* gate_part;
     int gate_part_k;
+    int attn_pre_two_phase;
 } st_decoder_io;
 
 int st_decoder_gate_split_k(const st_decoder_dims* d);
@@ -432,6 +438,7 @@
 int st_decoder_forward(const st_decoder_weights* w, const st_decoder_dims* d, const st_decoder_io* io,
                        void* stream);
 int st_decoder_fwd_forms(const st_decoder_dims* d, const st_decoder_io* io, int cus, int rng_capacity);
+int st_decoder_attn_pre_form(const st_decoder_dims* d, const st_decoder_io* io);
 
 int st_attn_step_bwd(const float* pq, const float* pm, const float* memory,
                      const float* w_prev, int ld_wprev, const float* w_cum_prev, const float* w, int ld_w,
diff --git a/semi_tts_amd/_lib.py b/semi_tts_amd/_lib.py
--- a/semi_tts_amd/_lib.py
+++ b/semi_tts_amd/_lib.py
@@ -72,7 +72,8 @@
                 ('pre1_step_floats', C.c_int), ('attn_s_step_floats', C.c_int), ('attn_loc_tape', C.c_void_p),
                 ('attn_split_ws', C.c_void_p), ('attn_split_parts', C.c_int), ('pq_granules', C.c_void_p),
                 ('dec_in0', C.c_void_p), ('pre_nat', C.c_void_p), ('attn_xchg', C.c_void_p), ('handoff_status', C.c_void_p),
-                ('pair_cells', C.c_int), ('pre_nat_tape', C.c_void_p), ('gate_part', C.c_void_p), ('gate_part_k', C.c_int)]
+                ('pair_cells', C.c_int), ('pre_nat_tape', C.c_void_p), ('gate_part', C.c_void_p), ('gate_part_k', C.c_int),
+                ('attn_pre_two_phase', C.c_int)]
 
 
 class StDecoderBwdWeights(C.Structure):
@@ -146,7 +147,7 @@
     _fields_ = [('pm', C.c_void_p), ('w_prev', C.c_void_p), ('ld_wprev', C.c_int), ('w_cum_prev', C.c_void_p),
                 ('loc_conv_w', C.c_void_p), ('loc_lin_w', C.c_void_p), ('s_buf', C.c_void_p),
                 ('L', C.c_int), ('A', C.c_int), ('F', C.c_int), ('K', C.c_int), ('parts', C.c_int), ('cf_out', C.c_void_p),
-                ('part', C.c_void_p)]
+                ('part', C.c_void_p), ('loc_filter', C.c_void_p)]
 
 
 class StAttnFinJob(C.Structure):
@@ -235,6 +236,9 @@
     'st_skinny_linear_packed_attnpre_fwd': [P, C.POINTER(StT16View), I, P, I, P, I, P, I, C.POINTER(StT16View), I, P, I, I,
                                             I, I, P, I, C.POINTER(StT16View), I, I, C.POINTER(StAttnPreJob), P],
     'st_attn_pre_fwd': [P, P, I, P, P, P, P, I, I, I, I, I, I, P],
+    'st_attn_loc_filter_floats': [I, I],
+    'st_attn_loc_filter_pack': [P, P, P, I, I, I, P],
+    'st_attn_pre_fused_fwd': [P, P, I, P, P, P, I, I, I, I, I, P],
     'st_attn_fin_t16_fwd': [P, P, P, P, P, I, P, P, C.POINTER(StT16View), I, P, I, I, I, I, I, I, I, I, P],
     'st_attn_fin_split_workspace_floats': [I, I, I],
     'st_attn_fin_split_fwd': [P, P, P, P, P, I, P, P, C.POINTER(StT16View), I, P, I, P, I, I, I, I, I, P],
@@ -257,6 +261,7 @@
     'st_decoder_pack': [C.POINTER(StDecoderWeights), C.POINTER(StDecoderDims), P, P],
     'st_decoder_forward': [C.POINTER(StDecoderWeights), C.POINTER(StDecoderDims), C.POINTER(StDecoderIO), P],
     'st_decoder_fwd_forms': [C.POINTER(StDecoderDims), C.POINTER(StDecoderIO), I, I],
+    'st_decoder_attn_pre_form': [C.POINTER(StDecoderDims), C.POINTER(StDecoderIO)],
     'st_attn_step_bwd': [P, P, P, P, I, P, P, I, P, P, P, C.POINTER(P), C.POINTER(I), I, C.POINTER(P), C.POINTER(I), I,
                          P, P, I, P, P, P, P, P, P, P, P, I, I, I, I, I, I, P],
     'st_attn_step_bwd_s': [P, P, P, P, I, P, P, I, P, P, P, C.POINTER(P), C.POINTER(I), I, C.POINTER(P), C.POINTER(I), I,
@@ -354,7 +359,7 @@
     'st_feature_noise': [P, C.c_long, I, C.c_ulonglong, P],
 }
 _RESTYPES = {'st_last_error': C.c_char_p, 'st_packed_weight_floats': C.c_size_t, 'st_t16_floats': C.c_size_t,
-             'st_decoder_packed_floats': C.c_size_t, 'st_vq_l2_workspace_floats': C.c_size_t, 'st_ctc_workspace_floats': C.c_size_t, 'st_decoder_tape_floats': C.c_size_t,
+             'st_decoder_packed_floats': C.c_size_t, 'st_attn_loc_filter_floats': C.c_size_t, 'st_vq_l2_workspace_floats': C.c_size_t, 'st_ctc_workspace_floats': C.c_size_t, 'st_decoder_tape_floats': C.c_size_t,
              'st_gemm_wgrad_workspace_floats': C.c_size_t, 'st_gemm_wgrad_batch_workspace_floats': C.c_size_t, 'st_freq_loss_workspace_floats': C.c_size_t, 'st_attn_fin_split_workspace_floats': C.c_size_t, 'st_attn_rng_xchg_words': C.c_size_t, 'st_colreduce_workspace_floats': C.c_size_t, 'st_mt_blocks': C.c_size_t, 'st_mt_table_misses': C.c_long,
              'st_bn_bank_workspace_floats': C.c_size_t, 'st_istft_workspace_floats': C.c_size_t, 'st_gl_workspace_floats': C.c_size_t,
              'st_features_workspace_floats': C.c_size_t, 'st_ctc_beam_workspace_bytes': C.c_size_t, 'st_ctc_align_workspace_bytes': C.c_size_t}
diff --git a/semi_tts_amd/csrc/attention.hip b/semi_tts_amd/csrc/attention.hip
--- a/semi_tts_amd/csrc/attention.hip
+++ b/semi_tts_amd/csrc/attention.hip
@@ -237,6 +237,53 @@
     return at_launch<1>(a, (hipStream_t)stream);
 }
 
+namespace {
+
+__global__ __launch_bounds__(256) void at_loc_filter_pack_kernel(const float* conv_w, const float* lin_w, float* out, int A, int F, int K) {
+    const size_t total = at_wf_floats(A);
+    for (size_t idx = (size_t)blockIdx.x * blockDim.x + threadIdx.x; idx < total; idx += (size_t)gridDim.x * blockDim.x) {
+        const int e = (int)(idx & 3), lane = (int)((idx >> 2) & 63), q = (int)((idx >> 8) % (AT_WF_KS / 4)), mt = (int)((idx >> 8) / (AT_WF_KS / 4));
+        const int s = 4 * q + e, c = s / (AT_WF_KS / 2), k = 4 * (s % (AT_WF_KS / 2)) + (lane >> 4), row = mt * 16 + (lane & 15);
+        double acc = 0.0;
+        if (k < K)
+            for (int f = 0; f < F; ++f) acc += (double)lin_w[(size_t)row * F + f] * (double)conv_w[((size_t)f * 2 + c) * K + k];
+        out[idx] = (float)acc;
+    }
+}
+
+__global__ __launch_bounds__(AT_THREADS) void at_pre_fused_kernel(const AtArgs a) { at_pre_fused_body(a, blockIdx.x); }
+
+}
+
+extern "C" size_t st_attn_loc_filter_floats(int A, int K) { return at_wf_shape_ok(A, K) ? at_wf_floats(A) : 0; }
+
+extern "C" int st_attn_loc_filter_pack(const float* loc_conv_w, const float* loc_lin_w, float* loc_filter, int A, int F, int K, void* stream) {
+    (void)hipGetLastError();
+    ST_CHECK_ARG(loc_conv_w && loc_lin_w && loc_filter && F > 0, "st_attn_loc_filter_pack: null pointer / F=%d", F);
+    ST_CHECK_ARG(at_wf_shape_ok(A, K) && (K & 1), "st_attn_loc_filter_pack: A=%d must be a multiple of 16, K=%d odd and <= %d", A, K, AT_WF_KC);
+    const size_t total = at_wf_floats(A);
+    hipLaunchKernelGGL(at_loc_filter_pack_kernel, dim3((unsigned)((total + 255) / 256)), dim3(256), 0, (hipStream_t)stream, loc_conv_w, loc_lin_w,
+                       loc_filter, A, F, K);
+    ST_LAUNCH_CHECK();
+    return 0;
+}
+
+extern "C" int st_attn_pre_fused_fwd(const float* pm, const float* w_prev, int ld_wprev, const float* w_cum_prev, const float* loc_filter,
+                                     float* s_buf, int parts, int B, int L, int A, int K, void* stream) {
+    (void)hipGetLastError();
+    ST_CHECK_ARG(pm && w_prev && w_cum_prev && loc_filter && s_buf && B > 0 && L > 0, "st_attn_pre_fused_fwd: null pointer / B=%d L=%d", B, L);
+    ST_CHECK_ARG(at_wf_shape_ok(A, K) && (K & 1), "st_attn_pre_fused_fwd: A=%d must be a multiple of 16, K=%d odd and <= %d", A, K, AT_WF_KC);
+    ST_CHECK_ARG(st_aligned16(pm) && st_aligned16(s_buf) && st_aligned16(loc_filter), "st_attn_pre_fused_fwd: pm / s_buf / loc_filter must be 16-byte aligned");
+    AtArgs a;
+    memset(&a, 0, sizeof(a));
+    a.pm = pm; a.w_prev = w_prev; a.ld_wprev = ld_wprev; a.w_cum_prev = w_cum_prev; a.loc_filter = loc_filter; a.s_buf = s_buf;
+    a.pre_parts = (parts >= 2 && parts <= 64 && (parts & (parts - 1)) == 0) ? parts : 1;
+    a.B = B; a.L = L; a.A = A; a.E = 4; a.K = K;
+    hipLaunchKernelGGL(at_pre_fused_kernel, dim3(B * a.pre_parts), dim3(AT_THREADS), 0, (hipStream_t)stream, a);
+    ST_LAUNCH_CHECK();
+    return 0;
+}
+
 extern "C" int st_attn_fin_t16_fwd(const float* pq, const float* s_buf, const float* memory, const float* w_cum_prev,
                                    float* w_out, int ld_wout, float* w_cum_out, const float* v,
                                    const st_t16_view* ctx_dst, int n_ctx_dst, float* ctx, int ld_ctx, int parts,
diff --git a/semi_tts_amd/csrc/attention_body.h b/semi_tts_amd/csrc/attention_body.h
--- a/semi_tts_amd/csrc/attention_body.h
+++ b/semi_tts_amd/csrc/attention_body.h
@@ -29,7 +29,13 @@
     int B, L, A, E, F, K;
     const unsigned long long* pq_gran; unsigned epoch;
     unsigned* status;
+    const float* loc_filter;
 };
+
+constexpr int AT_WF_KC = 32;
+constexpr int AT_WF_KS = 2 * AT_WF_KC / 4;
+__host__ __device__ inline size_t at_wf_floats(int A) { return (size_t)(A >> 4) * (AT_WF_KS / 4) * 64 * 4; }
+__host__ __device__ inline bool at_wf_shape_ok(int A, int K) { return A > 0 && (A & 15) == 0 && K > 0 && K <= AT_WF_KC; }
 
 constexpr int AT_GRAN_SPINS = 1 << 18;
 __device__ __forceinline__ f32x4 at_wait_granules(const unsigned long long* base, unsigned epoch, int lane, int A, unsigned* status,
@@ -680,6 +686,70 @@
 }
 
 
+constexpr int AT_PF_MT = 2, AT_PF_NT = 3;
+__device__ __forceinline__ void at_pre_fused_body(const AtArgs& a, const int wg) {
+    const int nparts = a.pre_parts > 1 ? a.pre_parts : 1;
+    const int pshift = 31 - __builtin_clz((unsigned)nparts);
+    const int b = wg >> pshift, ipart = wg & (nparts - 1);
+    const int tid = threadIdx.x, lane = tid & 63, wave = __builtin_amdgcn_readfirstlane(tid >> 6);
+    const int L = a.L, A = a.A, K = a.K;
+    const int pos_per = (L + nparts - 1) >> pshift;
+    const int pos_lo = min(L, ipart * pos_per), pos_hi = min(L, pos_lo + pos_per);
+    const int g = lane >> 4, n = lane & 15;
+    const int pad = (K - 1) / 2, MT = A >> 4;
+    const int ntile = (pos_hi - pos_lo + 15) >> 4;
+    const unsigned L4 = (unsigned)L * 4u;
+    const __amdgpu_buffer_rsrc_t r0 = __builtin_amdgcn_make_buffer_rsrc((void*)(a.w_prev + (size_t)b * a.ld_wprev), 0, L * 4, 0x00020000);
+    const __amdgpu_buffer_rsrc_t r1 = __builtin_amdgcn_make_buffer_rsrc((void*)(a.w_cum_prev + (size_t)b * L), 0, L * 4, 0x00020000);
+    const float* pmb = a.pm + (size_t)b * L * A;
+    const f32x4* wf = reinterpret_cast<const f32x4*>(a.loc_filter);
+    for (int j0 = 0; j0 < ntile; j0 += AT_PF_NT) {
+        float hv[AT_PF_NT][AT_WF_KS];
+#pragma unroll
+        for (int jj = 0; jj < AT_PF_NT; ++jj) {
+            const int lbase = pos_lo + (j0 + jj) * 16 + n - pad;
+#pragma unroll
+            for (int s = 0; s < AT_WF_KS / 2; ++s) {
+                const int k = 4 * s + g;
+                const unsigned off = k < K ? min((unsigned)((lbase + k) * 4), L4) : L4;
+                hv[jj][s] = __uint_as_float(__builtin_amdgcn_raw_buffer_load_b32(r0, off, 0, 0));
+                hv[jj][s + AT_WF_KS / 2] = __uint_as_float(__builtin_amdgcn_raw_buffer_load_b32(r1, off, 0, 0));
+            }
+        }
+        for (int m0 = wave; m0 < MT; m0 += AT_PF_MT * AT_WAVES) {
+            f32x4 aw[AT_PF_MT][AT_WF_KS / 4], pm4[AT_PF_MT][AT_PF_NT];
+#pragma unroll
+            for (int i = 0; i < AT_PF_MT; ++i) {
+                const int mt = min(m0 + i * AT_WAVES, MT - 1);
+#pragma unroll
+                for (int q = 0; q < AT_WF_KS / 4; ++q) aw[i][q] = wf[((size_t)mt * (AT_WF_KS / 4) + q) * 64 + lane];
+#pragma unroll
+                for (int jj = 0; jj < AT_PF_NT; ++jj) {
+                    const int l = min(pos_lo + (j0 + jj) * 16 + n, L - 1);
+                    pm4[i][jj] = st_ld4(pmb + (size_t)l * A + mt * 16 + 4 * g);
+                }
+            }
+#pragma unroll
+            for (int i = 0; i < AT_PF_MT; ++i) {
+                const int mt = m0 + i * AT_WAVES;
+                if (mt >= MT) break;
+#pragma unroll
+                for (int jj = 0; jj < AT_PF_NT; ++jj) {
+                    if (j0 + jj >= ntile) break;
+                    f32x4 acc = {0.f, 0.f, 0.f, 0.f};
+#pragma unroll
+                    for (int s = 0; s < AT_WF_KS; ++s) acc = __builtin_amdgcn_mfma_f32_16x16x4f32(aw[i][s >> 2][s & 3], hv[jj][s], acc, 0, 0, 0);
+                    const int l = pos_lo + (j0 + jj) * 16 + n;
+                    if (l < pos_hi) {
+                        const f32x4 sv = {acc[0] + pm4[i][jj][0], acc[1] + pm4[i][jj][1], acc[2] + pm4[i][jj][2], acc[3] + pm4[i][jj][3]};
+                        *reinterpret_cast<f32x4*>(a.s_buf + ((size_t)b * L + l) * A + mt * 16 + 4 * g) = sv;
+                    }
+                }
+            }
+        }
+    }
+}
+
 template <bool VEC, int PART, int NT = AT_THREADS>
 __global__ __launch_bounds__(NT) void at_kernel(const float* pq, const float* pm, const float* v, const float* w_cum_prev, const float* memory,
                                                 float* s_buf, const int L, const int A, const int E, const int fin_parts, const AtArgs rest) {
diff --git a/semi_tts_amd/csrc/decoder.hip b/semi_tts_amd/csrc/decoder.hip
--- a/semi_tts_amd/csrc/decoder.hip
+++ b/semi_tts_amd/csrc/decoder.hip
@@ -22,7 +22,7 @@
 namespace {
 
 struct PackedLayout {
-    size_t q, pq, d, pg, p0, p1, total;
+    size_t q, pq, d, pg, p0, p1, wf, total;
 };
 
 PackedLayout packed_layout(const st_decoder_dims* d) {
@@ -35,6 +35,8 @@
     { int k[2] = {d->D, d->E}; o.pg = p; p += st_packed_weight_floats(k, 2, in_dim + 1 + (d->fuse_pre0 ? d->P : 0), 0); }
     { int k[1] = {in_dim}; o.p0 = p; p += st_packed_weight_floats(k, 1, d->P, 0); }
     { int k[1] = {d->P}; o.p1 = p; p += st_packed_weight_floats(k, 1, d->P, 0); }
+    p = (p + 3) & ~(size_t)3;
+    o.wf = p; p += st_attn_loc_filter_floats(d->A, d->K);
     o.total = p;
     return o;
 }
@@ -137,7 +139,11 @@
     j[3].N = in_dim + 1 + (d->fuse_pre0 ? d->P : 0); j[3].packed = packed + pl.pg;
     seg(j[4], 0, w->prenet_w0, in_dim, in_dim); j[4].N = d->P; j[4].packed = packed + pl.p0;
     seg(j[5], 0, w->prenet_w1, d->P, d->P); j[5].N = d->P; j[5].packed = packed + pl.p1;
-    return st_pack_weight_batch(j, 6, stream);
+    int rc = st_pack_weight_batch(j, 6, stream);
+    if (rc) return rc;
+    if (st_attn_loc_filter_floats(d->A, d->K) && w->attn_loc_conv_w && w->attn_loc_lin_w && d->F > 0 && (d->K & 1))
+        rc = st_attn_loc_filter_pack(w->attn_loc_conv_w, w->attn_loc_lin_w, packed + pl.wf, d->A, d->F, d->K, stream);
+    return rc;
 }
 
 extern "C" size_t st_decoder_tape_floats(const st_decoder_dims* d, int which) {
@@ -170,6 +176,7 @@
     FwdProd prod;
     int fin_parts;
     int pq_pre_parts;
+    bool pre_fused;
     int d_k0;
 };
 
@@ -203,6 +210,8 @@
     else if (fuse_pq_fin && (A / 16) * BT + B * f.fin_parts + (4 * D) / 32 <= cus) f.prod = PROD_PQ_FIN;
     else f.prod = PROD_OWN;
     f.d_k0 = (io->gate_part_k ? io->gate_part_k : st_decoder_gate_split_k(d)) / 16;
+    f.pre_fused = split_attn && !io->attn_pre_two_phase && !io->attn_loc_tape && st_attn_loc_filter_floats(A, d->K) > 0 && d->F > 0 && (d->K & 1) &&
+                  st_aligned16(io->pm) && st_aligned16(io->attn_s_buf) && (io->attn_s_step_floats & 3) == 0 && st_aligned16(io->packed);
     return f;
 }
 
@@ -215,6 +224,13 @@
     const FwdForms f = fwd_forms(d, io, cus > 0 ? cus : st_device_cus(), rng_capacity > 0 ? rng_capacity : pk_attnrng_capacity());
     return (int)f.attn | ((int)f.prod << 4) | (f.pure_tf ? 1 << 8 : 0) | (f.defer ? 1 << 9 : 0) | (f.pre_in_pq ? 1 << 10 : 0) |
            (f.pair_cells ? 1 << 11 : 0) | (f.fin_parts << 12) | ((f.prod != PROD_NONE ? f.d_k0 & 0xfff : 0) << 16);
+}
+
+extern "C" int st_decoder_attn_pre_form(const st_decoder_dims* d, const st_decoder_io* io) {
+    if (!d || !io) return -1;
+    st_decoder_io q = *io;
+    q.steps = 0;
+    return fwd_forms(d, &q, st_device_cus(), pk_attnrng_capacity()).pre_fused ? 1 : 0;
 }
 
 static int decoder_forward_issue(const st_decoder_weights* w, const st_decoder_dims* d, const st_decoder_io* io, void* stream);
@@ -353,6 +369,7 @@
                 st_attn_pre_job job = {io->pm, io->align_out + (size_t)(t - 1) * L, ldal, io->wcum_tape + (size_t)t * BL,
                                        w->attn_loc_conv_w, w->attn_loc_lin_w, io->attn_s_buf + (size_t)t * io->attn_s_step_floats, L, A, d->F,
                                        d->K, f.pq_pre_parts, io->attn_loc_tape ? io->attn_loc_tape + (size_t)t * BL * d->F : nullptr};
+                if (f.pre_fused) job.loc_filter = io->packed + pl.wf;
                 if (f.prod == PROD_PQ_PRE) job.part = &pj_d;
                 rc = st_skinny_linear_packed_attnpre_fwd(io->packed + pl.pq, &hq_dst, 16 * kb16(Q), nullptr, ST_ACT_NONE, nullptr, 0,
                                                          io->pq_buf, A, nullptr, 0, nullptr, 0, 0, 0, 0, nullptr, 0, nullptr, B, A,
@@ -463,6 +480,7 @@
                                w->attn_loc_conv_w, w->attn_loc_lin_w,
                                split_attn ? io->attn_s_buf + (size_t)(t + 1) * io->attn_s_step_floats : nullptr, L, A, d->F, d->K,
                                io->attn_pre_parts, io->attn_loc_tape ? io->attn_loc_tape + (size_t)(t + 1) * BL * d->F : nullptr};
+        if (f.pre_fused) job.loc_filter = io->packed + pl.wf;
         if (!ST_SKIPPED(4)) {
             rc = st_skinny_linear_packed_attnpre_fwd(io->packed + pl.pg, &xo_v, ST_SKIPPED(7) ? Ko / 4 : Ko, w->projgate_b, ST_ACT_NONE, nullptr, 0,
                                                      io->mel_out + (size_t)t * in_dim, (int)ldmel, fuse ? nullptr : &mel_dst, in_dim,
diff --git a/semi_tts_amd/csrc/skinny_packed.hip b/semi_tts_amd/csrc/skinny_packed.hip
--- a/semi_tts_amd/csrc/skinny_packed.hip
+++ b/semi_tts_amd/csrc/skinny_packed.hip
@@ -918,6 +918,7 @@
         const int by = n_lin <= 2 * tiles_a ? (i >= tiles_a ? 1 : 0) : i / tiles_a;
         pk_body<1, NB, KW, TRIP>(a, i - by * tiles_a, by, red);
     }
+    else if (VEC && t.loc_filter) at_pre_fused_body(t, i - n_lin);
     else at_body<VEC, 1>(t, i - n_lin, pk_dyn_lds);
 }
 
@@ -938,7 +939,8 @@
     } else if (i < n_lin + n_at) {
         AtArgs t = t_rest;
         t.pm = at_pm; t.w_prev = at_wprev; t.L = at_L;
-        at_body<VEC, 1>(t, i - n_lin, pk_dyn_lds);
+        if (VEC && t.loc_filter) at_pre_fused_body(t, i - n_lin);
+        else at_body<VEC, 1>(t, i - n_lin, pk_dyn_lds);
     } else pk_part_body<KW, 2>(p, i - n_lin - n_at, reinterpret_cast<f32x4*>(pk_dyn_lds));
 }
 
@@ -1000,13 +1002,16 @@
 int pk_fill(PkArgs& a, const float* packed_w, const st_t16_view* x, int K, const char* who);
 
 template <int NB>
-int pk_launch_attnpre(const PkArgs& a, int tiles, const AtArgs& t, hipStream_t st, const PkPartArgs* pp = nullptr) {
+int pk_launch_attnpre(const PkArgs& a, int tiles, const AtArgs& t_in, hipStream_t st, const PkPartArgs* pp = nullptr) {
     constexpr int KW = 8, TRIP = NB == 1 ? PK_TRIP_SMALL : 2;
     const int BT = (a.B + 15) >> 4, gy = (BT + NB - 1) / NB;
+    AtArgs t = t_in;
+    const bool fused = t.loc_filter && !t.cf_out && at_wf_shape_ok(t.A, t.K) && st_aligned16(t.pm) && st_aligned16(t.s_buf) && st_aligned16(t.loc_filter);
+    if (!fused) t.loc_filter = nullptr;
+    const bool vec = fused || ((t.A % 4 == 0) && (t.F % 4 == 0) && st_aligned16(t.pm) && st_aligned16(t.loc_lin_w) && st_aligned16(t.s_buf));
     if constexpr (NB == 1) if (pp) {
-        const bool vec = (t.A % 4 == 0) && (t.F % 4 == 0) && st_aligned16(t.pm) && st_aligned16(t.loc_lin_w) && st_aligned16(t.s_buf);
         const AtLds o = at_layout(t.L, t.A, t.E, t.F, t.K, 1, at_pos_per(t.L, t.pre_parts > 1 ? t.pre_parts : 1), vec && t.F == 32 && t.A % 16 == 0);
-        size_t lds = (size_t)o.total * sizeof(float);
+        size_t lds = fused ? 0 : (size_t)o.total * sizeof(float);
         if (lds < sizeof(f32x4) * KW * 4 * 64) lds = sizeof(f32x4) * KW * 4 * 64;
         ST_CHECK_ARG(lds + sizeof(f32x4) * KW * NB * 64 <= 160 * 1024, "linear + attention-pre launch: L=%d needs too much LDS (use more parts)", t.L);
         auto kern = vec ? pk_attnpre_part_kernel<NB, KW, TRIP, true> : pk_attnpre_part_kernel<NB, KW, TRIP, false>;
@@ -1021,9 +1026,8 @@
         ST_LAUNCH_CHECK();
         return 0;
     }
-    const bool vec = (t.A % 4 == 0) && (t.F % 4 == 0) && st_aligned16(t.pm) && st_aligned16(t.loc_lin_w) && st_aligned16(t.s_buf);
     const AtLds o = at_layout(t.L, t.A, t.E, t.F, t.K, 1, at_pos_per(t.L, t.pre_parts > 1 ? t.pre_parts : 1), vec && t.F == 32 && t.A % 16 == 0);
-    const size_t lds = (size_t)o.total * sizeof(float);
+    const size_t lds = fused ? 0 : (size_t)o.total * sizeof(float);
     ST_CHECK_ARG(lds + sizeof(f32x4) * KW * NB * 64 <= 160 * 1024, "linear + attention-pre launch: L=%d needs too much LDS (use more parts)", t.L);
     auto kern = vec ? pk_attnpre_kernel<NB, KW, TRIP, true> : pk_attnpre_kernel<NB, KW, TRIP, false>;
     static size_t configured[2] = {0, 0};
@@ -1343,6 +1347,7 @@
         memset(&t, 0, sizeof(t));
         t.pm = pre->pm; t.w_prev = pre->w_prev; t.ld_wprev = pre->ld_wprev; t.w_cum_prev = pre->w_cum_prev;
         t.loc_conv_w = pre->loc_conv_w; t.loc_lin_w = pre->loc_lin_w; t.s_buf = pre->s_buf; t.cf_out = pre->cf_out;
+        t.loc_filter = pre->loc_filter;
         t.B = B; t.L = pre->L; t.A = pre->A; t.E = 4; t.F = pre->F; t.K = pre->K;
         t.pre_parts = (pre->parts >= 2 && pre->parts <= 64 && (pre->parts & (pre->parts - 1)) == 0) ? pre->parts : 1;
         const int BT = (B + 15) >> 4;
diff --git a/semi_tts_amd/module.py b/semi_tts_amd/module.py
--- a/semi_tts_amd/module.py
+++ b/semi_tts_amd/module.py
@@ -311,6 +311,8 @@
         self.cache_packed = False
         self.attn_split = True
         self.attn_pre_parts = 4
+        self.attn_pre_fused = os.environ.get('ST_ATTN_PRE_FUSED', '1') != '0'
+        self._last_attn_pre_form = None
         self.attn_fin_parts = 2
         self.attn_pq_in_fin = True
         self.split_gates = os.environ.get('ST_SPLIT_GATES', '1') != '0'
@@ -567,7 +569,9 @@
                 if self.handoff_status is None or self.handoff_status.device != dev:
                     self.handoff_status = torch.zeros(1, device=dev, dtype=torch.int32)
                 io.handoff_status = ops._p(self.handoff_status, torch.int32)
+        io.attn_pre_two_phase = 0 if self.attn_pre_fused else 1
         self._last_fwd_forms = int(lib.st_decoder_fwd_forms(C.byref(dims), C.byref(io), 0, 0))
+        self._last_attn_pre_form = int(lib.st_decoder_attn_pre_form(C.byref(dims), C.byref(io)))
         check(lib.st_decoder_forward(C.byref(w), C.byref(dims), C.byref(io), ops.stream_handle()),
               'st_decoder_forward')
         if io.handoff_status and self.check_handoff and not ops.capturing():
diff --git a/semi_tts_amd/ops.py b/semi_tts_amd/ops.py
--- a/semi_tts_amd/ops.py
+++ b/semi_tts_amd/ops.py
@@ -194,6 +194,27 @@
         s_buf = torch.empty(B, L, A, device=pm.device, dtype=torch.float32)
     check(_lib.load().st_attn_pre_fwd(_p(pm), _p(w_prev), int(w_prev.stride(0)), _p(w_cum_prev), _p(loc_conv_w), _p(loc_lin_w),
                                       _p(s_buf), int(parts), B, L, A, F_, K, stream_handle()), 'st_attn_pre_fwd')
+    return s_buf
+
+
+def attn_loc_filter(loc_conv_w, loc_lin_w):
+    F_, _, K = loc_conv_w.shape
+    A = loc_lin_w.shape[0]
+    lib = _lib.load()
+    n = int(lib.st_attn_loc_filter_floats(A, K))
+    if n == 0:
+        return None
+    filt = torch.empty(n, device=loc_lin_w.device, dtype=torch.float32)
+    check(lib.st_attn_loc_filter_pack(_p(loc_conv_w), _p(loc_lin_w), _p(filt), A, F_, K, stream_handle()), 'st_attn_loc_filter_pack')
+    return filt
+
+
+def attn_pre_fused(pm, w_prev, w_cum_prev, loc_filter, K, s_buf=None, parts=1):
+    B, L, A = pm.shape
+    if s_buf is None:
+        s_buf = torch.empty(B, L, A, device=pm.device, dtype=torch.float32)
+    check(_lib.load().st_attn_pre_fused_fwd(_p(pm), _p(w_prev), int(w_prev.stride(0)), _p(w_cum_prev), _p(loc_filter), _p(s_buf), int(parts),
+                                            B, L, A, int(K), stream_handle()), 'st_attn_pre_fused_fwd')
     return s_buf
 
 
```

Measured after the change: 2.868 million. About the same (-1.0%).
